# pixeli99/SVD_Xtend

Hardware: NVIDIA H100
Metric: SVD UNet train-step frames/sec @ 14x320x512 bf16 (higher is better)
Workload: dtype bf16

## Files before the change

include/svd_xtend_b200.h:

```cpp
#ifndef SVD_XTEND_B200_H_
#define SVD_XTEND_B200_H_

#include <stdint.h>

#ifdef __cplusplus
extern "C" {
#endif

#define SVDX_OK 0
#define SVDX_E_BADARG (-1)
#define SVDX_E_CUDA (-2)
#define SVDX_E_NODRIVER (-3)

#define SVDX_MAX_TAPS 27

#define SVDX_A_ROWS 0
#define SVDX_A_CONV2D 1

#define SVDX_OUT_BF16 0
#define SVDX_OUT_F32 1
#define SVDX_OUT_F32_ATOMIC 2

typedef struct SvdxTapGemm {
  const void* a;
  int64_t lda;
  int32_t a_mode;
  int32_t a_major_mn;
  int32_t rows_per_group, groups;
  int32_t W, H, nimg;
  int32_t num_taps;
  int32_t tap_d0[SVDX_MAX_TAPS];
  int32_t tap_d1[SVDX_MAX_TAPS];
  int32_t tap_d2[SVDX_MAX_TAPS];
  const void* b;
  int64_t ldb;
  int32_t b_major_mn;
  int32_t b_mode;
  int32_t M, N, K;
  int32_t block_n;
  int32_t split_k;
  void* out;
  int64_t ldo;
  int32_t out_dtype;
  int32_t geglu;
  const float* bias;
  const float* rowbias;
  int32_t rowbias_div;
  int64_t ldrb;
  const void* res1;
  int64_t ldr1;
  const void* res2;
  int64_t ldr2;
  const float* scales;
  void* pre;
  int64_t ldpre;
  float* gn_sum;
  int64_t gn_ld;
  int32_t gn_rows;
  const void* gnb_x;
  int64_t gnb_ldx;
  const void* gnb_x2;
  int64_t gnb_ldx2;
  int32_t gnb_c1;
  const float* gnb_ab;
  float* gnb_sum;
  int32_t gnb_rows;
  int32_t gnb_silu;
  int32_t interleave;
  int32_t phase_h, phase_w;
  int32_t act;
} SvdxTapGemm;

#define SVDX_ACT_NONE 0
#define SVDX_ACT_GELU 1
#define SVDX_ACT_QUICK_GELU 2

int svdx_tapgemm(const SvdxTapGemm* desc, void* stream);

int svdx_splitk_epilogue(float* ws, int64_t ldw, void* out, int64_t ldo, int64_t rows, int32_t cols, const float* bias,
                         const float* rowbias, int32_t rowbias_div, int64_t ldrb, const void* res1, int64_t ldr1,
                         const void* res2, int64_t ldr2, const float* scales, void* stream);

int svdx_num_sms(void);
int svdx_enable_peer_access(int32_t peer_device);
int svdx_ipc_export(const void* ptr, void* handle64_out, int64_t* offset_out);
int svdx_ipc_import(const void* handle64, int64_t offset, void** ptr_out);
int svdx_struct_size(int which);
const char* svdx_last_error(void);

int svdx_groupnorm_sums(const void* x, int64_t ldx, int32_t C1, const void* x2, int64_t ldx2, int32_t C2,
                        int32_t outer, int32_t rows, float* sums, int64_t ld, void* stream);
int svdx_groupnorm_apply_fused(const void* x, int64_t ldx, int32_t C1, const void* x2, int64_t ldx2, int32_t C2,
                               int32_t outer, int32_t rows, int32_t num_groups, float eps,
                               const float* csum1, int64_t ldc1, const float* csum2, int64_t ldc2,
                               float* mean, float* rstd, const float* gamma, const float* beta,
                               int32_t fuse_silu, void* y, int64_t ldy, float* ab_out, void* stream);
int svdx_groupnorm_bwd_sums(const void* x, int64_t ldx, int32_t C1, const void* x2, int64_t ldx2, int32_t C2,
                            const void* dy, int64_t lddy, int32_t outer, int32_t rows, const float* ab, int32_t fuse_silu,
                            float* sums, void* stream);
int svdx_groupnorm_bwd_fused(const void* x, int64_t ldx, int32_t C1, const void* x2, int64_t ldx2, int32_t C2,
                             const void* dy, int64_t lddy, int32_t outer, int32_t rows, int32_t num_groups,
                             const float* mean, const float* rstd, const float* gamma, const float* beta,
                             int32_t fuse_silu, const float* csum, void* dx, int64_t lddx, void* dx2, int64_t lddx2,
                             float* dgamma, float* dbeta, const void* dres, int64_t lddres, void* stream);

int svdx_layernorm_fwd(const void* x, int64_t ldx, int32_t rows, int32_t C, const float* gamma, const float* beta,
                       float eps, void* y, int64_t ldy, float* mean, float* rstd,
                       const float* addvec, int32_t add_div, void* xsum, int64_t ldxs, void* stream);
int svdx_layernorm_bwd(const void* x, int64_t ldx, const void* dy, int64_t lddy, int32_t rows, int32_t C,
                       const float* gamma, const float* mean, const float* rstd,
                       void* dx, int64_t lddx, const void* dres, int64_t lddres,
                       float* dgamma, float* dbeta, void* stream);

typedef struct SvdxAttn {
  const void* q; const void* k; const void* v; void* o;
  int64_t ldq, ldk, ldv, ldo;
  int32_t nseq, heads, S;
  int32_t inner;
  int64_t outer_stride, inner_stride, tok_stride;
  float scale;
  float* lse;
  const void* dout; int64_t lddo;
  void* dq; void* dk; void* dv; int64_t lddq, lddk, lddv;
  float* delta;
} SvdxAttn;
int svdx_attention_fwd(const SvdxAttn* d, void* stream);
int svdx_attention_bwd(const SvdxAttn* d, void* stream);

int svdx_attention_hd80_fwd(const void* q, int64_t ldq, const void* k, int64_t ldk, const void* v, int64_t ldv, void* o,
                            int64_t ldo, int32_t nseq, int32_t heads, int32_t S, float scale, void* stream);

#define SVDX_CLIP_MAX_TAPS 63
int svdx_clip_preprocess(const void* x, int32_t x_dtype, const int64_t* x_strides, int32_t B, int32_t H, int32_t W,
                         const float* gy, int32_t ky, const float* gx, int32_t kx, const float* affine,
                         int32_t out_size, int32_t patch, void* out, int64_t ldo, void* stream);

int svdx_prep_weight(const void* src, int32_t src_bf16, void* dst, int32_t mode,
                     int32_t O, int32_t I, int32_t taps, int32_t i_pad, void* stream);
int svdx_unprep_conv_grad(const float* src, float* dst, int32_t O, int32_t I, int32_t taps, int32_t i_pad, void* stream);
int svdx_dot_diff(const void* dy, const void* a, const void* b, int64_t n, float* out, void* stream);
int svdx_silu_bwd_f32(const float* x, const float* dy, float* dx, int64_t n, void* stream);
int svdx_cast_f32_bf16(const float* src, void* dst, int64_t n, void* stream);
int svdx_cast_bf16_f32(const void* src, float* dst, int64_t n, void* stream);
int svdx_cast_f16_f32(const void* src, float* dst, int64_t n, void* stream);
int svdx_nchw_to_nhwc(const void* src, int32_t src_bf16, void* dst, int32_t N, int32_t C, int32_t H, int32_t W,
                      int32_t c_pad, void* stream);
int svdx_nhwc_to_nchw(const void* src, int64_t lds, void* dst, int32_t dst_bf16, int32_t N, int32_t C, int32_t H,
                      int32_t W, void* stream);
int svdx_time_conv_out(const float* x, int64_t ldx, int32_t N, int32_t T, int32_t C, int32_t H, int32_t W, const float* w,
                       const float* bias, void* y, int32_t y_dtype, void* stream);
int svdx_upsample2x(const void* src, void* dst, int32_t N, int32_t H, int32_t W, int32_t C, void* stream);
int svdx_upsample2x_bwd(const void* dsrc, void* ddst, int32_t N, int32_t H, int32_t W, int32_t C, void* stream);
int svdx_space_to_planes(const void* src, void* dst, int32_t N, int32_t H, int32_t W, int32_t C, void* stream);
int svdx_planes_to_space(const void* src, void* dst, int32_t N, int32_t H, int32_t W, int32_t C, void* stream);
int svdx_concat_channels(const void* a, int32_t Ca, const void* b, int32_t Cb, void* dst, int64_t rows, void* stream);
int svdx_split_channels(const void* src, void* a, int32_t Ca, void* b, int32_t Cb, int64_t rows, int32_t accumulate_a,
                        void* stream);
int svdx_add_bf16(const void* a, const void* b, void* y, int64_t n, void* stream);
int svdx_axpby_bf16(const void* a, const void* b, const float* scales, void* y, int64_t n, void* stream);
int svdx_silu_f32(const float* x, float* y, int64_t n, void* stream);
int svdx_colsum(const void* x, int64_t ldx, int64_t rows, int32_t cols, float* out, int32_t accumulate, void* stream);
int svdx_geglu_bwd(const void* pre, int64_t ldpre, const void* dout, int64_t lddo, void* dpre, int64_t lddpre,
                   int64_t rows, int32_t h, float* bias_grad, void* stream);
int svdx_softmax_rows(const void* x, int64_t ldx, int64_t rows, int32_t cols, float scale, void* y, int64_t ldy, void* stream);
int svdx_gemv(const void* a, int64_t lda, const void* w, int64_t ldw, int32_t M, int32_t N, int32_t K, const float* bias,
              void* out, int64_t ldo, int32_t out_dtype, float scale, int32_t accumulate, void* stream);
int svdx_outer_accum(const void* dy, int64_t lddy, const void* x, int64_t ldx, int32_t T, int32_t O, int32_t K,
                     const float* scale, float* g, int64_t ldg, void* stream);
int svdx_blend_scales(const float* mix_factor, float* out16, void* stream);
int svdx_adamw_graph(float* p, const float* g, float* m, float* v, int64_t n, float* state, float grad_scale,
                     void* shadow_bf16, void* stream);
int svdx_adamw_p2p(float* p, float* m, float* v, const void* const* grads, void* const* shadows, int32_t world,
                   int64_t lo, int64_t n, float* state, float grad_scale, int32_t tick, void* stream);

int svdx_grad_sumsq(const float* g, int64_t n, double* sumsq, void* stream);
int svdx_grad_sumsq_p2p(const void* const* grads, int32_t world, int64_t lo, int64_t n, double* sumsq, void* stream);
int svdx_clip_coef(const double* sumsq, const float* max_norm, float scale, float* out, void* stream);

int svdx_adamw_graph_ema(float* p, const float* g, float* m, float* v, int64_t n, float* state, float grad_scale,
                         void* shadow_bf16, float* ema, double* ema_state, void* stream);
int svdx_adamw_p2p_ema(float* p, float* m, float* v, const void* const* grads, void* const* shadows, int32_t world,
                       int64_t lo, int64_t n, float* state, float grad_scale, int32_t tick, float* ema, double* ema_state,
                       void* stream);
int svdx_ema_multi(const void* jobs, const int32_t* block_prefix, int32_t njobs, int32_t total_blocks, double* ema_state,
                   void* stream);

int svdx_adamw8bit(const void* jobs, const int32_t* block_prefix, int32_t njobs, int32_t total_blocks, const float* qmap1,
                   const float* qmap2, float* state, float grad_scale, void* stream);
int svdx_adamw8bit_ema(const void* jobs, const int32_t* block_prefix, int32_t njobs, int32_t total_blocks, const float* qmap1,
                       const float* qmap2, float* state, float grad_scale, double* ema_state, void* stream);

int svdx_adamw_graph_mul(float* p, const float* g, float* m, float* v, int64_t n, float* state, float grad_scale,
                         void* shadow_bf16, const float* grad_mul, void* stream);
int svdx_adamw_graph_ema_mul(float* p, const float* g, float* m, float* v, int64_t n, float* state, float grad_scale,
                             void* shadow_bf16, float* ema, double* ema_state, const float* grad_mul, void* stream);
int svdx_adamw_p2p_mul(float* p, float* m, float* v, const void* const* grads, void* const* shadows, int32_t world,
                       int64_t lo, int64_t n, float* state, float grad_scale, int32_t tick, const float* grad_mul, void* stream);
int svdx_adamw_p2p_ema_mul(float* p, float* m, float* v, const void* const* grads, void* const* shadows, int32_t world,
                           int64_t lo, int64_t n, float* state, float grad_scale, int32_t tick, float* ema, double* ema_state,
                           const float* grad_mul, void* stream);
int svdx_adamw8bit_mul(const void* jobs, const int32_t* block_prefix, int32_t njobs, int32_t total_blocks, const float* qmap1,
                       const float* qmap2, float* state, float grad_scale, const float* grad_mul, void* stream);
int svdx_adamw8bit_ema_mul(const void* jobs, const int32_t* block_prefix, int32_t njobs, int32_t total_blocks, const float* qmap1,
                           const float* qmap2, float* state, float grad_scale, double* ema_state, const float* grad_mul, void* stream);

int svdx_vae_frames_in(const void* x, int32_t x_dtype, const float* cond_eps, const float* cond_sigma, int32_t B, int32_t F,
                       int32_t H, int32_t W, int32_t c_pad, void* dst, void* stream);
int svdx_vae_frames_in_range(const void* x, int32_t x_dtype, const float* cond_eps, const float* cond_sigma, int32_t B, int32_t F,
                             int32_t H, int32_t W, int32_t first, int32_t count, int32_t c_pad, void* dst, void* stream);
typedef struct svdx_clip_desc {
  int64_t start;
  int32_t H0, W0;
  int32_t ty_off, tx_off;
} svdx_clip_desc;
int svdx_resize_taps_ksize(int32_t in_size, int32_t out_size);
int svdx_resize_taps(int32_t in_size, int32_t out_size, int32_t* taps);
int svdx_resize_taps_box_ksize(int32_t in_size, int32_t out_size, float in0, float in1);
int svdx_resize_taps_box(int32_t in_size, int32_t out_size, float in0, float in1, int32_t* taps);
int svdx_frames_u8_in(const uint8_t* src, int32_t H0, int32_t W0, const int32_t* taps_y, int32_t ksize_y, const int32_t* taps_x,
                      int32_t ksize_x, const float* cond_eps, const float* cond_sigma, int32_t B, int32_t F, int32_t H, int32_t W,
                      int32_t first, int32_t count, int32_t c_pad, void* dst, float* first_frames, void* stream);
int svdx_frames_u8_in_clips(const uint8_t* src, int64_t src_bytes, const svdx_clip_desc* descs, const int32_t* taps_y,
                            int32_t ty_rows, int32_t ksize_y, const int32_t* taps_x, int32_t tx_rows, int32_t ksize_x,
// ... 17 lines not shown
```

svd_xtend_b200/_lib.py:

```python
from __future__ import annotations

import ctypes as C
import os
from pathlib import Path

PKG = Path(__file__).resolve().parent
LIB_PATH = Path(os.environ["SVDX_LIB"]) if os.environ.get("SVDX_LIB") else PKG / "lib" / "libsvdx_b200.so"

SVDX_MAX_TAPS = 27
SVDX_CLIP_MAX_TAPS = 63
A_ROWS, A_CONV2D = 0, 1
OUT_BF16, OUT_F32, OUT_F32_ATOMIC = 0, 1, 2
ACT_NONE, ACT_GELU, ACT_QUICK_GELU = 0, 1, 2

c_void_p, c_int, c_i64, c_float = C.c_void_p, C.c_int32, C.c_int64, C.c_float


class SvdxTapGemm(C.Structure):
    _fields_ = [
        ("a", c_void_p), ("lda", c_i64), ("a_mode", c_int), ("a_major_mn", c_int),
        ("rows_per_group", c_int), ("groups", c_int),
        ("W", c_int), ("H", c_int), ("nimg", c_int),
        ("num_taps", c_int),
        ("tap_d0", c_int * SVDX_MAX_TAPS), ("tap_d1", c_int * SVDX_MAX_TAPS), ("tap_d2", c_int * SVDX_MAX_TAPS),
        ("b", c_void_p), ("ldb", c_i64), ("b_major_mn", c_int), ("b_mode", c_int),
        ("M", c_int), ("N", c_int), ("K", c_int),
        ("block_n", c_int), ("split_k", c_int),
        ("out", c_void_p), ("ldo", c_i64), ("out_dtype", c_int), ("geglu", c_int),
        ("bias", c_void_p), ("rowbias", c_void_p), ("rowbias_div", c_int), ("ldrb", c_i64),
        ("res1", c_void_p), ("ldr1", c_i64), ("res2", c_void_p), ("ldr2", c_i64),
        ("scales", c_void_p), ("pre", c_void_p), ("ldpre", c_i64),
        ("gn_sum", c_void_p), ("gn_ld", c_i64), ("gn_rows", c_int),
        ("gnb_x", c_void_p), ("gnb_ldx", c_i64), ("gnb_x2", c_void_p), ("gnb_ldx2", c_i64), ("gnb_c1", c_int),
        ("gnb_ab", c_void_p), ("gnb_sum", c_void_p), ("gnb_rows", c_int), ("gnb_silu", c_int),
        ("interleave", c_int), ("phase_h", c_int), ("phase_w", c_int),
        ("act", c_int),
    ]


class SvdxAttn(C.Structure):
    _fields_ = [
        ("q", c_void_p), ("k", c_void_p), ("v", c_void_p), ("o", c_void_p),
        ("ldq", c_i64), ("ldk", c_i64), ("ldv", c_i64), ("ldo", c_i64),
        ("nseq", c_int), ("heads", c_int), ("S", c_int), ("inner", c_int),
        ("outer_stride", c_i64), ("inner_stride", c_i64), ("tok_stride", c_i64),
        ("scale", c_float), ("lse", c_void_p),
        ("dout", c_void_p), ("lddo", c_i64),
        ("dq", c_void_p), ("dk", c_void_p), ("dv", c_void_p),
        ("lddq", c_i64), ("lddk", c_i64), ("lddv", c_i64),
        ("delta", c_void_p),
    ]


_PROTOS = {
    "svdx_tapgemm": [C.POINTER(SvdxTapGemm), c_void_p],
    "svdx_splitk_epilogue": [c_void_p, c_i64, c_void_p, c_i64, c_i64, c_int, c_void_p, c_void_p, c_int, c_i64, c_void_p, c_i64,
                             c_void_p, c_i64, c_void_p, c_void_p],
    "svdx_num_sms": [],
    "svdx_enable_peer_access": [c_int],
    "svdx_ipc_export": [c_void_p, c_void_p, c_void_p],
    "svdx_ipc_import": [c_void_p, c_i64, c_void_p],
    "svdx_struct_size": [c_int],
    "svdx_groupnorm_sums": [c_void_p, c_i64, c_int, c_void_p, c_i64, c_int, c_int, c_int, c_void_p, c_i64, c_void_p],
    "svdx_groupnorm_apply_fused": [c_void_p, c_i64, c_int, c_void_p, c_i64, c_int, c_int, c_int, c_int, c_float,
                                   c_void_p, c_i64, c_void_p, c_i64, c_void_p, c_void_p, c_void_p, c_void_p, c_int, c_void_p, c_i64, c_void_p,
                                   c_void_p],
    "svdx_groupnorm_bwd_fused": [c_void_p, c_i64, c_int, c_void_p, c_i64, c_int, c_void_p, c_i64, c_int, c_int, c_int,
                                 c_void_p, c_void_p, c_void_p, c_void_p, c_int, c_void_p, c_void_p, c_i64, c_void_p, c_i64,
                                 c_void_p, c_void_p, c_void_p, c_i64, c_void_p],
    "svdx_groupnorm_bwd_sums": [c_void_p, c_i64, c_int, c_void_p, c_i64, c_int, c_void_p, c_i64, c_int, c_int, c_void_p, c_int,
                                c_void_p, c_void_p],
    "svdx_layernorm_fwd": [c_void_p, c_i64, c_int, c_int, c_void_p, c_void_p, c_float, c_void_p, c_i64,
                           c_void_p, c_void_p, c_void_p, c_int, c_void_p, c_i64, c_void_p],
    "svdx_layernorm_bwd": [c_void_p, c_i64, c_void_p, c_i64, c_int, c_int, c_void_p, c_void_p, c_void_p,
                           c_void_p, c_i64, c_void_p, c_i64, c_void_p, c_void_p, c_void_p],
    "svdx_attention_fwd": [C.POINTER(SvdxAttn), c_void_p],
    "svdx_attention_bwd": [C.POINTER(SvdxAttn), c_void_p],
    "svdx_attention_hd80_fwd": [c_void_p, c_i64, c_void_p, c_i64, c_void_p, c_i64, c_void_p, c_i64, c_int, c_int, c_int, c_float, c_void_p],
    "svdx_clip_preprocess": [c_void_p, c_int, C.POINTER(c_i64), c_int, c_int, c_int, C.POINTER(c_float), c_int, C.POINTER(c_float), c_int,
                             C.POINTER(c_float), c_int, c_int, c_void_p, c_i64, c_void_p],
    "svdx_prep_weight": [c_void_p, c_int, c_void_p, c_int, c_int, c_int, c_int, c_int, c_void_p],
    "svdx_unprep_conv_grad": [c_void_p, c_void_p, c_int, c_int, c_int, c_int, c_void_p],
    "svdx_dot_diff": [c_void_p, c_void_p, c_void_p, c_i64, c_void_p, c_void_p],
    "svdx_silu_bwd_f32": [c_void_p, c_void_p, c_void_p, c_i64, c_void_p],
    "svdx_cast_f32_bf16": [c_void_p, c_void_p, c_i64, c_void_p],
    "svdx_cast_bf16_f32": [c_void_p, c_void_p, c_i64, c_void_p],
    "svdx_cast_f16_f32": [c_void_p, c_void_p, c_i64, c_void_p],
    "svdx_nchw_to_nhwc": [c_void_p, c_int, c_void_p, c_int, c_int, c_int, c_int, c_int, c_void_p],
    "svdx_nhwc_to_nchw": [c_void_p, c_i64, c_void_p, c_int, c_int, c_int, c_int, c_int, c_void_p],
    "svdx_time_conv_out": [c_void_p, c_i64, c_int, c_int, c_int, c_int, c_int, c_void_p, c_void_p, c_void_p, c_int, c_void_p],
    "svdx_upsample2x": [c_void_p, c_void_p, c_int, c_int, c_int, c_int, c_void_p],
    "svdx_upsample2x_bwd": [c_void_p, c_void_p, c_int, c_int, c_int, c_int, c_void_p],
    "svdx_space_to_planes": [c_void_p, c_void_p, c_int, c_int, c_int, c_int, c_void_p],
    "svdx_planes_to_space": [c_void_p, c_void_p, c_int, c_int, c_int, c_int, c_void_p],
    "svdx_concat_channels": [c_void_p, c_int, c_void_p, c_int, c_void_p, c_i64, c_void_p],
    "svdx_split_channels": [c_void_p, c_void_p, c_int, c_void_p, c_int, c_i64, c_int, c_void_p],
    "svdx_add_bf16": [c_void_p, c_void_p, c_void_p, c_i64, c_void_p],
    "svdx_axpby_bf16": [c_void_p, c_void_p, c_void_p, c_void_p, c_i64, c_void_p],
    "svdx_silu_f32": [c_void_p, c_void_p, c_i64, c_void_p],
    "svdx_colsum": [c_void_p, c_i64, c_i64, c_int, c_void_p, c_int, c_void_p],
    "svdx_geglu_bwd": [c_void_p, c_i64, c_void_p, c_i64, c_void_p, c_i64, c_i64, c_int, c_void_p, c_void_p],
    "svdx_softmax_rows": [c_void_p, c_i64, c_i64, c_int, c_float, c_void_p, c_i64, c_void_p],
    "svdx_gemv": [c_void_p, c_i64, c_void_p, c_i64, c_int, c_int, c_int, c_void_p, c_void_p, c_i64, c_int, c_float, c_int, c_void_p],
    "svdx_outer_accum": [c_void_p, c_i64, c_void_p, c_i64, c_int, c_int, c_int, c_void_p, c_void_p, c_i64, c_void_p],
    "svdx_blend_scales": [c_void_p, c_void_p, c_void_p],
    "svdx_adamw_graph": [c_void_p, c_void_p, c_void_p, c_void_p, c_i64, c_void_p, c_float, c_void_p, c_void_p],
    "svdx_adamw_p2p": [c_void_p, c_void_p, c_void_p, c_void_p, c_void_p, c_int, c_i64, c_i64, c_void_p, c_float, c_int, c_void_p],
    "svdx_grad_sumsq": [c_void_p, c_i64, c_void_p, c_void_p],
    "svdx_grad_sumsq_p2p": [c_void_p, c_int, c_i64, c_i64, c_void_p, c_void_p],
    "svdx_clip_coef": [c_void_p, c_void_p, c_float, c_void_p, c_void_p],
    "svdx_adamw_graph_ema": [c_void_p, c_void_p, c_void_p, c_void_p, c_i64, c_void_p, c_float, c_void_p, c_void_p, c_void_p, c_void_p],
    "svdx_adamw_p2p_ema": [c_void_p, c_void_p, c_void_p, c_void_p, c_void_p, c_int, c_i64, c_i64, c_void_p, c_float, c_int, c_void_p,
                           c_void_p, c_void_p],
    "svdx_ema_multi": [c_void_p, c_void_p, c_int, c_int, c_void_p, c_void_p],
    "svdx_adamw8bit": [c_void_p, c_void_p, c_int, c_int, c_void_p, c_void_p, c_void_p, c_float, c_void_p],
    "svdx_adamw8bit_ema": [c_void_p, c_void_p, c_int, c_int, c_void_p, c_void_p, c_void_p, c_float, c_void_p, c_void_p],
    "svdx_adamw_graph_mul": [c_void_p, c_void_p, c_void_p, c_void_p, c_i64, c_void_p, c_float, c_void_p, c_void_p, c_void_p],
    "svdx_adamw_graph_ema_mul": [c_void_p, c_void_p, c_void_p, c_void_p, c_i64, c_void_p, c_float, c_void_p, c_void_p, c_void_p,
                                 c_void_p, c_void_p],
    "svdx_adamw_p2p_mul": [c_void_p, c_void_p, c_void_p, c_void_p, c_void_p, c_int, c_i64, c_i64, c_void_p, c_float, c_int, c_void_p,
                           c_void_p],
    "svdx_adamw_p2p_ema_mul": [c_void_p, c_void_p, c_void_p, c_void_p, c_void_p, c_int, c_i64, c_i64, c_void_p, c_float, c_int,
                               c_void_p, c_void_p, c_void_p, c_void_p],
    "svdx_adamw8bit_mul": [c_void_p, c_void_p, c_int, c_int, c_void_p, c_void_p, c_void_p, c_float, c_void_p, c_void_p],
    "svdx_adamw8bit_ema_mul": [c_void_p, c_void_p, c_int, c_int, c_void_p, c_void_p, c_void_p, c_float, c_void_p, c_void_p, c_void_p],
    "svdx_multi_transpose": [c_void_p, c_void_p, c_void_p, c_int, c_int, c_void_p],
    "svdx_lora_merge": [c_void_p, c_void_p, c_void_p, c_int, c_int, c_void_p],
    "svdx_vae_frames_in": [c_void_p, c_int, c_void_p, c_void_p, c_int, c_int, c_int, c_int, c_int, c_void_p, c_void_p],
    "svdx_vae_frames_in_range": [c_void_p, c_int, c_void_p, c_void_p, c_int, c_int, c_int, c_int, c_int, c_int, c_int, c_void_p,
                                 c_void_p],
    "svdx_resize_taps_ksize": [c_int, c_int],
    "svdx_resize_taps": [c_int, c_int, c_void_p],
    "svdx_resize_taps_box_ksize": [c_int, c_int, c_float, c_float],
    "svdx_resize_taps_box": [c_int, c_int, c_float, c_float, c_void_p],
    "svdx_frames_u8_in": [c_void_p, c_int, c_int, c_void_p, c_int, c_void_p, c_int, c_void_p, c_void_p, c_int, c_int, c_int, c_int,
                          c_int, c_int, c_int, c_void_p, c_void_p, c_void_p],
    "svdx_frames_u8_in_clips": [c_void_p, c_i64, c_void_p, c_void_p, c_int, c_int, c_void_p, c_int, c_int, c_void_p, c_void_p, c_int,
                                c_int, c_int, c_int, c_int, c_int, c_int, c_void_p, c_void_p, c_void_p],
    "svdx_edm_prepare": [c_void_p, c_void_p, c_void_p, c_void_p, c_void_p, c_void_p, c_float, c_int, c_int, c_int, c_int, c_int,
                         c_void_p, c_void_p, c_void_p, c_void_p],
}

EXPORTED_SYMBOLS = tuple(_PROTOS) + ("svdx_last_error",)

_lib = None


def load() -> C.CDLL:
    global _lib
    if _lib is None:
        if not LIB_PATH.exists():
            raise RuntimeError(
                f"svd_xtend_b200: native library {LIB_PATH} is missing — run `python -m svd_xtend_b200.build` "
                "(there is no CPU or PyTorch fallback for the hot path)")
        lib = C.CDLL(str(LIB_PATH))
        missing = [n for n in _PROTOS if not hasattr(lib, n)]
        if missing and os.environ.get("SVDX_ALLOW_PARTIAL"):
            for n in missing:
                _PROTOS.pop(n)
            missing = []
        if missing:
            raise RuntimeError(f"svd_xtend_b200: {LIB_PATH} lacks symbols {missing}; rebuild it")
        for name, args in _PROTOS.items():
            fn = getattr(lib, name)
            fn.argtypes = args
            fn.restype = C.c_int
        if lib.svdx_struct_size(0) != C.sizeof(SvdxTapGemm) or lib.svdx_struct_size(1) != C.sizeof(SvdxAttn):
            raise RuntimeError("svd_xtend_b200: ctypes struct layout does not match the C ABI")
        lib.svdx_last_error.restype = C.c_char_p
        lib.svdx_last_error.argtypes = []
        _lib = lib
    return _lib


class SvdxError(RuntimeError):
    pass


def check(rc: int, what: str = "") -> None:
    if rc != 0:
        msg = load().svdx_last_error().decode(errors="replace")
        raise SvdxError(f"{what} failed with status {rc}: {msg}")
```

svd_xtend_b200/csrc/common.cuh:

```cuda
#pragma once
#include <cuda.h>
#include <cuda_bf16.h>
#include <cuda_runtime.h>
#include <stdint.h>
#include <stdio.h>

#include "wgmma.cuh"

namespace svdx {

typedef __nv_bfloat16 bf16;

#define SVDX_DEVINL __device__ __forceinline__

#ifndef SVDX_WAIT_TIMEOUT_CYCLES
#define SVDX_WAIT_TIMEOUT_CYCLES (4000000000ll)
#endif

SVDX_DEVINL uint32_t smem_u32(const void* p) { return (uint32_t)__cvta_generic_to_shared(p); }

SVDX_DEVINL uint32_t lane_id() { return threadIdx.x & 31; }

SVDX_DEVINL bool elect_one() {
  uint32_t pred = 0;
// ... 8 lines not shown
SVDX_DEVINL void mbar_init(uint32_t bar, uint32_t count) {
  asm volatile("mbarrier.init.shared::cta.b64 [%0], %1;" ::"r"(bar), "r"(count) : "memory");
}
SVDX_DEVINL void fence_barrier_init() {
  asm volatile("fence.mbarrier_init.release.cluster;" ::: "memory");
}
SVDX_DEVINL void fence_proxy_async_smem() {
  asm volatile("fence.proxy.async.shared::cta;" ::: "memory");
}
SVDX_DEVINL void mbar_expect_tx(uint32_t bar, uint32_t bytes) {
  asm volatile("mbarrier.arrive.expect_tx.shared::cta.b64 _, [%0], %1;" ::"r"(bar), "r"(bytes) : "memory");
}
SVDX_DEVINL void mbar_arrive(uint32_t bar) {
  asm volatile("mbarrier.arrive.shared::cta.b64 _, [%0];" ::"r"(bar) : "memory");
}
SVDX_DEVINL bool mbar_try_wait(uint32_t bar, uint32_t parity) {
  uint32_t ok;
  asm volatile(
      "{\n\t.reg .pred P;\n\t"
      "mbarrier.try_wait.parity.shared::cta.b64 P, [%1], %2;\n\t"
      "selp.u32 %0, 1, 0, P;\n\t}\n"
      : "=r"(ok)
      : "r"(bar), "r"(parity)
      : "memory");
  return ok != 0;
}
SVDX_DEVINL void mbar_wait(uint32_t bar, uint32_t parity) {
  if (mbar_try_wait(bar, parity)) return;
  long long t0 = clock64();
  while (!mbar_try_wait(bar, parity)) {
    if (clock64() - t0 > SVDX_WAIT_TIMEOUT_CYCLES) {
      printf("svdx: mbarrier wait timeout block %d thread %d bar %u parity %u\n", blockIdx.x, threadIdx.x, bar, parity);
      __trap();
    }
  }
}

SVDX_DEVINL void mbar_wait_mma(uint32_t bar, uint32_t parity) {
  if (mbar_try_wait(bar, parity)) return;
  long long t0 = clock64();
  while (!mbar_try_wait(bar, parity))
    if (clock64() - t0 > SVDX_WAIT_TIMEOUT_CYCLES) __trap();
}

SVDX_DEVINL void prefetch_tmap(const CUtensorMap* m) {
  asm volatile("prefetch.tensormap [%0];" ::"l"(reinterpret_cast<uint64_t>(m)) : "memory");
}
SVDX_DEVINL void tma_load_2d(const CUtensorMap* m, uint32_t bar, uint32_t dst, int c0, int c1) {
  asm volatile(
      "cp.async.bulk.tensor.2d.shared::cluster.global.mbarrier::complete_tx::bytes [%0], [%1, {%3, %4}], [%2];"
      ::"r"(dst), "l"(reinterpret_cast<uint64_t>(m)), "r"(bar), "r"(c0), "r"(c1)
      : "memory");
}
SVDX_DEVINL void tma_load_3d(const CUtensorMap* m, uint32_t bar, uint32_t dst, int c0, int c1, int c2) {
  asm volatile(
      "cp.async.bulk.tensor.3d.shared::cluster.global.mbarrier::complete_tx::bytes [%0], [%1, {%3, %4, %5}], [%2];"
      ::"r"(dst), "l"(reinterpret_cast<uint64_t>(m)), "r"(bar), "r"(c0), "r"(c1), "r"(c2)
      : "memory");
}
SVDX_DEVINL void tma_load_4d(const CUtensorMap* m, uint32_t bar, uint32_t dst, int c0, int c1, int c2, int c3) {
  asm volatile(
      "cp.async.bulk.tensor.4d.shared::cluster.global.mbarrier::complete_tx::bytes [%0], [%1, {%3, %4, %5, %6}], [%2];"
      ::"r"(dst), "l"(reinterpret_cast<uint64_t>(m)), "r"(bar), "r"(c0), "r"(c1), "r"(c2), "r"(c3)
      : "memory");
}
SVDX_DEVINL void tma_load_4d_im2col(const CUtensorMap* m, uint32_t bar, uint32_t dst, int c0, int c1, int c2, int c3, uint16_t ow,
                                    uint16_t oh) {
  asm volatile(
      "cp.async.bulk.tensor.4d.shared::cluster.global.im2col.mbarrier::complete_tx::bytes [%0], [%1, {%3, %4, %5, %6}], [%2], {%7, %8};"
      ::"r"(dst), "l"(reinterpret_cast<uint64_t>(m)), "r"(bar), "r"(c0), "r"(c1), "r"(c2), "r"(c3), "h"(ow), "h"(oh)
      : "memory");
}

SVDX_DEVINL void tma_store_3d(const CUtensorMap* m, uint32_t src, int c0, int c1, int c2) {
  asm volatile("cp.async.bulk.tensor.3d.global.shared::cta.bulk_group [%0, {%2, %3, %4}], [%1];"
               ::"l"(reinterpret_cast<uint64_t>(m)), "r"(src), "r"(c0), "r"(c1), "r"(c2)
               : "memory");
}
SVDX_DEVINL void tma_store_4d(const CUtensorMap* m, uint32_t src, int c0, int c1, int c2, int c3) {
  asm volatile("cp.async.bulk.tensor.4d.global.shared::cta.bulk_group [%0, {%2, %3, %4, %5}], [%1];"
               ::"l"(reinterpret_cast<uint64_t>(m)), "r"(src), "r"(c0), "r"(c1), "r"(c2), "r"(c3)
               : "memory");
}
SVDX_DEVINL void tma_reduce_add_3d(const CUtensorMap* m, uint32_t src, int c0, int c1, int c2) {
  asm volatile("cp.reduce.async.bulk.tensor.3d.global.shared::cta.add.bulk_group [%0, {%2, %3, %4}], [%1];"
               ::"l"(reinterpret_cast<uint64_t>(m)), "r"(src), "r"(c0), "r"(c1), "r"(c2)
               : "memory");
}
SVDX_DEVINL void bulk_commit() { asm volatile("cp.async.bulk.commit_group;" ::: "memory"); }
template <int N>
SVDX_DEVINL void bulk_wait_read() { asm volatile("cp.async.bulk.wait_group.read %0;" ::"n"(N) : "memory"); }
template <int N>
SVDX_DEVINL void bulk_wait() { asm volatile("cp.async.bulk.wait_group %0;" ::"n"(N) : "memory"); }
SVDX_DEVINL void st_shared_v4(uint32_t addr, uint32_t a, uint32_t b, uint32_t c, uint32_t d) {
  asm volatile("st.shared.v4.b32 [%0], {%1, %2, %3, %4};" ::"r"(addr), "r"(a), "r"(b), "r"(c), "r"(d) : "memory");
}

SVDX_DEVINL void wgmma_fence() { asm volatile("wgmma.fence.sync.aligned;" ::: "memory"); }
SVDX_DEVINL void wgmma_commit() { asm volatile("wgmma.commit_group.sync.aligned;" ::: "memory"); }
template <int N>
SVDX_DEVINL void wgmma_wait() { asm volatile("wgmma.wait_group.sync.aligned %0;" ::"n"(N) : "memory"); }
template <int R>
SVDX_DEVINL void reg_fence(float (&d)[R]) {
#pragma unroll
  for (int i = 0; i < R; ++i) asm volatile("" : "+f"(d[i])::"memory");
}

SVDX_DEVINL void named_bar_sync(int id, int nthreads) { asm volatile("bar.sync %0, %1;" ::"r"(id), "r"(nthreads) : "memory"); }

SVDX_DEVINL uint64_t make_smem_desc_sw128(uint32_t saddr, uint32_t lbo_bytes, uint32_t sbo_bytes) {
  uint64_t d = 0;
  d |= (uint64_t)((saddr & 0x3FFFF) >> 4);
  d |= (uint64_t)((lbo_bytes >> 4) & 0x3FFF) << 16;
  d |= (uint64_t)((sbo_bytes >> 4) & 0x3FFF) << 32;
  d |= (uint64_t)1 << 62;
  return d;
}

SVDX_DEVINL float silu_f(float x) { return __fdividef(x, 1.0f + __expf(-x)); }
SVDX_DEVINL float silu_grad_f(float x) {
  const float s = __fdividef(1.0f, 1.0f + __expf(-x));
  return s * fmaf(x, 1.0f - s, 1.0f);
}
#define SVDX_HDINL __host__ __device__ __forceinline__
SVDX_HDINL float gelu_tail_log2(float ax) {
  float p = -1.92123457e-06f;
  p = fmaf(p, ax, 6.32884985e-05f);
  p = fmaf(p, ax, -0.000943420862f);
  p = fmaf(p, ax, 0.0085562719f);
  p = fmaf(p, ax, -0.0540522821f);
  p = fmaf(p, ax, -0.458381772f);
  p = fmaf(p, ax, -1.15127838f);
  p = fmaf(p, ax, -0.999993861f);
  return p;
}
SVDX_HDINL float exp2_fast(float x) {
#ifdef __CUDA_ARCH__
  float y;
  asm("ex2.approx.ftz.f32 %0, %1;" : "=f"(y) : "f"(x));
  return y;
#else
  return exp2f(x);
#endif
}
SVDX_HDINL float normal_cdf_f(float x) {
  const float q = exp2_fast(gelu_tail_log2(fminf(fabsf(x), 5.5f)));
  return x < 0.f ? q : 1.0f - q;
}
SVDX_HDINL float gelu_erf_f(float x) { return x * normal_cdf_f(x); }
SVDX_HDINL float gelu_erf_grad_f(float x) {
  const float pdf = 0.3989422804014327f * exp2_fast(-0.72134752044448170f * x * x);
  return fmaf(x, pdf, normal_cdf_f(x));
}

SVDX_DEVINL uint32_t pack_bf16x2(float lo, float hi) {
  __nv_bfloat162 v = __floats2bfloat162_rn(lo, hi);
  return *reinterpret_cast<uint32_t*>(&v);
}
SVDX_DEVINL float2 unpack_bf16x2(uint32_t u) {
  __nv_bfloat162 v = *reinterpret_cast<__nv_bfloat162*>(&u);
  return __bfloat1622float2(v);
}

SVDX_DEVINL float warp_sum(float v) {
#pragma unroll
  for (int o = 16; o > 0; o >>= 1) v += __shfl_xor_sync(0xffffffffu, v, o);
  return v;
}
SVDX_DEVINL float warp_max(float v) {
#pragma unroll
  for (int o = 16; o > 0; o >>= 1) v = fmaxf(v, __shfl_xor_sync(0xffffffffu, v, o));
  return v;
}

}
```

svd_xtend_b200/csrc/elementwise.cu:

```cuda
#include "common.cuh"
#include "../../include/svd_xtend_b200.h"
#include "host_util.h"
#include <cuda_fp16.h>
#include <type_traits>

namespace svdx {

SVDX_DEVINL long long gtid() { return (long long)blockIdx.x * blockDim.x + threadIdx.x; }
static inline unsigned nblocks(long long n, int threads = 256) { return (unsigned)((n + threads - 1) / threads); }

template <typename T>
SVDX_DEVINL float ldf(const T* p, long long i);
template <>
SVDX_DEVINL float ldf<float>(const float* p, long long i) { return p[i]; }
template <>
SVDX_DEVINL float ldf<bf16>(const bf16* p, long long i) { return __bfloat162float(p[i]); }
template <>
SVDX_DEVINL float ldf<__half>(const __half* p, long long i) { return __half2float(p[i]); }

template <typename T>
__global__ void prep_gather_kernel(const T* __restrict__ src, bf16* __restrict__ dst, int mode, int O, int I, int taps, int i_pad) {
  const long long idx = gtid();
  if (mode == 0) {
    if (idx >= (long long)O * I) return;
// ... 137 lines not shown
  const int w2 = (int)(pix % (2 * W));
  const int h2 = (int)((pix / (2 * W)) % (2 * H));
  const int n = (int)(pix / ((long long)4 * W * H));
  dst[idx] = src[(((long long)n * H + (h2 >> 1)) * W + (w2 >> 1)) * CV + cv];
}
SVDX_DEVINL uint32_t add_bf16x2_f32(uint32_t a, uint32_t b, uint32_t c, uint32_t d) {
  const float2 x = unpack_bf16x2(a), y = unpack_bf16x2(b), z = unpack_bf16x2(c), w = unpack_bf16x2(d);
  return pack_bf16x2(x.x + y.x + z.x + w.x, x.y + y.y + z.y + w.y);
}
__global__ void upsample2x_bwd_kernel(const uint4* __restrict__ dsrc, uint4* __restrict__ ddst, int N, int H, int W, int CV) {
  const long long idx = gtid();
  const long long total = (long long)N * H * W * CV;
  if (idx >= total) return;
  const int cv = (int)(idx % CV);
  const long long pix = idx / CV;
  const int w = (int)(pix % W);
  const int h = (int)((pix / W) % H);
  const int n = (int)(pix / ((long long)W * H));
  const long long base = (((long long)n * 2 * H + 2 * h) * 2 * W + 2 * w) * CV + cv;
  const uint4 a = dsrc[base], b = dsrc[base + CV], c = dsrc[base + (long long)2 * W * CV], d = dsrc[base + (long long)2 * W * CV + CV];
  uint4 o;
  o.x = add_bf16x2_f32(a.x, b.x, c.x, d.x); o.y = add_bf16x2_f32(a.y, b.y, c.y, d.y);
  o.z = add_bf16x2_f32(a.z, b.z, c.z, d.z); o.w = add_bf16x2_f32(a.w, b.w, c.w, d.w);
  ddst[idx] = o;
}

__global__ void planes_kernel(const uint4* __restrict__ src, uint4* __restrict__ dst, int N, int H, int W, int CV, int to_planes) {
  const long long idx = gtid();
  const long long total = (long long)N * H * W * CV;
  if (idx >= total) return;
  const int cv = (int)(idx % CV);
  const long long pix = idx / CV;
  const int w = (int)(pix % W);
  const int h = (int)((pix / W) % H);
  const int n = (int)(pix / ((long long)W * H));
  const int Ho = H / 2, Wo = W / 2;
  const long long pidx = ((((long long)((h & 1) * 2 + (w & 1)) * N + n) * Ho + (h >> 1)) * Wo + (w >> 1)) * CV + cv;
  if (to_planes) dst[pidx] = src[idx]; else dst[idx] = src[pidx];
}

__global__ void concat_kernel(const uint4* __restrict__ a, int CVa, const uint4* __restrict__ b, int CVb, uint4* __restrict__ dst, long long rows) {
  const long long idx = gtid();
  const int CV = CVa + CVb;
  if (idx >= rows * CV) return;
  const long long r = idx / CV;
  const int c = (int)(idx - r * CV);
  dst[idx] = (c < CVa) ? a[r * CVa + c] : b[r * CVb + (c - CVa)];
}
__global__ void split_kernel(const uint4* __restrict__ src, uint4* __restrict__ a, int CVa, uint4* __restrict__ b, int CVb, long long rows,
                             int accumulate_a) {
  const long long idx = gtid();
  const int CV = CVa + CVb;
  if (idx >= rows * CV) return;
  const long long r = idx / CV;
  const int c = (int)(idx - r * CV);
  const uint4 v = src[idx];
  if (c < CVa) {
    uint4* p = a + r * CVa + c;
    if (accumulate_a) {
      const uint4 o = *p;
      uint4 s;
      float2 x, y;
      x = unpack_bf16x2(o.x); y = unpack_bf16x2(v.x); s.x = pack_bf16x2(x.x + y.x, x.y + y.y);
      x = unpack_bf16x2(o.y); y = unpack_bf16x2(v.y); s.y = pack_bf16x2(x.x + y.x, x.y + y.y);
      x = unpack_bf16x2(o.z); y = unpack_bf16x2(v.z); s.z = pack_bf16x2(x.x + y.x, x.y + y.y);
      x = unpack_bf16x2(o.w); y = unpack_bf16x2(v.w); s.w = pack_bf16x2(x.x + y.x, x.y + y.y);
      *p = s;
    } else {
      *p = v;
    }
  } else if (b) {
    b[r * CVb + (c - CVa)] = v;
  }
}

__global__ void axpby_kernel(const uint4* __restrict__ a, const uint4* __restrict__ b, const float* __restrict__ scales, uint4* __restrict__ y,
                             long long nvec) {
  const long long idx = gtid();
  if (idx >= nvec) return;
  const float s0 = scales ? scales[0] : 1.f, s1 = scales ? scales[1] : 1.f;
  const uint4 u = a[idx], v = b[idx];
  uint4 o;
  float2 x, z;
  x = unpack_bf16x2(u.x); z = unpack_bf16x2(v.x); o.x = pack_bf16x2(s0 * x.x + s1 * z.x, s0 * x.y + s1 * z.y);
  x = unpack_bf16x2(u.y); z = unpack_bf16x2(v.y); o.y = pack_bf16x2(s0 * x.x + s1 * z.x, s0 * x.y + s1 * z.y);
  x = unpack_bf16x2(u.z); z = unpack_bf16x2(v.z); o.z = pack_bf16x2(s0 * x.x + s1 * z.x, s0 * x.y + s1 * z.y);
  x = unpack_bf16x2(u.w); z = unpack_bf16x2(v.w); o.w = pack_bf16x2(s0 * x.x + s1 * z.x, s0 * x.y + s1 * z.y);
  y[idx] = o;
}

__global__ void silu_f32_kernel(const float* __restrict__ x, float* __restrict__ y, long long n) {
  const long long i = gtid();
  if (i < n) y[i] = silu_f(x[i]);
}

__global__ void __launch_bounds__(256) colsum_kernel(const bf16* __restrict__ x, long long ldx, long long rows, int cols, long long rows_per_cta,
                                                     float* __restrict__ out) {
  __shared__ float sh[8][256 + 8];
  const int cvl = threadIdx.x & 31, rl = threadIdx.x >> 5;
  const int c0 = (blockIdx.x * 32 + cvl) * 8;
  const long long r0 = (long long)blockIdx.y * rows_per_cta;
  const long long r1 = min(r0 + rows_per_cta, rows);
  float a[8];
#pragma unroll
  for (int k = 0; k < 8; ++k) a[k] = 0.f;
  if (c0 < cols) {
    long long r = r0 + rl;
    for (; r + 24 < r1; r += 32) {
      uint4 u[4];
#pragma unroll
      for (int q = 0; q < 4; ++q) u[q] = *reinterpret_cast<const uint4*>(x + (r + 8 * q) * ldx + c0);
#pragma unroll
      for (int q = 0; q < 4; ++q) {
        const uint32_t w[4] = {u[q].x, u[q].y, u[q].z, u[q].w};
#pragma unroll
        for (int k = 0; k < 4; ++k) { const float2 v = unpack_bf16x2(w[k]); a[2 * k] += v.x; a[2 * k + 1] += v.y; }
      }
    }
    for (; r < r1; r += 8) {
      const uint4 u = *reinterpret_cast<const uint4*>(x + r * ldx + c0);
      const uint32_t w[4] = {u.x, u.y, u.z, u.w};
#pragma unroll
      for (int k = 0; k < 4; ++k) { const float2 v = unpack_bf16x2(w[k]); a[2 * k] += v.x; a[2 * k + 1] += v.y; }
    }
  }
#pragma unroll
  for (int k = 0; k < 8; ++k) sh[rl][cvl * 8 + k] = a[k];
  __syncthreads();
  {
    const int c = threadIdx.x;
    float sacc = 0.f;
#pragma unroll
    for (int k = 0; k < 8; ++k) sacc += sh[k][c];
    const int cc = blockIdx.x * 256 + c;
    if (cc < cols) atomicAdd(out + cc, sacc);
  }
}

__global__ void geglu_bwd_plain_kernel(const bf16* __restrict__ pre, long long ldpre, const bf16* __restrict__ dout, long long lddo,
                                       bf16* __restrict__ dpre, long long lddpre, long long rows, int h) {
  const long long idx = gtid();
  const int hv = h / 8;
  if (idx >= rows * hv) return;
  const long long r = idx / hv;
  const int c = (int)(idx - r * hv) * 8;
  const uint4 uv = *reinterpret_cast<const uint4*>(pre + r * ldpre + c);
  const uint4 ug = *reinterpret_cast<const uint4*>(pre + r * ldpre + h + c);
  const uint4 ud = *reinterpret_cast<const uint4*>(dout + r * lddo + c);
  const uint32_t v[4] = {uv.x, uv.y, uv.z, uv.w}, g[4] = {ug.x, ug.y, ug.z, ug.w}, d[4] = {ud.x, ud.y, ud.z, ud.w};
  uint32_t ov[4], og[4];
#pragma unroll
  for (int k = 0; k < 4; ++k) {
    const float2 fv = unpack_bf16x2(v[k]), fg = unpack_bf16x2(g[k]), fd = unpack_bf16x2(d[k]);
    ov[k] = pack_bf16x2(fd.x * gelu_erf_f(fg.x), fd.y * gelu_erf_f(fg.y));
    og[k] = pack_bf16x2(fd.x * fv.x * gelu_erf_grad_f(fg.x), fd.y * fv.y * gelu_erf_grad_f(fg.y));
  }
  *reinterpret_cast<uint4*>(dpre + r * lddpre + c) = make_uint4(ov[0], ov[1], ov[2], ov[3]);
  *reinterpret_cast<uint4*>(dpre + r * lddpre + h + c) = make_uint4(og[0], og[1], og[2], og[3]);
}

__global__ void __launch_bounds__(256, 2) geglu_bwd_kernel(const bf16* __restrict__ pre, long long ldpre, const bf16* __restrict__ dout, long long lddo,
                                                        bf16* __restrict__ dpre, long long lddpre, long long rows, int h, long long rows_per_cta,
                                                        float* __restrict__ bias_grad) {
  __shared__ float sh[8][2][256 + 8];
  const int cvl = threadIdx.x & 31, rl = threadIdx.x >> 5;
  const int c = (blockIdx.x * 32 + cvl) * 8;
  const long long r0 = (long long)blockIdx.y * rows_per_cta;
  const long long r1 = min(r0 + rows_per_cta, rows);
  float av[8], ag[8];
#pragma unroll
  for (int k = 0; k < 8; ++k) { av[k] = 0.f; ag[k] = 0.f; }
  if (c < h) {
    for (long long r = r0 + rl; r < r1; r += 32) {
      uint4 uv[4], ug[4], ud[4];
#pragma unroll
      for (int q = 0; q < 4; ++q) {
        if (r + 8 * q < r1) {
          uv[q] = *reinterpret_cast<const uint4*>(pre + (r + 8 * q) * ldpre + c);
          ug[q] = *reinterpret_cast<const uint4*>(pre + (r + 8 * q) * ldpre + h + c);
          ud[q] = *reinterpret_cast<const uint4*>(dout + (r + 8 * q) * lddo + c);
        }
      }
#pragma unroll
      for (int q = 0; q < 4; ++q) {
        if (r + 8 * q >= r1) break;
        const uint32_t v[4] = {uv[q].x, uv[q].y, uv[q].z, uv[q].w}, g[4] = {ug[q].x, ug[q].y, ug[q].z, ug[q].w}, d[4] = {ud[q].x, ud[q].y, ud[q].z, ud[q].w};
        uint32_t ov[4], og[4];
#pragma unroll
        for (int k = 0; k < 4; ++k) {
          const float2 fv = unpack_bf16x2(v[k]), fg = unpack_bf16x2(g[k]), fd = unpack_bf16x2(d[k]);
          ov[k] = pack_bf16x2(fd.x * gelu_erf_f(fg.x), fd.y * gelu_erf_f(fg.y));
          og[k] = pack_bf16x2(fd.x * fv.x * gelu_erf_grad_f(fg.x), fd.y * fv.y * gelu_erf_grad_f(fg.y));
          const float2 rv = unpack_bf16x2(ov[k]), rg = unpack_bf16x2(og[k]);
          av[2 * k] += rv.x; av[2 * k + 1] += rv.y;
          ag[2 * k] += rg.x; ag[2 * k + 1] += rg.y;
        }
        const long long rr = r + 8 * q;
        *reinterpret_cast<uint4*>(dpre + rr * lddpre + c) = make_uint4(ov[0], ov[1], ov[2], ov[3]);
        *reinterpret_cast<uint4*>(dpre + rr * lddpre + h + c) = make_uint4(og[0], og[1], og[2], og[3]);
      }
    }
  }
#pragma unroll
  for (int k = 0; k < 8; ++k) { sh[rl][0][cvl * 8 + k] = av[k]; sh[rl][1][cvl * 8 + k] = ag[k]; }
  __syncthreads();
  {
    const int cc = threadIdx.x;
    float s0 = 0.f, s1 = 0.f;
#pragma unroll
    for (int k = 0; k < 8; ++k) { s0 += sh[k][0][cc]; s1 += sh[k][1][cc]; }
    const int col = blockIdx.x * 256 + cc;
    if (col < h) { atomicAdd(bias_grad + col, s0); atomicAdd(bias_grad + h + col, s1); }
  }
}

__global__ void unprep_conv_grad_kernel(const float* __restrict__ src, float* __restrict__ dst, int O, int I, int taps, int i_pad) {
  const long long idx = gtid();
  if (idx >= (long long)O * I * taps) return;
  const int t = (int)(idx % taps);
  const int i = (int)((idx / taps) % I);
  const int o = (int)(idx / ((long long)taps * I));
  dst[idx] += src[((long long)o * taps + t) * i_pad + i];
}

__global__ void __launch_bounds__(256) dot_diff_kernel(const uint4* __restrict__ dy, const uint4* __restrict__ a, const uint4* __restrict__ b,
                                                       long long nvec, float* out) {
  float acc = 0.f;
  for (long long i = gtid(); i < nvec; i += (long long)gridDim.x * blockDim.x) {
    const uint4 d = dy[i], x = a[i], y = b[i];
    const uint32_t dd[4] = {d.x, d.y, d.z, d.w}, xx[4] = {x.x, x.y, x.z, x.w}, yy[4] = {y.x, y.y, y.z, y.w};
#pragma unroll
    for (int k = 0; k < 4; ++k) {
      const float2 fd = unpack_bf16x2(dd[k]), fx = unpack_bf16x2(xx[k]), fy = unpack_bf16x2(yy[k]);
      acc += fd.x * (fx.x - fy.x) + fd.y * (fx.y - fy.y);
    }
  }
  acc = warp_sum(acc);
  __shared__ float sh[8];
  if ((threadIdx.x & 31) == 0) sh[threadIdx.x >> 5] = acc;
  __syncthreads();
  if (threadIdx.x == 0) {
    float s = 0.f;
    for (int k = 0; k < 8; ++k) s += sh[k];
    atomicAdd(out, s);
  }
}

__global__ void silu_bwd_f32_kernel(const float* __restrict__ x, const float* __restrict__ dy, float* __restrict__ dx, long long n) {
  const long long i = gtid();
  if (i < n) dx[i] = dy[i] * silu_grad_f(x[i]);
}

__global__ void __launch_bounds__(256) splitk_epilogue_kernel(float* __restrict__ ws, long long ldw, bf16* __restrict__ out, long long ldo,
                                                              long long rows, int cols, const float* __restrict__ bias,
                                                              const float* __restrict__ rowbias, int rb_div, long long ldrb,
                                                              const bf16* __restrict__ res1, long long ldr1, const bf16* __restrict__ res2,
                                                              long long ldr2, const float* __restrict__ scales) {
  const int cv = cols / 8;
  const long long idx = gtid();
  if (idx >= rows * cv) return;
  const long long r = idx / cv;
  const int c = (int)(idx - r * cv) * 8;
  float s0 = 1.f, s1 = 1.f, s2 = 1.f;
  if (scales) { s0 = scales[0]; s1 = scales[1]; s2 = scales[2]; }
  const float4 a = *reinterpret_cast<const float4*>(ws + r * ldw + c);
  const float4 b = *reinterpret_cast<const float4*>(ws + r * ldw + c + 4);
  *reinterpret_cast<float4*>(ws + r * ldw + c) = make_float4(0.f, 0.f, 0.f, 0.f);
  *reinterpret_cast<float4*>(ws + r * ldw + c + 4) = make_float4(0.f, 0.f, 0.f, 0.f);
  float f[8] = {a.x, a.y, a.z, a.w, b.x, b.y, b.z, b.w};
  if (bias) {
#pragma unroll
    for (int k = 0; k < 8; ++k) f[k] += bias[c + k];
  }
  if (rowbias) {
    const float* rb = rowbias + (r / rb_div) * ldrb + c;
#pragma unroll
    for (int k = 0; k < 8; ++k) f[k] += rb[k];
  }
#pragma unroll
  for (int k = 0; k < 8; ++k) f[k] *= s0;
  if (res1) {
    const uint4 u = *reinterpret_cast<const uint4*>(res1 + r * ldr1 + c);
    const uint32_t w[4] = {u.x, u.y, u.z, u.w};
#pragma unroll
    for (int k = 0; k < 4; ++k) { const float2 v = unpack_bf16x2(w[k]); f[2 * k] += s1 * v.x; f[2 * k + 1] += s1 * v.y; }
  }
  if (res2) {
    const uint4 u = *reinterpret_cast<const uint4*>(res2 + r * ldr2 + c);
    const uint32_t w[4] = {u.x, u.y, u.z, u.w};
#pragma unroll
    for (int k = 0; k < 4; ++k) { const float2 v = unpack_bf16x2(w[k]); f[2 * k] += s2 * v.x; f[2 * k + 1] += s2 * v.y; }
  }
  *reinterpret_cast<uint4*>(out + r * ldo + c) =
      make_uint4(pack_bf16x2(f[0], f[1]), pack_bf16x2(f[2], f[3]), pack_bf16x2(f[4], f[5]), pack_bf16x2(f[6], f[7]));
}

__global__ void blend_scales_kernel(const float* mix, float* out) {
  const float a = 1.f / (1.f + __expf(-mix[0]));
  out[0] = 1.f - a; out[1] = a; out[2] = 1.f - a; out[3] = 0.f;
  out[4] = 1.f - a; out[5] = 1.f; out[6] = 0.f; out[7] = a * (1.f - a);
  out[8] = 1.f - a; out[9] = 0.f; out[10] = 0.f; out[11] = 0.f;
  out[12] = a; out[13] = 0.f; out[14] = 1.f - a; out[15] = 0.f;
}

SVDX_DEVINL void adamw_advance(float* state) {
  const float step = state[5] + 1.f;
  state[5] = step;
  state[6] = 1.f - powf(state[1], step);
  state[7] = 1.f - powf(state[2], step);
}
__global__ void adamw_tick_kernel(float* state) { adamw_advance(state); }

SVDX_DEVINL void ema_advance(double* s) {
  const double t = s[0] + 1.0;
  s[0] = t;
  const double st = fmax(0.0, t - s[3] - 1.0);
  double d = 0.0;
  if (st > 0.0) {
    d = s[4] != 0.0 ? 1.0 - pow(1.0 + st / s[5], -s[6]) : (1.0 + st) / (10.0 + st);
    d = fmax(fmin(d, s[1]), s[2]);
  }
  s[7] = d;
  s[8] = 1.0 - d;
}
__global__ void ema_tick_kernel(double* ema_state) { ema_advance(ema_state); }
__global__ void adamw_ema_tick_kernel(float* state, double* ema_state) {
  adamw_advance(state);
  ema_advance(ema_state);
}
SVDX_DEVINL float ema_update(float e, float p, float omd) { return __fsub_rn(e, __fmul_rn(omd, __fsub_rn(e, p))); }

SVDX_DEVINL float4 ema_update4(float4 e, const float* p, float omd) {
  return make_float4(ema_update(e.x, p[0], omd), ema_update(e.y, p[1], omd), ema_update(e.z, p[2], omd), ema_update(e.w, p[3], omd));
}

struct AdamCoef {
  float b1, b2, eps, decay, step_size, inv_sqrt_bc2;
};
SVDX_DEVINL AdamCoef adamw_coef(const float* __restrict__ state) {
  const float lr = state[0], b1 = state[1], b2 = state[2], eps = state[3], wd = state[4], bc1 = state[6], bc2 = state[7];
  return {b1, b2, eps, 1.f - lr * wd, lr / bc1, rsqrtf(bc2)};
}
SVDX_DEVINL void adamw_update(const AdamCoef& c, float g, float& p, float& m, float& v) {
  m = c.b1 * m + (1.f - c.b1) * g;
  v = c.b2 * v + (1.f - c.b2) * g * g;
// ... 1145 lines not shown
```

svd_xtend_b200/csrc/tapgemm.cu:

```cuda
#include "tapgemm_common.cuh"

namespace svdx {

struct Ring {
  uint32_t sA, sB, bar_full, bar_empty;
  int stage;
  uint32_t phase;
};
template <int BN, int TA, int TB, int STG>
__device__ __forceinline__ void tile_mainloop(float (&acc)[BN / 2], int kb0, int kb1, Ring& rg, int wg) {
#pragma unroll
  for (int i = 0; i < BN / 2; ++i) acc[i] = 0.f;
  const int lane = threadIdx.x & 31;
  const uint32_t astep = TA ? (2048 >> 4) : (32 >> 4), bstep = TB ? (2048 >> 4) : (32 >> 4);
  int prev_stage = -1;
  for (int kb = kb0; kb < kb1; ++kb) {
    mbar_wait_mma(rg.bar_full + 8 * rg.stage, rg.phase);
    const uint32_t aaddr = rg.sA + rg.stage * A_STAGE_BYTES + wg * 8192;
    const uint32_t baddr = rg.sB + rg.stage * B_STAGE_BYTES;
    const uint64_t ad0 = make_smem_desc_sw128(aaddr, 8192, 1024);
    const uint64_t bd0 = make_smem_desc_sw128(baddr, 8192, 1024);
    wgmma_fence();
#pragma unroll
    for (int j = 0; j < BLOCK_K / 16; ++j) {
      const uint32_t accumulate = (kb > kb0 || j > 0) ? 1u : 0u;
      if constexpr (BN == 32) wgmma_ss_n32<TA, TB>(acc, ad0 + j * astep, bd0 + j * bstep, accumulate);
      else if constexpr (BN == 64) wgmma_ss_n64<TA, TB>(acc, ad0 + j * astep, bd0 + j * bstep, accumulate);
      else if constexpr (BN == 96) wgmma_ss_n96<TA, TB>(acc, ad0 + j * astep, bd0 + j * bstep, accumulate);
      else if constexpr (BN == 128) wgmma_ss_n128<TA, TB>(acc, ad0 + j * astep, bd0 + j * bstep, accumulate);
      else wgmma_ss_n160<TA, TB>(acc, ad0 + j * astep, bd0 + j * bstep, accumulate);
    }
    wgmma_commit();
    wgmma_wait<1>();
    reg_fence(acc);
    if (prev_stage >= 0) {
      __syncwarp();
      if (lane == 0) mbar_arrive(rg.bar_empty + 8 * prev_stage);
    }
    prev_stage = rg.stage;
    if (++rg.stage == STG) { rg.stage = 0; rg.phase ^= 1; }
  }
  wgmma_wait<0>();
  reg_fence(acc);
  __syncwarp();
  if (lane == 0 && prev_stage >= 0) mbar_arrive(rg.bar_empty + 8 * prev_stage);
}

template <int BN, int TA, int TB>
SVDX_DEVINL void tile_parked_bn(int kb0, int kb1, Ring& rg, uint32_t sAcc, int wg) {
  float acc[BN / 2];
  tile_mainloop<BN, TA, TB, STAGES_PARKED>(acc, kb0, kb1, rg, wg);
  const int lane = threadIdx.x & 31;
  const int r0 = wg * 64 + ((threadIdx.x >> 5) & 3) * 16 + (lane >> 2);
  const uint32_t base = sAcc + (uint32_t)(r0 * ACC_LD + 2 * (lane & 3)) * 4u;
#pragma unroll
  for (int j = 0; j < BN / 8; ++j) {
#pragma unroll
    for (int h = 0; h < 2; ++h)
      asm volatile("st.shared.v2.f32 [%0], {%1, %2};" ::"r"(base + (uint32_t)(h * 8 * ACC_LD + 8 * j) * 4u), "f"(acc[4 * j + 2 * h]),
                   "f"(acc[4 * j + 2 * h + 1]) : "memory");
  }
}

template <int TA, int TB>
SVDX_DEVINL void tile_parked(int bn, int kb0, int kb1, Ring& rg, uint32_t sAcc, int wg) {
  switch (bn) {
    case 32: tile_parked_bn<32, TA, TB>(kb0, kb1, rg, sAcc, wg); break;
    case 64: tile_parked_bn<64, TA, TB>(kb0, kb1, rg, sAcc, wg); break;
    case 96: tile_parked_bn<96, TA, TB>(kb0, kb1, rg, sAcc, wg); break;
    case 128: tile_parked_bn<128, TA, TB>(kb0, kb1, rg, sAcc, wg); break;
    default: tile_parked_bn<160, TA, TB>(kb0, kb1, rg, sAcc, wg); break;
  }
}

template <int EPI, int BN, int TB>
SVDX_DEVINL void tile_regs_bn(const TapGemmKParams& p, int kb0, int kb1, Ring& rg, int wg, PairStage& ps, const EpiTile& t, int lane,
                              float s_acc, float s_r1, float s_r2) {
  float acc[BN / 2];
  tile_mainloop<BN, 0, TB, STAGES_REGS>(acc, kb0, kb1, rg, wg);
  epilogue_regs<EPI, BN>(p, acc, ps, t, lane, s_acc, s_r1, s_r2);
}

template <int EPI>
SVDX_DEVINL void tile_regs(const TapGemmKParams& p, int kb0, int kb1, Ring& rg, int wg, PairStage& ps, const EpiTile& t, int lane,
                           float s_acc, float s_r1, float s_r2) {
  if constexpr (EPI == EPI_GEGLU) {
    if (p.block_n == 64) tile_regs_bn<EPI, 64, 0>(p, kb0, kb1, rg, wg, ps, t, lane, s_acc, s_r1, s_r2);
    else tile_regs_bn<EPI, 128, 0>(p, kb0, kb1, rg, wg, ps, t, lane, s_acc, s_r1, s_r2);
  } else {
    if constexpr (EPI == EPI_FAST) {
      if (p.b_mn) {
        if (p.block_n == 64) tile_regs_bn<EPI, 64, 1>(p, kb0, kb1, rg, wg, ps, t, lane, s_acc, s_r1, s_r2);
        else tile_regs_bn<EPI, 128, 1>(p, kb0, kb1, rg, wg, ps, t, lane, s_acc, s_r1, s_r2);
        return;
      }
    }
    switch (p.block_n) {
      case 32: tile_regs_bn<EPI, 32, 0>(p, kb0, kb1, rg, wg, ps, t, lane, s_acc, s_r1, s_r2); break;
      case 64: tile_regs_bn<EPI, 64, 0>(p, kb0, kb1, rg, wg, ps, t, lane, s_acc, s_r1, s_r2); break;
      case 96: tile_regs_bn<EPI, 96, 0>(p, kb0, kb1, rg, wg, ps, t, lane, s_acc, s_r1, s_r2); break;
      case 128: tile_regs_bn<EPI, 128, 0>(p, kb0, kb1, rg, wg, ps, t, lane, s_acc, s_r1, s_r2); break;
      default: tile_regs_bn<EPI, 160, 0>(p, kb0, kb1, rg, wg, ps, t, lane, s_acc, s_r1, s_r2); break;
    }
  }
}

template <int BN, int TA, int TB>
SVDX_DEVINL void tile_f32_bn(const TapGemmKParams& p, int kb0, int kb1, Ring& rg, int wg, EpiStage& st, const EpiTile& t, int sub, int lane,
                             float s_acc) {
  float acc[BN / 2];
  tile_mainloop<BN, TA, TB, STAGES_REGS>(acc, kb0, kb1, rg, wg);
  epilogue_f32<BN>(p, acc, st, t, sub, lane, s_acc);
}

template <int TA>
SVDX_DEVINL void tile_f32(const TapGemmKParams& p, int kb0, int kb1, Ring& rg, int wg, EpiStage& st, const EpiTile& t, int sub, int lane,
                          float s_acc) {
  if (p.b_mn) {
    if (p.block_n == 64) tile_f32_bn<64, TA, 1>(p, kb0, kb1, rg, wg, st, t, sub, lane, s_acc);
    else tile_f32_bn<128, TA, 1>(p, kb0, kb1, rg, wg, st, t, sub, lane, s_acc);
    return;
  }
  switch (p.block_n) {
    case 32: tile_f32_bn<32, TA, 0>(p, kb0, kb1, rg, wg, st, t, sub, lane, s_acc); break;
    case 64: tile_f32_bn<64, TA, 0>(p, kb0, kb1, rg, wg, st, t, sub, lane, s_acc); break;
    case 96: tile_f32_bn<96, TA, 0>(p, kb0, kb1, rg, wg, st, t, sub, lane, s_acc); break;
    case 128: tile_f32_bn<128, TA, 0>(p, kb0, kb1, rg, wg, st, t, sub, lane, s_acc); break;
    default: tile_f32_bn<160, TA, 0>(p, kb0, kb1, rg, wg, st, t, sub, lane, s_acc); break;
  }
}

template <int EPI>
__global__ void __launch_bounds__(NUM_THREADS, 1) tapgemm_kernel(const __grid_constant__ TapGemmKParams p) {
  constexpr bool PARKED = EPI == EPI_GENERIC;
  constexpr int STAGES = PARKED ? STAGES_PARKED : STAGES_REGS;
  extern __shared__ uint8_t smem_raw[];
  const uint32_t smem_base = (smem_u32(smem_raw) + 1023u) & ~1023u;
  const uint32_t sA = smem_base;
  const uint32_t sB = smem_base + STAGES * A_STAGE_BYTES;
  const uint32_t sAcc = sB + STAGES * B_STAGE_BYTES;
  const uint32_t sEpi = sAcc + (PARKED ? ACC_BYTES : 0);
  const uint32_t sBar = sEpi + NUM_EPI_WARPS * EPI_STAGE_BYTES;
  const uint32_t bar_full = sBar;
  const uint32_t bar_empty = sBar + 8 * STAGES;

  const int warp = threadIdx.x >> 5;
  const int lane = threadIdx.x & 31;

  if (warp == PRODUCER_WARP && lane == 0) {
    prefetch_tmap(&p.tma);
    prefetch_tmap(&p.tmb);
    for (int i = 0; i < STAGES; ++i) {
      mbar_init(bar_full + 8 * i, 1);
      mbar_init(bar_empty + 8 * i, NUM_EPI_WARPS);
    }
    fence_barrier_init();
  }
  __syncthreads();

  const int total_tiles = p.m_tiles * p.n_tiles * p.split_k;
  const int b_bytes = p.block_n * BLOCK_K * 2;

  if (warp == PRODUCER_WARP) {
    const bool conv_par = (p.a_mode == SVDX_A_CONV2D) && !p.a_mn && !p.b_mn && !p.geglu && !p.wtiles && !p.im2col && (BLOCK_M / p.W) <= 32;
    if (conv_par) {
      int stage = 0;
      uint32_t phase = 0;
      for (int tile = blockIdx.x; tile < total_tiles; tile += gridDim.x) {
        const int nt = tile % p.n_tiles;
        const int mt = (tile / p.n_tiles) % p.m_tiles;
        const int ks = tile / (p.n_tiles * p.m_tiles);
        const int kb0 = ks * p.kb_per_split;
        const int kb1 = min(kb0 + p.kb_per_split, p.kb_total);
        const int n0 = nt * p.block_n;
        ConvBox bx;
        conv_tile_boxes(p, mt, lane, bx);
        const CUtensorMap* amap = bx.lg == 0 ? &p.tma : &p.tma_bh[bx.lg - 1];
        int tap = kb0 / p.kb_per_tap;
        int kci = kb0 - tap * p.kb_per_tap;
        for (int kb = kb0; kb < kb1; ++kb) {
          const uint32_t full = bar_full + 8 * stage;
          if (lane == 0) {
            mbar_wait_mma(bar_empty + 8 * stage, phase ^ 1);
            mbar_expect_tx(full, A_STAGE_BYTES + b_bytes);
          }
          __syncwarp();
          const int kc = kci * BLOCK_K;
          if (bx.active)
            tma_load_4d(amap, full, sA + stage * A_STAGE_BYTES + bx.dst_off, kc, p.tap_d0[tap], bx.hh + p.tap_d1[tap],
                        bx.nvalid ? bx.n + p.tap_d2[tap] : (1 << 28));
          if (lane == 0) tma_load_2d(&p.tmb, full, sB + stage * B_STAGE_BYTES, tap * p.K + kc, n0);
          if (++kci == p.kb_per_tap) { kci = 0; ++tap; }
          if (++stage == STAGES) { stage = 0; phase ^= 1; }
        }
      }
    } else if (p.a_mn && p.b_mn && p.b_mode != 1) {
      int stage = 0;
      uint32_t phase = 0;
      const int nb = p.block_n / 64;
      for (int tile = blockIdx.x; tile < total_tiles; tile += gridDim.x) {
        const int nt = tile % p.n_tiles;
        const int mt = (tile / p.n_tiles) % p.m_tiles;
        const int ks = tile / (p.n_tiles * p.m_tiles);
        const int kb0 = ks * p.kb_per_split;
        const int kb1 = min(kb0 + p.kb_per_split, p.kb_total);
        const int n0 = nt * p.block_n;
        int g = 0, kbi = kb0;
        if (p.b_mode == 2) { g = kb0 / p.kb_per_group; kbi = kb0 - g * p.kb_per_group; }
        const int shift = p.b_mode == 2 ? p.tap_d0[0] : 0;
        for (int kb = kb0; kb < kb1; ++kb) {
          const uint32_t full = bar_full + 8 * stage;
          if (lane == 0) {
            mbar_wait_mma(bar_empty + 8 * stage, phase ^ 1);
            mbar_expect_tx(full, A_STAGE_BYTES + b_bytes);
          }
          __syncwarp();
          const uint32_t dA = sA + stage * A_STAGE_BYTES;
          const uint32_t dB = sB + stage * B_STAGE_BYTES;
          if (p.b_mode == 2) {
            const int k0 = kbi * BLOCK_K;
            if (lane < 2) tma_load_3d(&p.tma, full, dA + lane * 8192, mt * BLOCK_M + 64 * lane, k0, g);
            else if (lane < 2 + nb) tma_load_3d(&p.tmb, full, dB + (lane - 2) * 8192, n0 + 64 * (lane - 2), k0 + shift, g);
            if (++kbi == p.kb_per_group) { kbi = 0; ++g; }
          } else {
            if (lane < 2) tma_load_2d(&p.tma, full, dA + lane * 8192, mt * BLOCK_M + 64 * lane, kb * BLOCK_K);
            else if (lane < 2 + nb) tma_load_2d(&p.tmb, full, dB + (lane - 2) * 8192, n0 + 64 * (lane - 2), kb * BLOCK_K);
          }
          if (++stage == STAGES) { stage = 0; phase ^= 1; }
        }
      }
    } else if (lane == 0) {
      int stage = 0;
      uint32_t phase = 0;
      for (int tile = blockIdx.x; tile < total_tiles; tile += gridDim.x) {
        const int nt = tile % p.n_tiles;
        const int mt = (tile / p.n_tiles) % p.m_tiles;
        const int ks = tile / (p.n_tiles * p.m_tiles);
        const int kb0 = ks * p.kb_per_split;
        const int kb1 = min(kb0 + p.kb_per_split, p.kb_total);
        const int n0 = nt * (p.geglu ? p.block_n / 2 : p.block_n);
        int iw = 0, ih = 0, in = 0;
        if (p.im2col && p.a_mode == SVDX_A_CONV2D) {
          const int row = mt * BLOCK_M / p.W;
          iw = mt * BLOCK_M - row * p.W;
          in = row / p.H;
          ih = row - in * p.H;
        }
        int tap = kb0 / p.kb_per_tap;
        int kci = kb0 - tap * p.kb_per_tap - 1;
        for (int kb = kb0; kb < kb1; ++kb) {
          if (++kci == p.kb_per_tap) { kci = 0; ++tap; }
          mbar_wait_mma(bar_empty + 8 * stage, phase ^ 1);
          const uint32_t full = bar_full + 8 * stage;
          mbar_expect_tx(full, A_STAGE_BYTES + b_bytes);
          const uint32_t dA = sA + stage * A_STAGE_BYTES;
          const uint32_t dB = sB + stage * B_STAGE_BYTES;
          const int kc = kci * BLOCK_K;
          if (p.a_mn) {
            if (p.b_mode == 2) {
              const int g = kb / p.kb_per_group;
              const int k0 = (kb - g * p.kb_per_group) * BLOCK_K;
              tma_load_3d(&p.tma, full, dA, mt * BLOCK_M, k0, g);
              tma_load_3d(&p.tma, full, dA + 8192, mt * BLOCK_M + 64, k0, g);
            } else {
              tma_load_2d(&p.tma, full, dA, mt * BLOCK_M, kb * BLOCK_K);
              tma_load_2d(&p.tma, full, dA + 8192, mt * BLOCK_M + 64, kb * BLOCK_K);
            }
          } else if (p.a_mode == SVDX_A_ROWS) {
            const int g = mt / p.tiles_per_group;
            const int t = mt - g * p.tiles_per_group;
            tma_load_3d(&p.tma, full, dA, kc, t * BLOCK_M + p.tap_d0[tap], g);
          } else if (p.im2col) {
            tma_load_4d_im2col(&p.tma, full, dA, kc, iw - 1, ih - 1, in + p.tap_d2[tap], (uint16_t)(p.tap_d0[tap] + 1),
                               (uint16_t)(p.tap_d1[tap] + 1));
          } else if (p.wtiles) {
            const int row = mt / p.wtiles;
            const int w0 = (mt - row * p.wtiles) * BLOCK_M;
            const int n = row / p.H;
            const int h = row - n * p.H;
            tma_load_4d(&p.tma, full, dA, kc, w0 + p.tap_d0[tap], h + p.tap_d1[tap], (n < p.nimg) ? n + p.tap_d2[tap] : (1 << 28));
          } else {
            const int R = BLOCK_M / p.W;
            const int dw = p.tap_d0[tap], dh = p.tap_d1[tap], dn = p.tap_d2[tap];
            int rowid = mt * R, left = R;
            uint32_t dst = dA;
            while (left > 0) {
              const int n = rowid / p.H;
              const int h = rowid - n * p.H;
              const int nn = (n < p.nimg) ? n + dn : (1 << 28);
              int run = min(left, p.H - h);
              int hh = h;
              while (run > 0) {
                int lg = min(p.max_bh_log2, 31 - __clz(run));
                const int bh = 1 << lg;
                tma_load_4d(lg == 0 ? &p.tma : &p.tma_bh[lg - 1], full, dst, kc, dw, hh + dh, nn);
                dst += bh * p.W * 128;
                hh += bh; run -= bh; left -= bh; rowid += bh;
              }
            }
          }
          if (p.b_mn && p.b_mode == 1 && p.im2col) {
            const int pix0 = kb * BLOCK_K;
            const int row = pix0 / p.W;
            const int n = row / p.H;
            for (int j = 0; j < p.block_n / 64; ++j)
              tma_load_4d_im2col(&p.tmb, full, dB + j * 8192, n0 + 64 * j, pix0 - row * p.W - 1, row - n * p.H - 1, n + p.tap_d2[0],
                                 (uint16_t)(p.tap_d0[0] + 1), (uint16_t)(p.tap_d1[0] + 1));
          } else if (p.b_mn && p.b_mode == 1) {
            const int dw = p.tap_d0[0], dh = p.tap_d1[0], dn = p.tap_d2[0];
            const int pix0 = kb * BLOCK_K;
            for (int j = 0; j < p.block_n / 64; ++j) {
              if (p.W >= 64) {
                const int row = pix0 / p.W;
                const int n = row / p.H;
                const int nn = (n < p.nimg) ? n + dn : (1 << 28);
                tma_load_4d(&p.tmb, full, dB + j * 8192, n0 + 64 * j, pix0 - row * p.W + dw, row - n * p.H + dh, nn);
              } else {
                const int R = 64 / p.W;
                for (int i = 0; i < R; ++i) {
                  const int row = pix0 / p.W + i;
                  const int n = row / p.H;
                  const int nn = (n < p.nimg) ? n + dn : (1 << 28);
                  tma_load_4d(&p.tmb, full, dB + j * 8192 + i * p.W * 128, n0 + 64 * j, dw, row - n * p.H + dh, nn);
                }
              }
            }
          } else if (p.b_mn && p.b_mode == 2) {
            const int g = kb / p.kb_per_group;
            const int k0 = (kb - g * p.kb_per_group) * BLOCK_K;
            for (int j = 0; j < p.block_n / 64; ++j)
              tma_load_3d(&p.tmb, full, dB + j * 8192, n0 + 64 * j, k0 + p.tap_d0[0], g);
          } else if (p.b_mn) {
            for (int j = 0; j < p.block_n / 64; ++j)
              tma_load_2d(&p.tmb, full, dB + j * 8192, n0 + 64 * j, kb * BLOCK_K);
          } else if (p.geglu) {
            const int h = p.block_n / 2;
            tma_load_2d(&p.tmb, full, dB, tap * p.K + kc, n0);
            tma_load_2d(&p.tmb, full, dB + h * 128, tap * p.K + kc, p.N / 2 + n0);
          } else {
            tma_load_2d(&p.tmb, full, dB, tap * p.K + kc, n0);
          }
          if (++stage == STAGES) { stage = 0; phase ^= 1; }
        }
      }
    }
  } else {
    const int wg = warp >> 2;
    const int q = PARKED ? (warp & 3) : (warp >> 1);
    const int half = PARKED ? (warp >> 2) : (warp & 1);
    Ring rg{sA, sB, bar_full, bar_empty, 0, 0u};
    float s_acc = 1.f, s_r1 = 1.f, s_r2 = 1.f;
    if (p.scales) { s_acc = p.scales[0]; s_r1 = p.scales[1]; s_r2 = p.scales[2]; }
    const int n_out_total = p.geglu ? p.N / 2 : p.N;
    const int bn_out = p.geglu ? p.block_n / 2 : p.block_n;
    EpiStage st;
    st.base = sEpi + warp * EPI_STAGE_BYTES;
    st.off = 0;
    PairStage ps{sEpi + q * 2 * EPI_STAGE_BYTES, 2 + q, half, 0u};
    const uint32_t t_base = sAcc + (uint32_t)((q * 32 + lane) * ACC_LD) * 4u;
    for (int tile = blockIdx.x; tile < total_tiles; tile += gridDim.x) {
      const int nt = tile % p.n_tiles;
      const int mt = (tile / p.n_tiles) % p.m_tiles;
      const int ks = tile / (p.n_tiles * p.m_tiles);
      const int kb0 = ks * p.kb_per_split;
      const int kb1 = min(kb0 + p.kb_per_split, p.kb_total);
      const int n0 = nt * bn_out;
      long long m;
      bool row_ok;
      tile_row(p, mt, q * 32 + lane, m, row_ok);
      if (p.a_mode == SVDX_A_ROWS && !p.a_mn) {
        st.grp = mt / p.tiles_per_group;
        st.row0 = (mt - st.grp * p.tiles_per_group) * BLOCK_M + q * 32;
      } else {
        st.grp = 0;
        st.row0 = mt * BLOCK_M + q * 32;
      }
      long long m0;
      int valid_rows;
      if (p.a_mode == SVDX_A_ROWS && !p.a_mn) {
        m0 = (long long)st.grp * p.rows_per_group + st.row0;
        valid_rows = max(0, min(32, p.rows_per_group - st.row0));
      } else {
        m0 = st.row0;
        valid_rows = max(0, min(32, p.M - st.row0));
      }
      if constexpr (EPI == EPI_RES || EPI == EPI_RES_GN || EPI == EPI_FAST_GNB)
        prefetch_epilogue_operands(p, EPI, m0, valid_rows, n0, bn_out, n_out_total, lane, half);
      if constexpr (PARKED) {
        named_bar_sync(1, 32 * NUM_EPI_WARPS);
        if (p.a_mn && p.b_mn) tile_parked<1, 1>(p.block_n, kb0, kb1, rg, sAcc, wg);
        else if (p.a_mn) tile_parked<1, 0>(p.block_n, kb0, kb1, rg, sAcc, wg);
        else if (p.b_mn) tile_parked<0, 1>(p.block_n, kb0, kb1, rg, sAcc, wg);
        else tile_parked<0, 0>(p.block_n, kb0, kb1, rg, sAcc, wg);
        named_bar_sync(1, 32 * NUM_EPI_WARPS);
        epilogue_tile(p, t_base, m, row_ok, n0, half, bn_out, n_out_total, s_acc, s_r1, s_r2, st, lane);
      } else {
        EpiTile et;
        et.n0 = n0; et.n_out_total = n_out_total; et.row0 = st.row0; et.grp = st.grp; et.valid_rows = valid_rows; et.m0 = m0;
#pragma unroll
        for (int h = 0; h < 2; ++h) tile_row(p, mt, q * 32 + half * 16 + (lane >> 2) + 8 * h, et.m[h], et.ok[h]);
        if constexpr (EPI == EPI_F32) {
          if (p.a_mn) tile_f32<1>(p, kb0, kb1, rg, wg, st, et, half, lane, s_acc);
          else tile_f32<0>(p, kb0, kb1, rg, wg, st, et, half, lane, s_acc);
        } else {
          tile_regs<EPI>(p, kb0, kb1, rg, wg, ps, et, lane, s_acc, s_r1, s_r2);
        }
      }
    }
    if (lane == 0) bulk_wait<0>();
  }
}

}

using namespace svdx;

static int kernel_block_n(int block_n, bool step64) {
  const int step = step64 ? 64 : 32, cap = step64 ? 128 : MAX_BN;
  if (block_n <= cap) return block_n;
  for (int w = cap; w > step; w -= step)
    if (block_n % w == 0) return w;
  return step;
}

int svdx_tapgemm_fill(const SvdxTapGemm* d, TapGemmKParams& p) {
  if (!d || !d->a || !d->b || !d->out) return svdx_fail(SVDX_E_BADARG, "tapgemm: null pointer");
  const bool wide320 = d->block_n == 320;
  if (wide320 && (d->geglu || d->N % 320 || d->M < 512 || d->out_dtype != SVDX_OUT_BF16))
    return svdx_fail(SVDX_E_BADARG, "tapgemm: block_n 320 needs N %% 320 == 0, M >= 512 and a bf16 output without GEGLU");
  if (!wide320 && (d->block_n < 32 || d->block_n > 256 || d->block_n % 32))
    return svdx_fail(SVDX_E_BADARG, "tapgemm: block_n must be a multiple of 32 in [32,256] (or 320)");
  if (d->b_major_mn && d->block_n % 64) return svdx_fail(SVDX_E_BADARG, "tapgemm: block_n %% 64 for MN-major B");
  if (d->num_taps < 1 || d->num_taps > SVDX_MAX_TAPS) return svdx_fail(SVDX_E_BADARG, "tapgemm: num_taps");
  if (d->M <= 0 || d->N <= 0 || d->K <= 0) return svdx_fail(SVDX_E_BADARG, "tapgemm: empty problem");
  if (d->split_k < 1 || (d->split_k > 1 && d->out_dtype != SVDX_OUT_F32_ATOMIC)) return svdx_fail(SVDX_E_BADARG, "tapgemm: split_k needs atomic output");
  if (d->geglu && (d->N % 2 || d->block_n % 64 || d->b_major_mn || (d->N / 2) % (d->block_n / 2))) return svdx_fail(SVDX_E_BADARG, "tapgemm: geglu shape");
  if ((d->lda % 8) || (d->ldb % 8)) return svdx_fail(SVDX_E_BADARG, "tapgemm: lda/ldb must be multiples of 8 elements (16 B)");
  if ((reinterpret_cast<uintptr_t>(d->a) & 15) || (reinterpret_cast<uintptr_t>(d->b) & 15)) return svdx_fail(SVDX_E_BADARG, "tapgemm: operands must be 16 B aligned");
  if ((d->a_major_mn || d->b_major_mn) && (d->a_mode != SVDX_A_ROWS || d->num_taps != 1)) return svdx_fail(SVDX_E_BADARG, "tapgemm: MN-major operands only in single-tap ROWS mode");
  if (d->b_mode != 0 && !(d->a_major_mn && d->b_major_mn)) return svdx_fail(SVDX_E_BADARG, "tapgemm: b_mode needs MN-major A and B (weight-gradient form)");

  memset(&p, 0, sizeof(p));
  p.a_mode = d->a_mode; p.a_mn = d->a_major_mn; p.b_mn = d->b_major_mn;
  p.num_taps = d->num_taps;
  for (int i = 0; i < d->num_taps; ++i) { p.tap_d0[i] = d->tap_d0[i]; p.tap_d1[i] = d->tap_d1[i]; p.tap_d2[i] = d->tap_d2[i]; }
  const int block_n = kernel_block_n(d->block_n, d->b_major_mn || d->geglu);
  p.M = d->M; p.N = d->N; p.K = d->K; p.block_n = block_n; p.split_k = d->split_k;
  p.geglu = d->geglu;
  const int bn_out = d->geglu ? block_n / 2 : block_n;
  const int n_out = d->geglu ? d->N / 2 : d->N;
  p.n_tiles = (n_out + bn_out - 1) / bn_out;

  int rc;
  p.b_mode = d->b_mode;
  if (d->a_major_mn) {
    if (d->groups > 1 && d->b_mode != 2) return svdx_fail(SVDX_E_BADARG, "tapgemm: MN-major A requires groups==1");
    if (d->b_mode == 2) {
      uint64_t dims[3] = {(uint64_t)d->M, (uint64_t)d->rows_per_group, (uint64_t)d->groups};
      uint64_t strides[2] = {(uint64_t)d->lda * 2, (uint64_t)d->lda * 2 * (uint64_t)d->rows_per_group};
      uint32_t box[3] = {64, 64, 1};
      rc = svdx_make_tmap(&p.tma, d->a, 3, dims, strides, box);
    } else {
      uint64_t dims[2] = {(uint64_t)d->M, (uint64_t)d->K};
      uint64_t strides[1] = {(uint64_t)d->lda * 2};
      uint32_t box[2] = {64, 64};
      rc = svdx_make_tmap(&p.tma, d->a, 2, dims, strides, box);
    }
    p.rows_per_group = d->M; p.groups = 1; p.tiles_per_group = (d->M + BLOCK_M - 1) / BLOCK_M;
    p.m_tiles = p.tiles_per_group;
  } else if (d->a_mode == SVDX_A_ROWS) {
    if (d->rows_per_group <= 0 || d->groups <= 0 || (long long)d->rows_per_group * d->groups != d->M) return svdx_fail(SVDX_E_BADARG, "tapgemm: rows_per_group*groups != M");
    uint64_t dims[3] = {(uint64_t)d->K, (uint64_t)d->rows_per_group, (uint64_t)d->groups};
    uint64_t strides[2] = {(uint64_t)d->lda * 2, (uint64_t)d->lda * 2 * (uint64_t)d->rows_per_group};
    uint32_t box[3] = {64, 128, 1};
    rc = svdx_make_tmap(&p.tma, d->a, 3, dims, strides, box);
    p.rows_per_group = d->rows_per_group; p.groups = d->groups;
    p.tiles_per_group = (d->rows_per_group + BLOCK_M - 1) / BLOCK_M;
    p.m_tiles = p.tiles_per_group * d->groups;
  } else if (d->a_mode == SVDX_A_CONV2D) {
    const bool wide = d->W > 128;
    if (d->W <= 0 || d->H <= 0 || d->nimg <= 0) return svdx_fail(SVDX_E_BADARG, "tapgemm: conv2d needs W, H, images > 0");
    const bool boxes = wide ? (d->W % 128 == 0) : (128 % d->W == 0);
    uint64_t dims[4] = {(uint64_t)d->K, (uint64_t)d->W, (uint64_t)d->H, (uint64_t)d->nimg};
    uint64_t strides[3] = {(uint64_t)d->lda * 2, (uint64_t)d->lda * 2 * d->W, (uint64_t)d->lda * 2 * d->W * d->H};
    uint32_t box[4] = {64, (uint32_t)(wide ? 128 : d->W), 1, 1};
    p.max_bh_log2 = 0;
    if (!boxes) {
      for (int i = 0; i < d->num_taps; ++i)
        if (d->tap_d0[i] < -1 || d->tap_d0[i] > 1 || d->tap_d1[i] < -1 || d->tap_d1[i] > 1)
          return svdx_fail(SVDX_E_BADARG, "tapgemm: conv2d at a width with neither W | 128 nor 128 | W needs taps with |dw|, |dh| <= 1");
      rc = svdx_make_tmap_im2col(&p.tma, d->a, dims, strides, BLOCK_M);
      p.im2col = 1;
    } else {
      rc = svdx_make_tmap(&p.tma, d->a, 4, dims, strides, box);
    }
    p.wtiles = (wide && boxes) ? d->W / 128 : 0;
    for (int lg = 1; lg <= 4 && !rc && !wide && boxes; ++lg) {
      const int bh = 1 << lg;
      if (bh * d->W > BLOCK_M || bh > d->H) break;
      uint32_t boxh[4] = {64, (uint32_t)d->W, (uint32_t)bh, 1};
      rc = svdx_make_tmap(&p.tma_bh[lg - 1], d->a, 4, dims, strides, boxh);
      p.max_bh_log2 = lg;
    }
    p.W = d->W; p.H = d->H; p.nimg = d->M / (d->H * d->W);
    if ((long long)p.nimg * d->H * d->W != d->M) return svdx_fail(SVDX_E_BADARG, "tapgemm: conv2d M must be images*H*W");
    p.m_tiles = (d->M + BLOCK_M - 1) / BLOCK_M;
    p.rows_per_group = d->M; p.groups = 1; p.tiles_per_group = p.m_tiles;
  } else {
    return svdx_fail(SVDX_E_BADARG, "tapgemm: a_mode");
  }
  if (rc) return rc;

  if (d->b_major_mn && d->b_mode == 1) {
    if (d->W <= 0 || d->H <= 0 || d->nimg <= 0) return svdx_fail(SVDX_E_BADARG, "tapgemm: b_mode 1 needs W, H, images > 0");
    uint64_t dims[4] = {(uint64_t)d->N, (uint64_t)d->W, (uint64_t)d->H, (uint64_t)d->nimg};
    uint64_t strides[3] = {(uint64_t)d->ldb * 2, (uint64_t)d->ldb * 2 * d->W, (uint64_t)d->ldb * 2 * d->W * d->H};
    uint32_t box[4] = {64, (uint32_t)(d->W >= 64 ? 64 : d->W), 1, 1};
    if ((d->W < 64 && 64 % d->W) || (d->W >= 64 && d->W % 64)) {
      if (d->tap_d0[0] < -1 || d->tap_d0[0] > 1 || d->tap_d1[0] < -1 || d->tap_d1[0] > 1)
        return svdx_fail(SVDX_E_BADARG, "tapgemm: b_mode 1 at a width with neither W | 64 nor 64 | W needs a tap with |dw|, |dh| <= 1");
      rc = svdx_make_tmap_im2col(&p.tmb, d->b, dims, strides, 64);
      p.im2col = 1;
    } else {
      rc = svdx_make_tmap(&p.tmb, d->b, 4, dims, strides, box);
    }
    p.W = d->W; p.H = d->H; p.nimg = d->K / (d->W * d->H);
    if ((long long)p.nimg * d->W * d->H != d->K) return svdx_fail(SVDX_E_BADARG, "tapgemm: b_mode 1 K must be images*H*W");
  } else if (d->b_major_mn && d->b_mode == 2) {
    if (d->rows_per_group <= 0 || d->groups <= 0 || (long long)d->rows_per_group * d->groups != d->K) return svdx_fail(SVDX_E_BADARG, "tapgemm: b_mode 2 rows_per_group*groups != K");
    uint64_t dims[3] = {(uint64_t)d->N, (uint64_t)d->rows_per_group, (uint64_t)d->groups};
    uint64_t strides[2] = {(uint64_t)d->ldb * 2, (uint64_t)d->ldb * 2 * (uint64_t)d->rows_per_group};
    uint32_t box[3] = {64, 64, 1};
    rc = svdx_make_tmap(&p.tmb, d->b, 3, dims, strides, box);
    p.rows_per_group = d->rows_per_group; p.groups = d->groups;
  } else if (d->b_major_mn) {
    uint64_t dims[2] = {(uint64_t)d->N, (uint64_t)d->K};
    uint64_t strides[1] = {(uint64_t)d->ldb * 2};
    uint32_t box[2] = {64, 64};
    rc = svdx_make_tmap(&p.tmb, d->b, 2, dims, strides, box);
  } else {
    uint64_t dims[2] = {(uint64_t)d->K * d->num_taps, (uint64_t)d->N};
    uint64_t strides[1] = {(uint64_t)d->ldb * 2};
    uint32_t box[2] = {64, (uint32_t)(d->geglu ? block_n / 2 : block_n)};
    rc = svdx_make_tmap(&p.tmb, d->b, 2, dims, strides, box);
  }
  if (rc) return rc;

  p.kb_per_tap = (d->K + BLOCK_K - 1) / BLOCK_K;
  p.kb_total = p.kb_per_tap * d->num_taps;
  p.kb_per_group = p.kb_per_tap;
  if (d->b_mode == 2) {
    p.kb_per_group = (d->rows_per_group + BLOCK_K - 1) / BLOCK_K;
    p.kb_per_tap = p.kb_per_group * d->groups;
    p.kb_total = p.kb_per_tap;
  }
  p.kb_per_split = (p.kb_total + d->split_k - 1) / d->split_k;
  p.split_k = (p.kb_total + p.kb_per_split - 1) / p.kb_per_split;

  p.out = d->out; p.ldo = d->ldo; p.out_dtype = d->out_dtype;
  p.bias = d->bias; p.rowbias = d->rowbias; p.rowbias_div = d->rowbias_div > 0 ? d->rowbias_div : 1; p.ldrb = d->ldrb;
  p.res1 = reinterpret_cast<const bf16*>(d->res1); p.ldr1 = d->ldr1;
  p.res2 = reinterpret_cast<const bf16*>(d->res2); p.ldr2 = d->ldr2;
  p.scales = d->scales; p.pre = reinterpret_cast<bf16*>(d->pre); p.ldpre = d->ldpre;
  p.gn_sum = d->gn_sum; p.gn_ld = d->gn_ld; p.gn_rows = d->gn_rows;
  p.gnb_x = reinterpret_cast<const bf16*>(d->gnb_x); p.gnb_ldx = d->gnb_ldx; p.gnb_c1 = d->gnb_x2 ? d->gnb_c1 : d->N;
  p.gnb_x2 = reinterpret_cast<const bf16*>(d->gnb_x2); p.gnb_ldx2 = d->gnb_ldx2;
  p.gnb_ab = d->gnb_ab; p.gnb_sum = d->gnb_sum; p.gnb_rows = d->gnb_rows; p.gnb_silu = d->gnb_silu;
  {
    static int probe = -1;
    if (probe < 0) { const char* e = getenv("SVDX_EPI_PROBE"); probe = e ? atoi(e) : 0; }
    p.probe = probe;
  }
  {
    static int use = -1;
    if (use < 0) { const char* e = getenv("SVDX_TMA_STORE"); use = e ? atoi(e) : 1; }
    const bool grouped = (d->a_mode == SVDX_A_ROWS && !d->a_major_mn);
    const uint64_t R = grouped ? (uint64_t)d->rows_per_group : (uint64_t)d->M;
    const uint64_t G = grouped ? (uint64_t)d->groups : 1;
    const bool f32 = d->out_dtype != SVDX_OUT_BF16;
    const int esz = f32 ? 4 : 2;
    bool ok = use != 0 && (d->ldo * esz) % 16 == 0 && (reinterpret_cast<uintptr_t>(d->out) & 15) == 0;
    if (d->geglu && d->pre && ((d->N / 2) % 32 || (d->ldpre % 8) || (reinterpret_cast<uintptr_t>(d->pre) & 15))) ok = false;
    if (ok) {
      uint64_t dims[3] = {(uint64_t)n_out, R, G};
      uint64_t strides[2] = {(uint64_t)d->ldo * esz, (uint64_t)d->ldo * esz * R};
      uint32_t box[3] = {32, 32, 1};
      rc = svdx_make_tmap_ex(&p.tmo, d->out, f32, f32 ? 128 : 64, 3, dims, strides, box);
      if (rc) return rc;
      if (d->geglu && d->pre) {
        uint64_t pdims[3] = {(uint64_t)d->N, R, G};
        uint64_t pstrides[2] = {(uint64_t)d->ldpre * 2, (uint64_t)d->ldpre * 2 * R};
        rc = svdx_make_tmap_ex(&p.tmpre, d->pre, 0, 64, 3, pdims, pstrides, box);
        if (rc) return rc;
      }
      p.tma_store = 1;
    }
    p.epi_mode = EPI_GENERIC;
    const bool vec_ok = (reinterpret_cast<uintptr_t>(d->bias) & 15) == 0
                        && (!d->rowbias || ((reinterpret_cast<uintptr_t>(d->rowbias) & 15) == 0 && d->ldrb % 4 == 0));
    const bool has_res = d->res1 || d->res2 || d->scales;
    if (p.tma_store && !f32 && n_out % 32 == 0 && vec_ok && !d->a_major_mn && !(d->b_major_mn && has_res) && !p.probe && use != 2)
      p.epi_mode = d->geglu ? EPI_GEGLU : has_res ? EPI_RES : EPI_FAST;
    const bool f32_plain = !d->bias && !d->rowbias && !d->res1 && !d->res2 && !d->geglu && !d->gn_sum && !d->gnb_sum && !d->interleave &&
                           d->act == SVDX_ACT_NONE;
    if (p.tma_store && f32 && f32_plain && !p.probe && use != 2) {
      uint32_t box16[3] = {32, 16, 1};
      uint64_t dims[3] = {(uint64_t)n_out, R, G};
      uint64_t strides[2] = {(uint64_t)d->ldo * 4, (uint64_t)d->ldo * 4 * R};
      rc = svdx_make_tmap_ex(&p.tmo16, d->out, 1, 128, 3, dims, strides, box16);
      if (rc) return rc;
      p.epi_mode = EPI_F32;
    }
  }
  if (p.split_k > 1 && (p.bias || p.rowbias || p.res1 || p.res2 || p.geglu)) return svdx_fail(SVDX_E_BADARG, "tapgemm: split_k with epilogue operands");
  if (p.gnb_sum) {
    if (p.epi_mode != EPI_FAST || p.gn_sum)
      return svdx_fail(SVDX_E_BADARG, "tapgemm: gnb_sum needs the plain bf16 TMA-store epilogue (no residual / scales / GEGLU / split-K / gn_sum)");
    if (!p.gnb_x || p.gnb_rows <= 0 || (p.gnb_silu && !p.gnb_ab) || (d->N & 1) || (p.gnb_ldx % 8) || (reinterpret_cast<uintptr_t>(p.gnb_x) & 15) ||
        (reinterpret_cast<uintptr_t>(p.gnb_sum) & 7) || (p.gnb_ab && (reinterpret_cast<uintptr_t>(p.gnb_ab) & 7)) ||
        (p.gnb_x2 && (p.gnb_c1 <= 0 || p.gnb_c1 >= d->N || p.gnb_c1 % 32 || (p.gnb_ldx2 % 8) || (reinterpret_cast<uintptr_t>(p.gnb_x2) & 15))))
      return svdx_fail(SVDX_E_BADARG, "tapgemm: gnb operands (x rows 16-byte aligned, gnb_rows > 0, scale/shift table for SiLU, concat split % 32)");
    p.epi_mode = EPI_FAST_GNB;
  }
  if (d->interleave) {
    if (d->a_mode != SVDX_A_CONV2D || d->a_major_mn || d->b_major_mn || (d->phase_h & ~1) || (d->phase_w & ~1))
      return svdx_fail(SVDX_E_BADARG, "tapgemm: interleave needs CONV2D mode and phases in {0, 1}");
    if (p.epi_mode != EPI_FAST || p.rowbias || p.split_k > 1 || p.gnb_sum)
      return svdx_fail(SVDX_E_BADARG, "tapgemm: interleave needs the plain bf16 TMA-store epilogue (bias only: no rowbias / residual / "
                                      "scales / GEGLU / split-K / gnb sums; N %% 32 == 0, aligned rows)");
    if (p.W < 32 && 32 % p.W)
      return svdx_fail(SVDX_E_BADARG, "tapgemm: interleave with W < 32 needs W | 32 (a store chunk is whole image rows)");
    if (p.W < 32 && (p.H * p.W) % 32)
      return svdx_fail(SVDX_E_BADARG, "tapgemm: interleave with W < 32 needs H*W %% 32 == 0 (a store chunk must not straddle images)");
    const uint64_t rb = (uint64_t)d->ldo * 2;
    uint64_t dims[4] = {(uint64_t)n_out, (uint64_t)p.W, (uint64_t)p.H, (uint64_t)p.nimg};
    uint64_t strides[3] = {2 * rb, 4 * (uint64_t)p.W * rb, 4 * (uint64_t)p.W * p.H * rb};
    uint32_t box[4] = {32, (uint32_t)(p.W < 32 ? p.W : 32), (uint32_t)(p.W < 32 ? 32 / p.W : 1), 1};
    const bf16* base = reinterpret_cast<const bf16*>(d->out) + (2LL * p.W * d->phase_h + d->phase_w) * d->ldo;
    rc = svdx_make_tmap_ex(&p.tmo, base, 0, 64, 4, dims, strides, box);
    if (rc) return rc;
    p.il_out = const_cast<bf16*>(base);
    p.interleave = 1;
    p.epi_mode = EPI_FAST_IL;
  }
  if (d->act != SVDX_ACT_NONE) {
    if (d->act != SVDX_ACT_GELU && d->act != SVDX_ACT_QUICK_GELU) return svdx_fail(SVDX_E_BADARG, "tapgemm: act must be SVDX_ACT_GELU or SVDX_ACT_QUICK_GELU");
    if (p.epi_mode != EPI_FAST || p.rowbias || p.split_k > 1 || p.gn_sum)
      return svdx_fail(SVDX_E_BADARG, "tapgemm: act needs the plain bf16 TMA-store epilogue (bias only: no rowbias / residual / scales / "
                                      "GEGLU / split-K / gn_sum / gnb sums / interleave; N %% 32 == 0, aligned rows)");
    p.act = d->act;
    p.epi_mode = EPI_FAST_ACT;
  }
  if (d->b_major_mn && p.epi_mode != EPI_GENERIC && p.epi_mode != EPI_F32 && (p.epi_mode != EPI_FAST || p.gn_sum))
    return svdx_fail(SVDX_E_BADARG, "tapgemm: MN-major B takes the plain epilogue only (no gn_sum / gnb sums / act)");
  if (wide320 && p.epi_mode != EPI_FAST && p.epi_mode != EPI_RES && p.epi_mode != EPI_FAST_GNB && p.epi_mode != EPI_FAST_IL && p.epi_mode != EPI_FAST_ACT)
    return svdx_fail(SVDX_E_BADARG, "tapgemm: block_n 320 needs a bf16 output through the TMA-store epilogues (N % 320 == 0, aligned rows)");
  if (p.gn_sum) {
    if (p.epi_mode != EPI_FAST && p.epi_mode != EPI_RES && p.epi_mode != EPI_FAST_IL)
      return svdx_fail(SVDX_E_BADARG, "tapgemm: gn_sum needs a bf16 output through the TMA-store epilogues (N % 32 == 0, aligned rows), no split-K / GEGLU");
    if (p.gn_rows <= 0 || p.gn_ld < n_out || (p.gn_ld & 1) || (reinterpret_cast<uintptr_t>(p.gn_sum) & 7))
      return svdx_fail(SVDX_E_BADARG, "tapgemm: gn_sum needs gn_rows > 0, even gn_ld >= N, 8-byte aligned buffer");
  }
  if (d->out_dtype == SVDX_OUT_BF16 && ((d->ldo % 8) || (reinterpret_cast<uintptr_t>(d->out) & 15))) return svdx_fail(SVDX_E_BADARG, "tapgemm: out alignment");
  if (d->out_dtype != SVDX_OUT_BF16 && ((d->ldo % 4) || (reinterpret_cast<uintptr_t>(d->out) & 15))) return svdx_fail(SVDX_E_BADARG, "tapgemm: out alignment");
  if (d->res1 && ((d->ldr1 % 8) || (reinterpret_cast<uintptr_t>(d->res1) & 15))) return svdx_fail(SVDX_E_BADARG, "tapgemm: res1 alignment");
  if (d->res2 && ((d->ldr2 % 8) || (reinterpret_cast<uintptr_t>(d->res2) & 15))) return svdx_fail(SVDX_E_BADARG, "tapgemm: res2 alignment");
  if (d->pre && ((d->ldpre % 8) || (reinterpret_cast<uintptr_t>(d->pre) & 15))) return svdx_fail(SVDX_E_BADARG, "tapgemm: pre alignment");

  return SVDX_OK;
}

static constexpr int kernel_smem(int epi) { return epi == EPI_GENERIC ? smem_bytes(STAGES_PARKED, true) : smem_bytes(STAGES_REGS, false); }

template <int EPI>
static cudaError_t set_smem() {
  return cudaFuncSetAttribute(tapgemm_kernel<EPI>, cudaFuncAttributeMaxDynamicSharedMemorySize, kernel_smem(EPI));
}
template <int EPI>
static void launch(int grid, cudaStream_t stream, const TapGemmKParams& p) {
  tapgemm_kernel<EPI><<<grid, NUM_THREADS, kernel_smem(EPI), stream>>>(p);
}

extern "C" int svdx_tapgemm(const SvdxTapGemm* d, void* stream_v) {
  cudaStream_t stream = reinterpret_cast<cudaStream_t>(stream_v);
  TapGemmKParams p;
  int rc = svdx_tapgemm_fill(d, p);
  if (rc) return rc;
  static bool attr_done[SVDX_MAX_DEVICES] = {false};
  const int slot = svdx_device_slot();
  if (!attr_done[slot]) {
    cudaError_t e = set_smem<EPI_GENERIC>();
    if (e == cudaSuccess) e = set_smem<EPI_FAST>();
    if (e == cudaSuccess) e = set_smem<EPI_GEGLU>();
    if (e == cudaSuccess) e = set_smem<EPI_RES>();
    if (e == cudaSuccess) e = set_smem<EPI_FAST_GN>();
    if (e == cudaSuccess) e = set_smem<EPI_RES_GN>();
    if (e == cudaSuccess) e = set_smem<EPI_FAST_GNB>();
    if (e == cudaSuccess) e = set_smem<EPI_FAST_IL>();
    if (e == cudaSuccess) e = set_smem<EPI_FAST_IL_GN>();
    if (e == cudaSuccess) e = set_smem<EPI_FAST_ACT>();
    if (e == cudaSuccess) e = set_smem<EPI_F32>();
    if (e != cudaSuccess) return svdx_fail_cuda(e, "tapgemm: set smem attribute");
    attr_done[slot] = true;
  }
  const int total_tiles = p.m_tiles * p.n_tiles * p.split_k;
  int grid = svdx_num_sms();
  if (grid > total_tiles) grid = total_tiles;
  if (p.epi_mode == EPI_F32) launch<EPI_F32>(grid, stream, p);
  else if (p.epi_mode == EPI_FAST_ACT) launch<EPI_FAST_ACT>(grid, stream, p);
  else if (p.epi_mode == EPI_FAST_IL && p.gn_sum) launch<EPI_FAST_IL_GN>(grid, stream, p);
  else if (p.epi_mode == EPI_FAST_IL) launch<EPI_FAST_IL>(grid, stream, p);
  else if (p.epi_mode == EPI_FAST_GNB) launch<EPI_FAST_GNB>(grid, stream, p);
  else if (p.epi_mode == EPI_FAST && p.gn_sum) launch<EPI_FAST_GN>(grid, stream, p);
  else if (p.epi_mode == EPI_RES && p.gn_sum) launch<EPI_RES_GN>(grid, stream, p);
  else if (p.epi_mode == EPI_FAST) launch<EPI_FAST>(grid, stream, p);
  else if (p.epi_mode == EPI_GEGLU) launch<EPI_GEGLU>(grid, stream, p);
  else if (p.epi_mode == EPI_RES) launch<EPI_RES>(grid, stream, p);
  else launch<EPI_GENERIC>(grid, stream, p);
  cudaError_t e = cudaGetLastError();
  if (e != cudaSuccess) return svdx_fail_cuda(e, "tapgemm: launch");
  return SVDX_OK;
}
```

svd_xtend_b200/csrc/tapgemm_common.cuh:

```cuda
#pragma once
#include "common.cuh"
#include "../../include/svd_xtend_b200.h"
#include "host_util.h"

namespace svdx {

constexpr int BLOCK_M = 128;
constexpr int BLOCK_K = 64;
constexpr int MAX_BN = 160;
constexpr int A_STAGE_BYTES = BLOCK_M * BLOCK_K * 2;
constexpr int B_STAGE_BYTES = MAX_BN * BLOCK_K * 2;
constexpr int NUM_EPI_WARPS = 8;
constexpr int PRODUCER_WARP = NUM_EPI_WARPS;
constexpr int NUM_THREADS = 32 * NUM_EPI_WARPS + 32;
constexpr int ACC_LD = MAX_BN + 4;
constexpr int ACC_BYTES = BLOCK_M * ACC_LD * 4;
constexpr int EPI_STAGE_BYTES = 4096;
constexpr int STAGES_PARKED = 3;
constexpr int STAGES_REGS = 5;
constexpr int smem_bytes(int stages, bool parked) {
  return 1024 + stages * (A_STAGE_BYTES + B_STAGE_BYTES) + (parked ? ACC_BYTES : 0) + NUM_EPI_WARPS * EPI_STAGE_BYTES + 256;
}
static_assert(smem_bytes(STAGES_PARKED, true) <= 227 * 1024, "tapgemm shared memory exceeds the 227 KB a block may use");
static_assert(smem_bytes(STAGES_REGS, false) <= 227 * 1024, "tapgemm shared memory exceeds the 227 KB a block may use");
static_assert(16 * STAGES_REGS <= 256, "ring barriers must fit their 256-byte region");
static_assert((ACC_BYTES % 1024) == 0 && (B_STAGE_BYTES % 1024) == 0, "staging buffers must stay 1024-byte aligned");

struct __align__(64) TapGemmKParams {
  CUtensorMap tma;
  CUtensorMap tmb;
  CUtensorMap tma_bh[4];
  int max_bh_log2;
  int a_mode, a_mn, b_mn, b_mode, kb_per_group;
  int rows_per_group, groups, tiles_per_group;
  int W, H, nimg;
  int wtiles;
  int im2col;
  int num_taps;
  int tap_d0[SVDX_MAX_TAPS], tap_d1[SVDX_MAX_TAPS], tap_d2[SVDX_MAX_TAPS];
  int M, N, K;
  int block_n, m_tiles, n_tiles, split_k, kb_total, kb_per_split, kb_per_tap;
  void* out;
  long long ldo;
  int out_dtype, geglu;
  const float* bias;
  const float* rowbias;
  int rowbias_div;
  long long ldrb;
  const bf16* res1;
  long long ldr1;
  const bf16* res2;
  long long ldr2;
  const float* scales;
  bf16* pre;
  long long ldpre;
  CUtensorMap tmo;
  CUtensorMap tmo16;
  CUtensorMap tmpre;
  float* gn_sum;
  long long gn_ld;
  int gn_rows;
  const bf16* gnb_x;
  long long gnb_ldx;
  const bf16* gnb_x2;
  long long gnb_ldx2;
  int gnb_c1;
  const float* gnb_ab;
  float* gnb_sum;
  int gnb_rows, gnb_silu;
  int tma_store;
  int epi_mode;
  int probe;
  int interleave;
  int act;
  bf16* il_out;
};


SVDX_DEVINL void acc_ld32(uint32_t row, int col, uint32_t (&r)[32]) {
  const uint32_t a = row + col * 4;
#pragma unroll
  for (int k = 0; k < 8; ++k)
    asm volatile("ld.shared.v4.b32 {%0, %1, %2, %3}, [%4];" : "=r"(r[4 * k]), "=r"(r[4 * k + 1]), "=r"(r[4 * k + 2]), "=r"(r[4 * k + 3])
                 : "r"(a + 16 * k));
}

SVDX_DEVINL void tile_row(const TapGemmKParams& p, int mt, int r, long long& m, bool& row_ok) {
  if (p.a_mode == SVDX_A_ROWS && !p.a_mn) {
    const int g = mt / p.tiles_per_group;
    const int t = mt - g * p.tiles_per_group;
    const int rin = t * BLOCK_M + r;
    row_ok = rin < p.rows_per_group;
    m = (long long)g * p.rows_per_group + rin;
  } else {
    m = (long long)mt * BLOCK_M + r;
    row_ok = m < p.M;
  }
}

struct ConvBox {
  int lg, hh, n;
  uint32_t dst_off;
  bool nvalid, active;
};
SVDX_DEVINL void conv_tile_boxes(const TapGemmKParams& p, int t, int lane, ConvBox& mine) {
  const int R = BLOCK_M / p.W;
  int rowid = t * R, left = R, idx = 0;
  uint32_t off = 0;
  mine.active = false; mine.lg = 0; mine.hh = 0; mine.n = 0; mine.dst_off = 0; mine.nvalid = false;
  while (left > 0) {
    const int n = rowid / p.H;
    const int h = rowid - n * p.H;
    int run = min(left, p.H - h);
    int hh = h;
    while (run > 0) {
      const int lg = min(p.max_bh_log2, 31 - __clz(run));
      const int bh = 1 << lg;
      if (idx == lane) { mine.lg = lg; mine.hh = hh; mine.n = n; mine.nvalid = n < p.nimg; mine.dst_off = off; mine.active = true; }
      off += bh * p.W * 128;
      hh += bh; run -= bh; left -= bh; rowid += bh; ++idx;
    }
  }
}

struct EpiStage {
  uint32_t base;
  uint32_t off;
  int row0, grp;
};

SVDX_DEVINL void stage_store_bf16(const CUtensorMap* tm, EpiStage& st, int lane, const float (&f)[32], int col) {
  if (lane == 0) bulk_wait_read<1>();
  __syncwarp();
  const uint32_t buf = st.base + st.off;
  const uint32_t row = buf + lane * 64;
  const int sw = (lane >> 1) & 3;
#pragma unroll
  for (int j = 0; j < 4; ++j)
    st_shared_v4(row + ((j ^ sw) << 4), pack_bf16x2(f[8 * j], f[8 * j + 1]), pack_bf16x2(f[8 * j + 2], f[8 * j + 3]),
                 pack_bf16x2(f[8 * j + 4], f[8 * j + 5]), pack_bf16x2(f[8 * j + 6], f[8 * j + 7]));
  fence_proxy_async_smem();
  __syncwarp();
  if (lane == 0) { tma_store_3d(tm, buf, col, st.row0, st.grp); bulk_commit(); }
  st.off ^= 2048;
}

SVDX_DEVINL void stage_store_f32(const CUtensorMap* tm, EpiStage& st, int lane, const float (&f)[32], int col, bool reduce) {
  if (lane == 0) bulk_wait_read<0>();
  __syncwarp();
  const uint32_t row = st.base + lane * 128;
  const int sw = lane & 7;
#pragma unroll
  for (int j = 0; j < 8; ++j)
    st_shared_v4(row + ((j ^ sw) << 4), __float_as_uint(f[4 * j]), __float_as_uint(f[4 * j + 1]), __float_as_uint(f[4 * j + 2]),
                 __float_as_uint(f[4 * j + 3]));
  fence_proxy_async_smem();
  __syncwarp();
  if (lane == 0) {
    if (reduce) tma_reduce_add_3d(tm, st.base, col, st.row0, st.grp);
    else tma_store_3d(tm, st.base, col, st.row0, st.grp);
    bulk_commit();
  }
}

SVDX_DEVINL void gn_chunk_sums(const TapGemmKParams& p, uint32_t buf, int lane, int col0, int n_out_total, long long m0, int valid_rows) {
  const int pr = lane & 15, h = lane >> 4;
  const uint32_t in_chunk = (uint32_t)(pr & 3) * 4u;
  const int jch = pr >> 2;
  long long slab = m0 / p.gn_rows;
  int left = p.gn_rows - (int)(m0 - slab * p.gn_rows);
  int r = 0;
  while (r < valid_rows) {
    const int seg_end = min(valid_rows, r + left);
    float s0 = 0.f, s1 = 0.f, q0 = 0.f, q1 = 0.f;
    for (int rr = r + ((h ^ r) & 1); rr < seg_end; rr += 2) {
      uint32_t w;
      asm volatile("ld.shared.u32 %0, [%1];" : "=r"(w) : "r"(buf + rr * 64 + ((uint32_t)(jch ^ ((rr >> 1) & 3)) << 4) + in_chunk));
      const float2 v = unpack_bf16x2(w);
      s0 += v.x; s1 += v.y;
      q0 = fmaf(v.x, v.x, q0); q1 = fmaf(v.y, v.y, q1);
    }
    s0 += __shfl_xor_sync(0xffffffffu, s0, 16); s1 += __shfl_xor_sync(0xffffffffu, s1, 16);
    q0 += __shfl_xor_sync(0xffffffffu, q0, 16); q1 += __shfl_xor_sync(0xffffffffu, q1, 16);
    const int col = col0 + 2 * pr;
    if (h == 0 && col < n_out_total) {
      float* d = p.gn_sum + (2 * slab) * p.gn_ld + col;
      asm volatile("red.global.add.v2.f32 [%0], {%1, %2};" ::"l"(d), "f"(s0), "f"(s1) : "memory");
      asm volatile("red.global.add.v2.f32 [%0], {%1, %2};" ::"l"(d + p.gn_ld), "f"(q0), "f"(q1) : "memory");
    }
    r = seg_end; ++slab; left = p.gn_rows;
  }
}

constexpr int EPI_GENERIC = 0, EPI_FAST = 1, EPI_GEGLU = 2, EPI_RES = 3;
constexpr int EPI_FAST_GN = 4, EPI_RES_GN = 5;
constexpr int EPI_FAST_GNB = 6;
constexpr int EPI_FAST_IL = 7, EPI_FAST_IL_GN = 8;
constexpr int EPI_FAST_ACT = 9;
constexpr int EPI_F32 = 10;

template <int N>
SVDX_DEVINL void act_n(float (&f)[N], int act) {
  if (act == SVDX_ACT_GELU) {
#pragma unroll
    for (int i = 0; i < N; ++i) f[i] = gelu_erf_f(f[i]);
  } else {
#pragma unroll
    for (int i = 0; i < N; ++i) f[i] = __fdividef(f[i], 1.0f + __expf(-1.702f * f[i]));
  }
}

template <bool IL>
SVDX_DEVINL void store_chunk(const TapGemmKParams& p, uint32_t src, int col, int row0, int grp) {
  if constexpr (IL) {
    const int w0 = row0 % p.W, r = row0 / p.W;
    tma_store_4d(&p.tmo, src, col, w0, r % p.H, r / p.H);
  } else {
    tma_store_3d(&p.tmo, src, col, row0, grp);
  }
}

SVDX_DEVINL void il_store_next_row(const TapGemmKParams& p, uint32_t src, int col, int row0, int lane) {
  const int k = p.W - row0 % p.W;
  if (p.W < 32 || k >= 32 || lane < k || row0 + lane >= p.M) return;
  const long long orow = 4LL * p.W * (row0 / p.W + 1) + 2 * (lane - k);
  uint4* dst = reinterpret_cast<uint4*>(p.il_out + orow * p.ldo + col);
  const uint32_t row = src + lane * 64;
  const int sw = (lane >> 1) & 3;
#pragma unroll
  for (int j = 0; j < 4; ++j) {
    uint4 v;
    asm volatile("ld.shared.v4.b32 {%0, %1, %2, %3}, [%4];" : "=r"(v.x), "=r"(v.y), "=r"(v.z), "=r"(v.w) : "r"(row + ((j ^ sw) << 4)));
    dst[j] = v;
  }
}

SVDX_DEVINL void prefetch_rows_l2(const bf16* base, long long ld, long long m0, int valid_rows, int col0, int ncols, int lane, int half) {
  if (!base || lane >= valid_rows) return;
  const char* row = reinterpret_cast<const char*>(base + (m0 + lane) * ld + col0);
  const int bytes = ncols * 2;
  for (int b = half * 128; b < bytes; b += 256) asm volatile("prefetch.global.L2 [%0];" ::"l"(row + b));
}
SVDX_DEVINL void prefetch_epilogue_operands(const TapGemmKParams& p, int epi, long long m0, int valid_rows, int n0, int bn_out, int n_out_total,
                                            int lane, int half) {
  const int ncols = min(bn_out, n_out_total - n0);
  if (ncols <= 0) return;
  if (epi == EPI_RES || epi == EPI_RES_GN) {
    prefetch_rows_l2(p.res1, p.ldr1, m0, valid_rows, n0, ncols, lane, half);
    prefetch_rows_l2(p.res2, p.ldr2, m0, valid_rows, n0, ncols, lane, half);
  } else if (epi == EPI_FAST_GNB) {
    if (n0 < p.gnb_c1) prefetch_rows_l2(p.gnb_x, p.gnb_ldx, m0, valid_rows, n0, min(ncols, p.gnb_c1 - n0), lane, half);
    if (n0 + ncols > p.gnb_c1) {
      const int c0 = max(n0, p.gnb_c1);
      prefetch_rows_l2(p.gnb_x2, p.gnb_ldx2, m0, valid_rows, c0 - p.gnb_c1, n0 + ncols - c0, lane, half);
    }
  }
}

template <int ROWS = 32>
SVDX_DEVINL void gnb_chunk_sums(const TapGemmKParams& p, uint32_t buf_dy, uint32_t buf_x, int lane, int col0, int n_out_total, long long m0,
                                int valid_rows) {
  const int pr = lane & 15, h = lane >> 4;
  const uint32_t in_chunk = (uint32_t)(pr & 3) * 4u;
  const int jch = pr >> 2;
  long long slab = m0 / p.gnb_rows;
  int left = p.gnb_rows - (int)(m0 - slab * p.gnb_rows);
  const int col = col0 + 2 * pr;
  const bool col_ok = col < n_out_total;
  int r = 0;
  while (r < valid_rows) {
    const int seg_end = min(valid_rows, r + left);
    float2 A = make_float2(0.f, 0.f), B = make_float2(0.f, 0.f);
    if (col_ok && p.gnb_silu) {
      A = *reinterpret_cast<const float2*>(p.gnb_ab + (2 * slab) * p.N + col);
      B = *reinterpret_cast<const float2*>(p.gnb_ab + (2 * slab + 1) * p.N + col);
    }
    float s0 = 0.f, s1 = 0.f, x0 = 0.f, x1 = 0.f;
    if (r == 0 && seg_end == ROWS) {
#pragma unroll
      for (int b = 0; b < ROWS / 16; ++b) {
        uint32_t wd[8], wx[8];
#pragma unroll
        for (int i = 0; i < 8; ++i) {
          const int rr = h + 2 * (8 * b + i);
          const uint32_t off = rr * 64 + ((uint32_t)(jch ^ ((rr >> 1) & 3)) << 4) + in_chunk;
          asm volatile("ld.shared.u32 %0, [%1];" : "=r"(wd[i]) : "r"(buf_dy + off));
          asm volatile("ld.shared.u32 %0, [%1];" : "=r"(wx[i]) : "r"(buf_x + off));
        }
        float e0[8], e1[8];
#pragma unroll
        for (int i = 0; i < 8; ++i) {
          const float2 d = unpack_bf16x2(wd[i]), xv = unpack_bf16x2(wx[i]);
          e0[i] = d.x; e1[i] = d.y;
          if (p.gnb_silu) {
            e0[i] *= silu_grad_f(fmaf(xv.x, A.x, B.x));
            e1[i] *= silu_grad_f(fmaf(xv.y, A.y, B.y));
          }
        }
#pragma unroll
        for (int i = 0; i < 8; ++i) {
          const float2 xv = unpack_bf16x2(wx[i]);
          s0 += e0[i]; s1 += e1[i];
          x0 = fmaf(e0[i], xv.x, x0); x1 = fmaf(e1[i], xv.y, x1);
        }
      }
    } else {
      for (int rr = r + ((h ^ r) & 1); rr < seg_end; rr += 2) {
        const uint32_t off = rr * 64 + ((uint32_t)(jch ^ ((rr >> 1) & 3)) << 4) + in_chunk;
        uint32_t wd, wx;
        asm volatile("ld.shared.u32 %0, [%1];" : "=r"(wd) : "r"(buf_dy + off));
        asm volatile("ld.shared.u32 %0, [%1];" : "=r"(wx) : "r"(buf_x + off));
        const float2 d = unpack_bf16x2(wd), xv = unpack_bf16x2(wx);
        float e0 = d.x, e1 = d.y;
        if (p.gnb_silu) {
          e0 *= silu_grad_f(fmaf(xv.x, A.x, B.x));
          e1 *= silu_grad_f(fmaf(xv.y, A.y, B.y));
        }
        s0 += e0; s1 += e1;
        x0 = fmaf(e0, xv.x, x0); x1 = fmaf(e1, xv.y, x1);
      }
    }
    s0 += __shfl_xor_sync(0xffffffffu, s0, 16); s1 += __shfl_xor_sync(0xffffffffu, s1, 16);
    x0 += __shfl_xor_sync(0xffffffffu, x0, 16); x1 += __shfl_xor_sync(0xffffffffu, x1, 16);
    if (h == 0 && col_ok) {
      float* d = p.gnb_sum + (2 * slab) * p.N + col;
      asm volatile("red.global.add.v2.f32 [%0], {%1, %2};" ::"l"(d), "f"(s0), "f"(s1) : "memory");
      asm volatile("red.global.add.v2.f32 [%0], {%1, %2};" ::"l"(d + p.N), "f"(x0), "f"(x1) : "memory");
    }
    r = seg_end; ++slab; left = p.gnb_rows;
  }
}

struct PairStage {
  uint32_t slots;
  int bar;
  int sub;
  uint32_t round;
};
struct EpiTile {
  int n0, n_out_total, row0, grp, valid_rows;
  long long m0;
  long long m[2];
  bool ok[2];
};

SVDX_DEVINL uint32_t sw64(int r, int j) { return (uint32_t)(r * 64 + ((j ^ ((r >> 1) & 3)) << 4)); }
SVDX_DEVINL uint32_t frag_row_addr(uint32_t base16, int lane, int x) {
  const int mi = lane >> 3;
  return base16 + sw64(8 * (mi & 1) + (lane & 7), 2 * x + (mi >> 1));
}
SVDX_DEVINL void stmatrix_x4(uint32_t addr, uint32_t a, uint32_t b, uint32_t c, uint32_t d) {
  asm volatile("stmatrix.sync.aligned.m8n8.x4.shared.b16 [%0], {%1, %2, %3, %4};" ::"r"(addr), "r"(a), "r"(b), "r"(c), "r"(d) : "memory");
}
SVDX_DEVINL void ldmatrix_x4(uint32_t addr, uint32_t& a, uint32_t& b, uint32_t& c, uint32_t& d) {
  asm volatile("ldmatrix.sync.aligned.m8n8.x4.shared.b16 {%0, %1, %2, %3}, [%4];" : "=r"(a), "=r"(b), "=r"(c), "=r"(d) : "r"(addr) : "memory");
}
SVDX_DEVINL void stage_frag16(uint32_t base16, int lane, const float (&f)[16]) {
#pragma unroll
  for (int x = 0; x < 2; ++x)
    stmatrix_x4(frag_row_addr(base16, lane, x), pack_bf16x2(f[8 * x], f[8 * x + 1]), pack_bf16x2(f[8 * x + 2], f[8 * x + 3]),
                pack_bf16x2(f[8 * x + 4], f[8 * x + 5]), pack_bf16x2(f[8 * x + 6], f[8 * x + 7]));
}
SVDX_DEVINL void load_rows16(const bf16* base, long long ld, int nrows, int lane, uint4 (&v)[2]) {
#pragma unroll
  for (int j = 0; j < 2; ++j) {
    const int rr = (lane >> 2) + 8 * j;
    v[j] = rr < nrows ? *reinterpret_cast<const uint4*>(base + (long long)rr * ld + (lane & 3) * 8) : make_uint4(0u, 0u, 0u, 0u);
  }
}
SVDX_DEVINL void stage_rows16(uint32_t base16, int lane, const uint4 (&v)[2]) {
#pragma unroll
  for (int j = 0; j < 2; ++j) st_shared_v4(base16 + sw64((lane >> 2) + 8 * j, lane & 3), v[j].x, v[j].y, v[j].z, v[j].w);
}

template <int EPI, int BN>
SVDX_DEVINL void epilogue_regs(const TapGemmKParams& p, const float (&acc)[BN / 2], PairStage& ps, const EpiTile& t, int lane, float s_acc,
                               float s_r1, float s_r2) {
  constexpr bool GEGLU = EPI == EPI_GEGLU;
  constexpr bool RES = EPI == EPI_RES || EPI == EPI_RES_GN;
  constexpr bool GN = EPI == EPI_FAST_GN || EPI == EPI_RES_GN || EPI == EPI_FAST_IL_GN;
  constexpr bool IL = EPI == EPI_FAST_IL || EPI == EPI_FAST_IL_GN;
  constexpr bool GNB = EPI == EPI_FAST_GNB;
  constexpr int BN_OUT = GEGLU ? BN / 2 : BN;
  const int cq = 2 * (lane & 3);
  const bool issuer = ps.sub == 0 && lane == 0;
  const bool save_pre = GEGLU && p.pre != nullptr;
  const int vr = t.valid_rows - 16 * ps.sub;
  const long long mw = t.m0 + 16 * ps.sub;
  const float* bias = p.bias;
  const float* rb[2] = {nullptr, nullptr};
  const bf16* r2[2] = {nullptr, nullptr};
#pragma unroll
  for (int h = 0; h < 2; ++h) {
    if (!GEGLU && p.rowbias) rb[h] = p.rowbias + (t.ok[h] ? t.m[h] / p.rowbias_div : 0) * p.ldrb;
    if (RES && p.res2) r2[h] = p.res2 + (t.ok[h] ? t.m[h] : 0) * p.ldr2;
  }
#pragma unroll
  for (int ch = 0; ch < BN_OUT / 32; ++ch) {
    const int col0 = t.n0 + 32 * ch;
    if (col0 >= t.n_out_total) break;
    const uint32_t slot = ps.slots + 2048u * (GNB ? 2 * (ps.round & 1) : save_pre ? 2 : (ps.round & 3));
    const uint32_t mine = slot + 1024u * ps.sub;
    uint4 xa[2];
    if constexpr (RES) {
      if (p.res1) load_rows16(p.res1 + mw * p.ldr1 + col0, p.ldr1, vr, lane, xa);
    }
    if constexpr (GNB) {
      const bool src1 = col0 < p.gnb_c1;
      const long long xld = src1 ? p.gnb_ldx : p.gnb_ldx2;
      load_rows16((src1 ? p.gnb_x + col0 : p.gnb_x2 + (col0 - p.gnb_c1)) + mw * xld, xld, vr, lane, xa);
    }
    uint32_t a2[8];
    if constexpr (RES) {
      if (p.res2) {
#pragma unroll
        for (int k = 0; k < 8; ++k) a2[k] = *reinterpret_cast<const uint32_t*>(r2[k & 1] + col0 + 8 * (k >> 1) + cq);
      }
    }
    float f[16], g[16];
#pragma unroll
    for (int i = 0; i < 16; ++i) {
      f[i] = acc[16 * ch + i];
      if constexpr (GEGLU) g[i] = acc[BN_OUT / 2 + 16 * ch + i];
    }
    if (bias) {
#pragma unroll
      for (int j = 0; j < 4; ++j) {
        const float2 b = __ldg(reinterpret_cast<const float2*>(bias + col0 + 8 * j + cq));
        f[4 * j] += b.x; f[4 * j + 1] += b.y; f[4 * j + 2] += b.x; f[4 * j + 3] += b.y;
        if constexpr (GEGLU) {
          const float2 bg = __ldg(reinterpret_cast<const float2*>(bias + p.N / 2 + col0 + 8 * j + cq));
          g[4 * j] += bg.x; g[4 * j + 1] += bg.y; g[4 * j + 2] += bg.x; g[4 * j + 3] += bg.y;
        }
      }
    }
    if (!GEGLU && p.rowbias) {
#pragma unroll
      for (int k = 0; k < 8; ++k) {
        const float2 b = __ldg(reinterpret_cast<const float2*>(rb[k & 1] + col0 + 8 * (k >> 1) + cq));
        f[2 * k] += b.x; f[2 * k + 1] += b.y;
      }
    }
    if constexpr (EPI == EPI_FAST_ACT) act_n(f, p.act);
    if constexpr (RES) {
      if (p.scales) {
#pragma unroll
        for (int i = 0; i < 16; ++i) f[i] = __fmul_rn(f[i], s_acc);
      }
      if (p.res1) {
        uint32_t a1[8];
        stage_rows16(mine, lane, xa);
        __syncwarp();
        ldmatrix_x4(frag_row_addr(mine, lane, 0), a1[0], a1[1], a1[2], a1[3]);
        ldmatrix_x4(frag_row_addr(mine, lane, 1), a1[4], a1[5], a1[6], a1[7]);
        __syncwarp();
#pragma unroll
        for (int k = 0; k < 8; ++k) {
          const float2 a = unpack_bf16x2(a1[k]);
          f[2 * k] = __fmaf_rn(s_r1, a.x, f[2 * k]); f[2 * k + 1] = __fmaf_rn(s_r1, a.y, f[2 * k + 1]);
        }
      }
      if (p.res2) {
#pragma unroll
        for (int k = 0; k < 8; ++k) {
          const float2 a = unpack_bf16x2(a2[k]);
          f[2 * k] = __fmaf_rn(s_r2, a.x, f[2 * k]); f[2 * k + 1] = __fmaf_rn(s_r2, a.y, f[2 * k + 1]);
        }
      }
    }
    if constexpr (GEGLU) {
      if (save_pre) {
        stage_frag16(ps.slots + 1024u * ps.sub, lane, f);
        stage_frag16(ps.slots + 2048u + 1024u * ps.sub, lane, g);
        fence_proxy_async_smem();
        if (issuer) bulk_wait_read<0>();
        named_bar_sync(ps.bar, 64);
        if (issuer) {
          tma_store_3d(&p.tmpre, ps.slots, col0, t.row0, t.grp);
          tma_store_3d(&p.tmpre, ps.slots + 2048u, p.N / 2 + col0, t.row0, t.grp);
          bulk_commit();
        }
      }
#pragma unroll
      for (int i = 0; i < 16; ++i) {
        const float fv = __bfloat162float(__float2bfloat16(f[i]));
        const float gv = __bfloat162float(__float2bfloat16(g[i]));
        f[i] = fv * gelu_erf_f(gv);
      }
    }
    stage_frag16(mine, lane, f);
    if constexpr (GNB) stage_rows16(mine + 2048u, lane, xa);
    fence_proxy_async_smem();
    if (issuer) {
      if (GNB || save_pre) bulk_wait_read<0>();
      else bulk_wait_read<2>();
    }
    named_bar_sync(ps.bar, 64);
    if (issuer) { store_chunk<IL>(p, slot, col0, t.row0, t.grp); bulk_commit(); }
    if constexpr (IL) {
      if ((ps.round & 1) == (uint32_t)ps.sub) il_store_next_row(p, slot, col0, t.row0, lane);
    }
    if constexpr (GN) gn_chunk_sums(p, mine, lane, col0, t.n_out_total, mw, max(0, min(16, vr)));
    if constexpr (GNB) gnb_chunk_sums<16>(p, mine, mine + 2048u, lane, col0, t.n_out_total, mw, max(0, min(16, vr)));
    ++ps.round;
  }
}

template <int BN>
SVDX_DEVINL void epilogue_f32(const TapGemmKParams& p, const float (&acc)[BN / 2], EpiStage& st, const EpiTile& t, int sub, int lane,
                              float s_acc) {
  const bool reduce = p.out_dtype == SVDX_OUT_F32_ATOMIC;
  const uint32_t row_off = (uint32_t)(lane >> 2) * 128u + 8u * (lane & 1);
  const int sw = lane >> 2, pc = (lane & 3) >> 1;
#pragma unroll
  for (int ch = 0; ch < BN / 32; ++ch) {
    const int col0 = t.n0 + 32 * ch;
    if (col0 >= t.n_out_total) break;
    if (lane == 0) bulk_wait_read<1>();
    __syncwarp();
    const uint32_t buf = st.base + st.off + row_off;
#pragma unroll
    for (int j = 0; j < 4; ++j) {
      const uint32_t a = buf + ((uint32_t)((2 * j + pc) ^ sw) << 4);
#pragma unroll
      for (int h = 0; h < 2; ++h) {
        float x = acc[16 * ch + 4 * j + 2 * h], y = acc[16 * ch + 4 * j + 2 * h + 1];
        if (p.scales) { x *= s_acc; y *= s_acc; }
        asm volatile("st.shared.v2.f32 [%0], {%1, %2};" ::"r"(a + h * 1024u), "f"(x), "f"(y) : "memory");
      }
    }
    fence_proxy_async_smem();
    __syncwarp();
    if (lane == 0) {
      const uint32_t src = st.base + st.off;
      if (reduce) tma_reduce_add_3d(&p.tmo16, src, col0, t.row0 + 16 * sub, t.grp);
      else tma_store_3d(&p.tmo16, src, col0, t.row0 + 16 * sub, t.grp);
      bulk_commit();
    }
    st.off ^= 2048;
  }
}

SVDX_DEVINL void epilogue_tile(const TapGemmKParams& p, uint32_t t_base, long long m, bool row_ok, int n0, int half, int bn_out,
                               int n_out_total, float s_acc, float s_r1, float s_r2, EpiStage& st, int lane) {
      if (p.probe == 2) return;
      const float* rb = (p.rowbias && row_ok) ? p.rowbias + (m / p.rowbias_div) * p.ldrb : nullptr;
      for (int c = half * 32; c < bn_out; c += 64) {
        uint32_t v[32];
        uint32_t gte[32];
        const int col0 = n0 + c;
        if (col0 >= n_out_total) break;
        const bool full_chunk = (col0 + 32 <= n_out_total);
        uint4 rr1[4], rr2[4];
        if (row_ok && full_chunk) {
          if (p.res1) {
            const uint4* r1p = reinterpret_cast<const uint4*>(p.res1 + m * p.ldr1 + col0);
#pragma unroll
            for (int k = 0; k < 4; ++k) rr1[k] = r1p[k];
          }
          if (p.res2) {
            const uint4* r2p = reinterpret_cast<const uint4*>(p.res2 + m * p.ldr2 + col0);
#pragma unroll
            for (int k = 0; k < 4; ++k) rr2[k] = r2p[k];
          }
        }
        __syncwarp();
        acc_ld32(t_base, c, v);
        if (p.geglu) acc_ld32(t_base, bn_out + c, gte);
        float f[32];
#pragma unroll
        for (int i = 0; i < 32; ++i) f[i] = __uint_as_float(v[i]);
        if (p.geglu) {
          float g[32];
#pragma unroll
          for (int i = 0; i < 32; ++i) g[i] = __uint_as_float(gte[i]);
          if (p.bias) {
            if (full_chunk && ((p.N / 2) & 3) == 0) {
              const float4* bv = reinterpret_cast<const float4*>(p.bias + col0);
              const float4* bg = reinterpret_cast<const float4*>(p.bias + p.N / 2 + col0);
#pragma unroll
              for (int k = 0; k < 8; ++k) {
                const float4 x4 = __ldg(bv + k), y4 = __ldg(bg + k);
                f[4 * k] += x4.x; f[4 * k + 1] += x4.y; f[4 * k + 2] += x4.z; f[4 * k + 3] += x4.w;
                g[4 * k] += y4.x; g[4 * k + 1] += y4.y; g[4 * k + 2] += y4.z; g[4 * k + 3] += y4.w;
              }
            } else {
#pragma unroll
              for (int i = 0; i < 32; ++i) {
                if (full_chunk || col0 + i < n_out_total) {
                  f[i] += __ldg(p.bias + col0 + i);
                  g[i] += __ldg(p.bias + p.N / 2 + col0 + i);
                }
              }
            }
          }
          if (p.pre) {
            if (p.tma_store) {
              stage_store_bf16(&p.tmpre, st, lane, f, col0);
              stage_store_bf16(&p.tmpre, st, lane, g, p.N / 2 + col0);
            } else if (row_ok) {
              bf16* pv = p.pre + m * p.ldpre + col0;
              bf16* pg = pv + p.N / 2;
              if (full_chunk) {
#pragma unroll
                for (int i = 0; i < 32; i += 8) {
                  uint4 a, b;
                  a.x = pack_bf16x2(f[i], f[i + 1]); a.y = pack_bf16x2(f[i + 2], f[i + 3]);
                  a.z = pack_bf16x2(f[i + 4], f[i + 5]); a.w = pack_bf16x2(f[i + 6], f[i + 7]);
                  b.x = pack_bf16x2(g[i], g[i + 1]); b.y = pack_bf16x2(g[i + 2], g[i + 3]);
                  b.z = pack_bf16x2(g[i + 4], g[i + 5]); b.w = pack_bf16x2(g[i + 6], g[i + 7]);
                  *reinterpret_cast<uint4*>(pv + i) = a;
                  *reinterpret_cast<uint4*>(pg + i) = b;
                }
              } else {
                for (int i = 0; i < 32; ++i)
                  if (col0 + i < n_out_total) { pv[i] = __float2bfloat16(f[i]); pg[i] = __float2bfloat16(g[i]); }
              }
            }
          }
#pragma unroll
          for (int i = 0; i < 32; ++i) {
            const float fv = __bfloat162float(__float2bfloat16(f[i]));
            const float gv = __bfloat162float(__float2bfloat16(g[i]));
            f[i] = fv * gelu_erf_f(gv);
          }
        } else {
          if (p.bias) {
            if (full_chunk) {
              const float4* bp = reinterpret_cast<const float4*>(p.bias + col0);
#pragma unroll
              for (int k = 0; k < 8; ++k) {
                const float4 b4 = __ldg(bp + k);
                f[4 * k] += b4.x; f[4 * k + 1] += b4.y; f[4 * k + 2] += b4.z; f[4 * k + 3] += b4.w;
              }
            } else {
              for (int i = 0; i < 32; ++i)
                if (col0 + i < n_out_total) f[i] += __ldg(p.bias + col0 + i);
            }
          }
        }
        if (rb) {
          if (full_chunk && (reinterpret_cast<uintptr_t>(rb + col0) & 15) == 0) {
            const float4* bp = reinterpret_cast<const float4*>(rb + col0);
#pragma unroll
            for (int k = 0; k < 8; ++k) {
              const float4 b4 = __ldg(bp + k);
              f[4 * k] += b4.x; f[4 * k + 1] += b4.y; f[4 * k + 2] += b4.z; f[4 * k + 3] += b4.w;
            }
          } else {
#pragma unroll
            for (int i = 0; i < 32; ++i)
// ... 89 lines not shown
```

svd_xtend_b200/engine.py:

```python
from __future__ import annotations

from typing import Callable, Dict, List, Optional, Sequence, Tuple

import torch

from . import raw
from .raw import A_CONV2D, A_ROWS, OUT_F32_ATOMIC, bf16

F32 = torch.float32


class Var:

    __slots__ = ("data", "grad", "needs_grad", "owned", "csum", "gnb", "gnb_sums")

    def __init__(self, data: torch.Tensor, needs_grad: bool = False):
        self.data = data
        self.grad: Optional[torch.Tensor] = None
        self.needs_grad = needs_grad
        self.owned = False
        self.csum = None
        self.gnb = None
        self.gnb_sums = None

    def take_grad(self) -> Optional[torch.Tensor]:
        g, self.grad, self.owned = self.grad, None, False
        return g

    @property
    def rows(self) -> int:
        return self.data.shape[0]

    @property
    def cols(self) -> int:
        return self.data.shape[1]


class Geom:

    __slots__ = ("B", "T", "H", "W")

    def __init__(self, B, T, H, W):
        self.B, self.T, self.H, self.W = B, T, H, W

    @property
    def HW(self):
        return self.H * self.W

    @property
    def M(self):
        return self.B * self.T * self.H * self.W

    def down(self):
        return Geom(self.B, self.T, self.H // 2, self.W // 2)

    def up(self):
        return Geom(self.B, self.T, self.H * 2, self.W * 2)


CONV3x3_TAPS = tuple((kw - 1, kh - 1, 0) for kh in range(3) for kw in range(3))


def _neg_taps(taps):
    return tuple((-a, -b, -c) for a, b, c in taps)


def _copy_taps(dst: torch.Tensor, src: torch.Tensor, sel: Sequence[int]) -> None:
    for j, t in enumerate(sel):
        dst[:, j, :].copy_(src[:, t, :])


class WeightCache:

    def __init__(self):
        self._store: Dict[Tuple, Tuple[torch.Tensor, Tuple, Callable[[], None], bool]] = {}

    @staticmethod
    def _ver(params):
        return tuple((p._version, p.data_ptr()) for p in params)

    def get(self, key, params: Sequence[torch.Tensor], shape, build: Callable[[torch.Tensor], None], dtype=bf16):
        ent = self._store.get(key)
        ver = self._ver(params)
        if ent is None or ent[0].shape != torch.Size(shape) or ent[0].device != params[0].device:
            buf = torch.empty(shape, device=params[0].device, dtype=dtype)
            fn = lambda buf=buf: build(buf)
            fn()
            self._store[key] = (buf, ver, fn, any(p.requires_grad for p in params))
            return buf
        if ent[1] != ver:
            ent[2]()
            self._store[key] = (ent[0], ver, ent[2], ent[3])
        return ent[0]

    def refresh_trainable(self):
        for key, (buf, ver, fn, trainable) in list(self._store.items()):
            if trainable:
                fn()

    def clear(self):
        self._store.clear()


class Engine:

    def __init__(self):
        self.wc = WeightCache()
        self.tape: List[Callable[[], None]] = []
        self.recording = False
        self.pgrads: Dict[torch.nn.Parameter, torch.Tensor] = {}
        self.launches = 0
        self.grad_views: Dict[torch.nn.Parameter, torch.Tensor] = {}
        self.arena = None
        self.keep: List[torch.Tensor] = []
        self._consts: Dict[Tuple, torch.Tensor] = {}
        self.grad_ready_hook: Optional[Callable[[List[torch.nn.Parameter]], None]] = None
        self._stat_arena: Optional[torch.Tensor] = None
        self._stat_ptr = 0

    def begin(self, recording: bool):
        self.tape = []
        self.recording = recording
        if self._stat_arena is not None:
            self._stat_arena.zero_()
        self._stat_ptr = 0

    STAT_ARENA_FLOATS = 8 << 20

    def stat_zeros(self, n: int, device) -> torch.Tensor:
        n_al = (n + 63) // 64 * 64
        if self._stat_arena is None or self._stat_arena.device != torch.device(device):
            self._stat_arena = torch.zeros(self.STAT_ARENA_FLOATS, device=device, dtype=F32)
            self._stat_ptr = 0
        if self._stat_ptr + n_al > self._stat_arena.numel():
            return torch.zeros(n, device=device, dtype=F32)
        t = self._stat_arena[self._stat_ptr:self._stat_ptr + n]
        self._stat_ptr += n_al
        return t

    def _gn_sink(self, gn_rows: Optional[int], M: int, N: int, K: int, ntaps: int, device, n_out: Optional[int] = None):
        if gn_rows is None or N % 32 or M % gn_rows:
            return None
        if raw.split_plan(True, M, N, K, ntaps) is not None:
            return None
        return self.stat_zeros((M // gn_rows) * 2 * N, device).view(M // gn_rows, 2, N)

    def _gnb_for(self, x: Var, M: int, N: int, K: int, ntaps: int, scales, device):
        ctx = x.gnb
        if ctx is None or scales is not None or x.grad is not None or N % 32 or M % ctx["rows"] or N != ctx["C"] or M <= 8:
            return None
        if raw.split_plan(True, M, N, K, ntaps) is not None:
            return None
        sums = self.stat_zeros((M // ctx["rows"]) * 2 * N, device).view(M // ctx["rows"], 2, N)
        return dict(x=ctx["x"], x2=ctx["x2"], ab=ctx["ab"], rows=ctx["rows"], silu=ctx["silu"], sum=sums)

    def detach_tape(self) -> List[Callable[[], None]]:
        tape, self.tape = self.tape, []
        self.recording = False
        return tape

    def record(self, fn: Callable[[], None]):
        if self.recording:
            self.tape.append(fn)

    def run_backward(self, tape: Optional[List[Callable[[], None]]] = None):
        if tape is None:
            tape, self.tape = self.tape, []
        self.pgrads = {}
        was, self.recording = self.recording, True
        try:
            while tape:
                tape.pop()()
        finally:
            self.recording = was
        self.keep.clear()

    def checkpoint(self, fn: Callable[..., Var], *inputs: Var) -> Var:
        if not self.recording:
            return fn(*inputs)
        self.recording = False
        try:
            out = fn(*inputs)
        finally:
            self.recording = True
        if not out.needs_grad:
            return out

        def bwd():
            dy = out.take_grad()
            if dy is None:
                return
            outer, self.tape = self.tape, []
            ins2 = [Var(v.data, v.needs_grad) for v in inputs]
            out2 = fn(*ins2)
            self.add_grad(out2, dy, owned=False)
            sub, self.tape = self.tape, outer
            while sub:
                sub.pop()()
            for v, v2 in zip(inputs, ins2):
                g = v2.take_grad()
                if g is not None:
                    self.add_grad(v, g)
        self.record(bwd)
        return out

    def add_grad(self, v: Var, g: torch.Tensor, owned: bool = True):
        if not v.needs_grad:
            return
        v.gnb_sums = None
        if v.grad is None:
            v.grad, v.owned = g, owned
        elif v.grad.dtype != bf16:
            v.grad = v.grad + g
            v.owned = True
        elif v.owned:
            raw.axpby(v.grad, g, v.grad)
        else:
            out = torch.empty_like(v.grad)
            raw.axpby(v.grad, g, out)
            v.grad, v.owned = out, True

    def pgrad(self, p: torch.nn.Parameter) -> torch.Tensor:
        g = self.pgrads.get(p)
        if g is None:
            g = self.grad_views.get(p)
            if g is None:
                g = torch.zeros(p.shape, device=p.device, dtype=F32)
            self.pgrads[p] = g
        return g

    def w_lin(self, p: torch.Tensor, transposed: bool) -> torch.Tensor:
        if self.arena is not None and p.dim() == 2:
            m = self.arena.transposed_matrix([p]) if transposed else self.arena.shadow_matrix([p])
            if m is not None:
                return m
        O, I = p.shape[0], p[0].numel()
        src = lambda: p.detach().reshape(O, I)
        if transposed:
            return self.wc.get(("linT", id(p)), [p], (I, O), lambda buf: raw.prep_weight(src(), buf, 1, O, I))
        return self.wc.get(("lin", id(p)), [p], (O, I), lambda buf: raw.prep_weight(src(), buf, 0, O, I))

    def w_lin_cat(self, ps: Sequence[torch.Tensor], transposed: bool) -> torch.Tensor:
        if self.arena is not None:
            m = self.arena.transposed_matrix(list(ps)) if transposed else self.arena.shadow_matrix(list(ps))
            if m is not None:
                return m
        I = ps[0].shape[1]
        Os = [p.shape[0] for p in ps]
        key = ("catT" if transposed else "cat",) + tuple(id(p) for p in ps)
        if transposed:
            def build(buf):
                tmp = torch.empty(sum(Os), I, device=buf.device, dtype=bf16)
                o0 = 0
                for p, O in zip(ps, Os):
                    raw.prep_weight(p.detach(), tmp[o0:o0 + O], 0, O, I)
                    o0 += O
                raw.prep_weight(tmp, buf, 1, sum(Os), I)
            return self.wc.get(key, list(ps), (I, sum(Os)), build)

        def build(buf):
            o0 = 0
            for p, O in zip(ps, Os):
                raw.prep_weight(p.detach(), buf[o0:o0 + O], 0, O, I)
                o0 += O
        return self.wc.get(key, list(ps), (sum(Os), I), build)

    def w_conv(self, p: torch.Tensor, transposed: bool, i_pad: Optional[int] = None) -> torch.Tensor:
        O, I = p.shape[0], p.shape[1]
        taps = p[0, 0].numel()
        if transposed:
            Op = (O + 7) // 8 * 8
            if Op != O:
                def build(buf):
                    w = p.detach()
                    wp = torch.zeros(Op, I, taps, device=w.device, dtype=w.dtype)
                    wp[:O] = w.reshape(O, I, taps)
                    raw.prep_weight(wp, buf, 3, Op, I, taps)
                return self.wc.get(("convT", id(p)), [p], (I, taps * Op), build)
            return self.wc.get(("convT", id(p)), [p], (I, taps * O), lambda buf: raw.prep_weight(p.detach(), buf, 3, O, I, taps))
        ip = i_pad if i_pad is not None else I
        return self.wc.get(("conv", id(p), ip), [p], (O, taps * ip), lambda buf: raw.prep_weight(p.detach(), buf, 2, O, I, taps, ip))

    def vec_f32(self, p: Optional[torch.Tensor]) -> Optional[torch.Tensor]:
        if p is None:
            return None
        if p.dtype == F32:
            return p.detach()
        return self.wc.get(("f32", id(p)), [p], tuple(p.shape), lambda buf: raw.cast_to_f32(p.detach().contiguous(), buf), dtype=F32)

    @staticmethod
    def empty(rows, cols, like: torch.Tensor, dtype=bf16):
        return torch.empty(rows, cols, device=like.device, dtype=dtype)

    def _bias_grad(self, bias_p, dy: torch.Tensor, scale: Optional[torch.Tensor] = None):
        if bias_p is None or not bias_p.requires_grad:
            return
        g = self.pgrad(bias_p)
        n = g.numel()
        if scale is None and dy.shape[1] == n:
            raw.colsum(dy, g, accumulate=True)
        else:
            tmp = torch.empty(dy.shape[1], device=dy.device, dtype=F32)
            raw.colsum(dy, tmp)
            g.add_(tmp[:n] if scale is None else tmp[:n] * scale)

    def _res_grad(self, r: Optional[Var], dy: torch.Tensor, scale: Optional[torch.Tensor]):
        if r is None or not r.needs_grad:
            return
        if scale is None:
            self.add_grad(r, dy, owned=False)
        else:
            self.add_grad(r, self._scaled(dy, scale))

    def _rowbias_grad(self, rb: Optional[Var], dy: torch.Tensor, div: int, scale: Optional[torch.Tensor]):
        if rb is None or not rb.needs_grad:
            return
        nb = rb.rows
        g = torch.empty(nb, dy.shape[1], device=dy.device, dtype=F32)
        for b in range(nb):
            raw.colsum(dy[b * div:(b + 1) * div], g[b])
        if scale is not None:
            g = g * scale
        self.add_grad(rb, g)

    def linear(self, x: Var, weight, bias=None, *, res1: Optional[Var] = None, res2: Optional[Var] = None,
               scales: Optional[torch.Tensor] = None, res1_unit: bool = False, geglu: bool = False,
               rowbias: Optional[Var] = None, rowbias_div: int = 1, out_f32: bool = False,
               fused: Optional[Sequence] = None, blend=None, lora: Optional[Sequence] = None, gn_rows: Optional[int] = None) -> Var:
        ws = list(fused) if fused is not None else [weight]
        wf = self.w_lin_cat(ws, False) if fused is not None else self.w_lin(weight, False)
        N, K = wf.shape
        M = x.rows
        n_out = N // 2 if geglu else N
        out = self.empty(M, n_out, x.data, F32 if out_f32 else bf16)
        pre = self.empty(M, N, x.data) if (geglu and self.recording) else None
        b32 = self.vec_f32(bias)
        lora = [l for l in (lora or []) if l is not None]
        sink = None if (geglu or out_f32 or lora) else self._gn_sink(gn_rows, M, N, K, 1, out.device)
        raw.tapgemm_auto(x.data, wf, out, M=M, N=N, K=K, bias=b32, res1=None if res1 is None else res1.data,
                         res2=None if res2 is None else res2.data, scales=scales, geglu=geglu, pre=pre,
                         rowbias=None if rowbias is None else rowbias.data, rowbias_div=rowbias_div, gn_sum=sink, gn_rows=gn_rows or 0)
        lora_t = []
        for (off, n, A, Bm, sc) in lora:
            rp = (A.shape[0] + 7) // 8 * 8
            t = self.empty(M, rp, x.data)
            ov = out[:, off:off + n]
            if M <= 8:
                raw.gemv(x.data, self.w_lora(A, "A", False), t, M=M, N=rp, K=K)
                raw.gemv(t, self.w_lora(Bm, "B", False), ov, M=M, N=n, K=rp, scale=sc, accumulate=True)
            else:
                raw.tapgemm(x.data, self.w_lora(A, "A", False), t, M=M, N=rp, K=K)
                raw.tapgemm(t, self.w_lora(Bm, "B", False), ov, M=M, N=n, K=rp, res1=ov, scales=self._lora_scales(sc, out.device))
            lora_t.append(t)
        w_train = any(p.requires_grad for p in ws) or (bias is not None and bias.requires_grad) \
            or (blend is not None and blend[0].requires_grad) or any(l[2].requires_grad or l[3].requires_grad for l in lora)
        need = x.needs_grad or w_train or any(v is not None and v.needs_grad for v in (res1, res2, rowbias))
        y = Var(out, need)
        if sink is not None:
            y.csum = (gn_rows, [(sink, N)])
        if need and self.recording:
            def bwd():
                dy = y.take_grad()
                if dy is None:
                    return
                if dy.dtype != bf16:
                    dy = raw.cast_f32_bf16(dy.contiguous(), torch.empty(dy.shape, device=dy.device, dtype=bf16))
                s_acc = None if scales is None else scales[0:1]
                self._mix_grad(blend, dy, res1, out)
                self._res_grad(res1, dy, None if (scales is None or res1_unit) else scales[1:2])
                self._res_grad(res2, dy, None if scales is None else scales[2:3])
                bias_done = False
                if geglu:
                    fuse_b = bias is not None and bias.requires_grad and scales is None and self.pgrad(bias).numel() == pre.shape[1]
                    dyl = raw.geglu_bwd(pre, dy, torch.empty_like(pre), bias_grad=self.pgrad(bias) if fuse_b else None)
                    bias_done = fuse_b
                else:
                    dyl = dy
                self._rowbias_grad(rowbias, dyl, rowbias_div, s_acc)
                sc3 = self._acc_only(s_acc)
                if x.needs_grad:
                    wt = self.w_lin_cat(ws, True) if fused is not None else self.w_lin(weight, True)
                    dx = self.empty(M, K, x.data)
                    gnb = None if lora else self._gnb_for(x, M, K, N, 1, sc3, dyl.device)
                    raw.tapgemm_auto(dyl, wt, dx, M=M, N=K, K=N, scales=sc3, **({} if gnb is None else {"gnb": gnb}))
                    self.add_grad(x, dx)
                    if gnb is not None:
                        x.gnb_sums = (gnb["sum"], dx)
                if any(p.requires_grad for p in ws):
                    self._wgrad(dyl, x.data, ws, N, K, M, sc3)
                if bias is not None and bias.requires_grad and not bias_done:
                    self._bias_grad(bias, dyl, s_acc)
                for (off, n, A, Bm, sc), t in zip(lora, lora_t):
                    r = A.shape[0]
                    rp = (r + 7) // 8 * 8
                    dys = dyl[:, off:off + n]
                    s3 = self._lora_scales(sc, dyl.device, acc_only=True)
                    dt = self.empty(M, rp, x.data)
                    if M <= 8:
                        raw.gemv(dys, self.w_lora(Bm, "B", True), dt, M=M, N=rp, K=n, scale=sc)
                    else:
                        raw.tapgemm(dys, self.w_lora(Bm, "B", True), dt, M=M, N=rp, K=n, scales=s3)
                    if Bm.requires_grad:
                        self._wgrad(dys, t, [Bm], n, rp, M, s3, pad_to=(n, rp))
                    if A.requires_grad:
                        self._wgrad(dt, x.data, [A], rp, K, M, None, pad_to=(rp, K))
                    if x.needs_grad:
                        dxl = self.empty(M, K, x.data)
                        if M <= 8:
                            raw.gemv(dt, self.w_lora(A, "A", True), dxl, M=M, N=K, K=rp)
                        else:
                            raw.tapgemm(dt, self.w_lora(A, "A", True), dxl, M=M, N=K, K=rp)
                        self.add_grad(x, dxl)
            self.record(bwd)
        return y

    def _lora_scales(self, scale: float, device, acc_only: bool = False) -> torch.Tensor:
        key = ("lora_scale", float(scale), acc_only, str(device))
        t = self._consts.get(key)
        if t is None:
            t = torch.tensor([float(scale), 0.0 if acc_only else 1.0, 0.0], device=device, dtype=F32)
            self._consts[key] = t
        return t

    @staticmethod
    def _blend_base(view: torch.Tensor):
        base = view._base
        if base is not None and base.numel() == 16 and base.dtype == F32:
            return base, (view.data_ptr() - base.data_ptr()) // 4
        return None, 0

    def _acc_only(self, s3):
        if s3 is None:
            return None
        base, _ = self._blend_base(s3)
        if base is not None:
            return base[8:11]
        t = torch.zeros(3, device=s3.device, dtype=F32)
        t[0:1].copy_(s3[0:1])
        self.keep.append(t)
        return t

    def _scaled(self, t: torch.Tensor, s: torch.Tensor) -> torch.Tensor:
        out = torch.empty_like(t)
        base, off = self._blend_base(s)
        if base is not None and off in (1, 2):
            sc = base[12:14] if off == 1 else base[14:16]
        else:
            sc = torch.zeros(2, device=t.device, dtype=F32)
            sc[0:1].copy_(s)
            self.keep.append(sc)
        raw.axpby(t.reshape(-1), t.reshape(-1), out.reshape(-1), sc)
        return out

    def w_lora(self, p: torch.Tensor, which: str, transposed: bool) -> torch.Tensor:
        r = p.shape[0] if which == "A" else p.shape[1]
        rp = (r + 7) // 8 * 8
        if rp == r:
            return self.w_lin(p, transposed)
        O, I = p.shape
        Op, Ip = (rp, I) if which == "A" else (O, rp)
        shape = (Ip, Op) if transposed else (Op, Ip)

        def build(buf):
            buf.zero_()
            src = p.detach().t() if transposed else p.detach()
            buf[:src.shape[0], :src.shape[1]].copy_(src)
        return self.wc.get(("lora", id(p), transposed), [p], shape, build)

    def _wgrad(self, dy: torch.Tensor, x: torch.Tensor, ws, N, K, M, scales3, pad_to=None):
        if pad_to is not None and tuple(pad_to) != tuple(ws[0].shape):
            p = ws[0]
            if not p.requires_grad:
                return
            tmp = torch.zeros(pad_to, device=dy.device, dtype=F32)
            bn = raw.choose_block_n(pad_to[0], pad_to[1], mn_major=True)
            raw.tapgemm(dy, x, tmp, M=pad_to[0], N=pad_to[1], K=M, a_mn=True, b_mn=True, split_k=1, out_dtype=OUT_F32_ATOMIC,
                        block_n=bn, lda=dy.stride(0), ldb=x.stride(0), scales=scales3)
            self.pgrad(p).add_(tmp[:p.shape[0], :p.shape[1]])
            return
        if M <= 8 and (pad_to is None or tuple(pad_to) == tuple(ws[0].shape)) and K % 4 == 0 and dy.shape[1] >= sum(p.shape[0] for p in ws):
            o0 = 0
            for p in ws:
                O = p.shape[0]
                if p.requires_grad:
                    raw.outer_accum(dy[:, o0:o0 + O], x, self.pgrad(p).view(O, -1), None if scales3 is None else scales3[0:1])
                o0 += O
            return
        fused_g = None
        if len(ws) > 1 and self.arena is not None and all(p.requires_grad for p in ws):
            fused_g = self.arena.grad_matrix(list(ws))
        if fused_g is not None:
            for p in ws:
                self.pgrads.setdefault(p, self.grad_views[p])
            targets = [(None, 0, N)]
        elif len(ws) == 1:
            targets = [(ws[0], 0, N)]
        else:
            targets, o0 = [], 0
            for p in ws:
                targets.append((p, o0, p.shape[0]))
                o0 += p.shape[0]
        for p, o0, O in targets:
            if p is not None and not p.requires_grad:
                continue
            g = fused_g if p is None else self.pgrad(p).view(O, -1)
            dyp = dy[:, o0:o0 + O]
            bn, split = raw.wgrad_plan(O, K, M)
            raw.tapgemm(dyp, x, g, M=O, N=K, K=M, a_mn=True, b_mn=True, split_k=split, out_dtype=OUT_F32_ATOMIC,
                        block_n=bn, lda=dy.stride(0), ldb=x.stride(0), scales=scales3)

    def _conv_wgrad(self, dy: torch.Tensor, x: torch.Tensor, w: torch.nn.Parameter, taps, *, b_mode: int, Opad: int, ip: int,
                    K: int, conv_whn=None, rows_per_group=None, groups=1, scales3=None):
        O, I = w.shape[0], w.shape[1]
        nt = len(taps)
        ws = torch.zeros(Opad, nt * ip, device=dy.device, dtype=F32)
        bn = raw.choose_block_n(Opad, ip, mn_major=True)
        tiles = ((Opad + 127) // 128) * ((ip + bn - 1) // bn)
        kb = (K + 63) // 64
        split = max(1, min(kb // 32, raw.num_sms() // max(tiles, 1)))
        for t, tap in enumerate(taps):
            raw.tapgemm(dy, x, ws[:, t * ip:(t + 1) * ip], M=Opad, N=ip, K=K, a_mn=True, b_mn=True, b_mode=b_mode, taps=(tap,),
                        conv_whn=conv_whn, rows_per_group=rows_per_group if rows_per_group is not None else K, groups=groups,
                        split_k=split, out_dtype=OUT_F32_ATOMIC, block_n=bn, lda=dy.stride(0), ldb=x.stride(0), ldo=nt * ip,
                        scales=scales3)
        raw.unprep_conv_grad(ws, self.pgrad(w).view(O, I, nt), O, I, nt, ip)

    def _mix_grad(self, blend, dy: torch.Tensor, res1: Var, out: torch.Tensor):
        if blend is None or not blend[0].requires_grad:
            return
        mix, alpha = blend
        acc = torch.zeros(1, device=dy.device, dtype=F32)
        raw.dot_diff(dy.reshape(-1), res1.data.reshape(-1), out.reshape(-1), acc)
        self.pgrad(mix).add_((acc * alpha).to(F32).view(mix.shape))

    def conv2d_3x3(self, x: Var, g: Geom, conv, *, rowbias: Optional[Var] = None, rowbias_div=1, res1: Optional[Var] = None,
                   scales=None, res1_unit: bool = False, i_pad=None, n_pad=None, planes: bool = False, gn_rows: Optional[int] = None,
                   planes_pad0: bool = False) -> Var:
        w = conv.weight
        O, I = w.shape[0], w.shape[1]
        ip = i_pad if i_pad is not None else I
# ... 309 lines not shown
```

svd_xtend_b200/raw.py:

```python
from __future__ import annotations

import ctypes as C
import functools
import math
import os
from typing import Optional, Sequence

import numpy as np
import torch

from . import _lib
from ._lib import ACT_GELU, ACT_NONE, ACT_QUICK_GELU, A_CONV2D, A_ROWS, OUT_BF16, OUT_F32, OUT_F32_ATOMIC, SvdxAttn, SvdxTapGemm, load

bf16 = torch.bfloat16

_DTYPE_CODE = {torch.float32: 0, torch.bfloat16: 1, torch.float16: 2}


def dtype_code(t: torch.Tensor, what: str) -> int:
    try:
        return _DTYPE_CODE[t.dtype]
    except KeyError:
        raise TypeError(f"svd_xtend_b200: {what} has dtype {t.dtype}; supported: float32, bfloat16, float16") from None

LAUNCHES = [0]
_KERNELS_PER_CALL = {"svdx_groupnorm_apply_fused": 1, "svdx_attention_bwd": 3, "svdx_adamw_graph": 2, "svdx_adamw_p2p": 2,
                     "svdx_adamw_graph_ema": 2, "svdx_adamw_p2p_ema": 2, "svdx_ema_multi": 2, "svdx_adamw8bit": 2,
                     "svdx_adamw8bit_ema": 2, "svdx_adamw_graph_mul": 2, "svdx_adamw_graph_ema_mul": 2, "svdx_adamw8bit_mul": 2,
                     "svdx_adamw8bit_ema_mul": 2, "svdx_adamw_p2p_mul": 2, "svdx_adamw_p2p_ema_mul": 2, "svdx_grad_sumsq": 2,
                     "svdx_grad_sumsq_p2p": 2}


def check(rc: int, what: str = "") -> None:
    LAUNCHES[0] += _KERNELS_PER_CALL.get(what, 1)
    _lib.check(rc, what)


ABLATE: set = set()
ACCOUNT = None
SHAPE_LOG = None


def _fam(family: str, flops: float = 0.0, nbytes: float = 0.0) -> bool:
    if ACCOUNT is not None:
        ACCOUNT(family, flops, nbytes)
    return family in ABLATE


def _stream() -> int:
    return torch.cuda.current_stream().cuda_stream


def _ptr(t: Optional[torch.Tensor]) -> Optional[int]:
    return None if t is None else t.data_ptr()


def _layout(t: torch.Tensor) -> dict:
    return dict(shape=list(t.shape), stride=list(t.stride()), dtype=str(t.dtype).replace("torch.", ""))


def _rowmajor(t: torch.Tensor, name: str) -> int:
    if t.stride(-1) != 1:
        raise ValueError(f"{name}: last dimension must be contiguous")
    return t.stride(-2)


def pick_block_n(n_out: int, mn_major: bool = False) -> int:
    if mn_major:
        for bn in (256, 192, 128, 64):
            if n_out % bn == 0:
                return bn
        return 256 if n_out > 256 else ((n_out + 63) // 64) * 64
    for bn in (256, 160, 128, 96, 64, 32):
        if n_out % bn == 0:
            return bn
    return 256 if n_out > 256 else ((n_out + 31) // 32) * 32


_NUM_SMS = [0]


def num_sms() -> int:
    if _NUM_SMS[0] == 0:
        _NUM_SMS[0] = int(load().svdx_num_sms())
    return _NUM_SMS[0]


_L2_BYTES_PER_CLK = 4500.0


def _tile_cost(M: int, n_out: int, bn_out: int, geglu: bool, sms: int) -> float:
    bn = 2 * bn_out if geglu else bn_out
    ctas = ((M + 127) // 128) * ((n_out + bn_out - 1) // bn_out)
    active = min(ctas, sms)
    mma = 4 * max(bn / 2.0, 32.0 + bn / 4.0)
    l2 = (16384 + 128 * bn) * active / _L2_BYTES_PER_CLK
    waves = (ctas + sms - 1) // sms
    return waves * max(mma, l2)


def choose_block_n(M: int, n_out: int, geglu: bool = False, mn_major: bool = False) -> int:
    sms = num_sms()
    if mn_major:
        best, best_cost = None, None
        m_tiles = (M + 127) // 128
        for bn in (128, 64):
            cost = m_tiles * ((n_out + bn - 1) // bn) * max(bn / 2.0, 32.0 + bn / 4.0)
            if best_cost is None or cost < best_cost - 1e-9:
                best, best_cost = bn, cost
        return best
    cands = [64, 32] if geglu else [160, 128, 96, 64, 32]
    best, best_cost = None, None
    for bn in cands:
        if n_out % bn and n_out > bn:
            continue
        cost = _tile_cost(M, n_out, bn, geglu, sms)
        if best_cost is None or cost < best_cost * 0.98:
            best, best_cost = bn, cost
    if best is None:
        best = pick_block_n(n_out, False)
    return 2 * best if geglu else best


WIDE_TILE = os.environ.get("SVDX_WIDE", "1") != "0"
WIDE_MIN_K = int(os.environ.get("SVDX_WIDE_MIN_K", "960"))


def _wide_tile_ok(M, N, k_total, out, ldo, geglu, a_mn, b_mn, b_mode, split_k, out_dtype, bias, rowbias) -> bool:
    if not WIDE_TILE or geglu or a_mn or b_mn or b_mode != 0 or split_k != 1 or N % 320 or N % 256 == 0 or M < 512 or k_total < WIDE_MIN_K:
        return False
    if out.dtype != bf16 or (out_dtype is not None and out_dtype != OUT_BF16):
        return False
    ld = ldo if ldo is not None else out.stride(0)
    if ld % 8 or out.data_ptr() % 16:
        return False
    if bias is not None and bias.data_ptr() % 16:
        return False
    if rowbias is not None and (rowbias.data_ptr() % 16 or rowbias.stride(0) % 4):
        return False
    return True


_WGRAD_SM_BYTES_PER_CLK = 34.0
_WGRAD_L2_BYTES_PER_CLK = 4500.0
_WGRAD_TILE_CLK = 4000.0
_WGRAD_SPLITS = (1, 2, 3, 4, 5, 6, 8, 10, 12, 14, 16, 20, 24, 32)


def wgrad_plan(O: int, K: int, M: int):
    return _wgrad_plan(O, K, M, num_sms())


@functools.lru_cache(maxsize=None)
def _wgrad_plan(O: int, K: int, M: int, sms: int):
    kb = (M + 63) // 64
    m_tiles = (O + 127) // 128
    best = None
    for bn in ((128, 64) if K > 64 else (64,)):
        n_tiles = (K + bn - 1) // bn
        tiles = m_tiles * n_tiles
        for split in _WGRAD_SPLITS:
            if split > 1 and (tiles * split > 4 * sms or kb // split < 4 or -(-kb // -(-kb // split)) != split):
                continue
            ctas = tiles * split
            active = min(ctas, sms)
            bytes_kb = 16384 + 128.0 * K / n_tiles
            per = max(4.0 * max(bn / 2.0, 32.0 + bn / 4.0), bytes_kb / _WGRAD_SM_BYTES_PER_CLK,
                      bytes_kb * active / _WGRAD_L2_BYTES_PER_CLK)
            waves = -(-ctas // sms)
            cost = waves * ((kb / split) * per + _WGRAD_TILE_CLK)
            if best is None or cost < best[0] * 0.97:
                best = (cost, bn, split)
    return best[1], best[2]


def tapgemm(
    a: torch.Tensor,
    b: torch.Tensor,
    out: torch.Tensor,
    *,
    M: int,
    N: int,
    K: int,
    mode: int = A_ROWS,
    taps: Sequence[Sequence[int]] = ((0, 0, 0),),
    rows_per_group: Optional[int] = None,
    groups: int = 1,
    conv_whn: Optional[Sequence[int]] = None,
    lda: Optional[int] = None,
    ldb: Optional[int] = None,
    ldo: Optional[int] = None,
    a_mn: bool = False,
    b_mn: bool = False,
    b_mode: int = 0,
    block_n: Optional[int] = None,
    split_k: int = 1,
    out_dtype: Optional[int] = None,
    geglu: bool = False,
    bias: Optional[torch.Tensor] = None,
    rowbias: Optional[torch.Tensor] = None,
    rowbias_div: int = 1,
    res1: Optional[torch.Tensor] = None,
    res2: Optional[torch.Tensor] = None,
    scales: Optional[torch.Tensor] = None,
    pre: Optional[torch.Tensor] = None,
    gn_sum: Optional[torch.Tensor] = None,
    gn_rows: int = 0,
    gnb: Optional[dict] = None,
    phase: Optional[Sequence[int]] = None,
    act: int = ACT_NONE,
) -> torch.Tensor:
    family = "conv" if (mode == A_CONV2D or len(taps) > 1 or b_mode != 0) else "linear"
    if _fam(family, 2.0 * M * N * K * len(taps)):
        return out
    if SHAPE_LOG is not None:
        SHAPE_LOG.append(dict(M=M, N=N, K=K, taps=len(taps), conv2d=int(mode == A_CONV2D), geglu=int(geglu), a_mn=int(a_mn), b_mode=b_mode,
                              split_k=split_k, block_n=block_n, f32out=int(out.dtype != bf16), bias=int(bias is not None),
                              rowbias=int(rowbias is not None), res=int(res1 is not None) + int(res2 is not None),
                              scales=int(scales is not None), pre=int(pre is not None),
                              launch=dict(M=M, N=N, K=K, mode=mode, taps=[[int(v) for v in t] for t in taps], rows_per_group=rows_per_group,
                                          groups=groups, conv_whn=None if conv_whn is None else [int(v) for v in conv_whn], lda=lda, ldb=ldb,
                                          ldo=ldo, a_mn=bool(a_mn), b_mn=bool(b_mn), b_mode=b_mode, block_n=block_n, split_k=split_k,
                                          out_dtype=out_dtype, geglu=bool(geglu), rowbias_div=rowbias_div, gn_rows=gn_rows,
                                          phase=None if phase is None else [int(v) for v in phase], act=int(act),
                                          gnb=None if gnb is None else dict(rows=int(gnb["rows"]), silu=bool(gnb["silu"])),
                                          tensors={k: _layout(t) for k, t in (
                                              ("a", a), ("b", b), ("out", out), ("bias", bias), ("rowbias", rowbias), ("res1", res1),
                                              ("res2", res2), ("scales", scales), ("pre", pre), ("gn_sum", gn_sum),
                                              ("gnb_x", None if gnb is None else gnb["x"]), ("gnb_x2", None if gnb is None else gnb.get("x2")),
                                              ("gnb_ab", None if gnb is None else gnb.get("ab")), ("gnb_sum", None if gnb is None else gnb["sum"]))
                                              if t is not None})))
    d = SvdxTapGemm()
    assert a.dtype == bf16 and b.dtype == bf16
    d.a = a.data_ptr()
    d.lda = lda if lda is not None else _rowmajor(a, "a")
    d.a_mode = mode
    d.a_major_mn = int(a_mn)
    d.rows_per_group = rows_per_group if rows_per_group is not None else M
    d.groups = groups
    if conv_whn is not None:
        d.W, d.H, d.nimg = conv_whn
    d.num_taps = len(taps)
    for i, t in enumerate(taps):
        d.tap_d0[i], d.tap_d1[i], d.tap_d2[i] = int(t[0]), int(t[1]), int(t[2])
    d.b = b.data_ptr()
    d.ldb = ldb if ldb is not None else _rowmajor(b, "b")
    d.b_major_mn = int(b_mn)
    d.b_mode = b_mode
    d.M, d.N, d.K = M, N, K
    n_out = N // 2 if geglu else N
    if block_n is None:
        block_n = choose_block_n(M, n_out, geglu, b_mn)
        if _wide_tile_ok(M, N, K * len(taps), out, ldo, geglu, a_mn, b_mn, b_mode, split_k, out_dtype, bias, rowbias):
            block_n = 320
    d.block_n = block_n
    d.split_k = split_k
    d.out = out.data_ptr()
    d.ldo = ldo if ldo is not None else _rowmajor(out, "out")
    if out_dtype is None:
        out_dtype = OUT_BF16 if out.dtype == bf16 else OUT_F32
    d.out_dtype = out_dtype
    d.geglu = int(geglu)
    if bias is not None:
        assert bias.dtype == torch.float32
        d.bias = bias.data_ptr()
    if rowbias is not None:
        assert rowbias.dtype == torch.float32
        d.rowbias = rowbias.data_ptr()
        d.rowbias_div = rowbias_div
        d.ldrb = _rowmajor(rowbias, "rowbias")
    if res1 is not None:
        assert res1.dtype == bf16
        d.res1 = res1.data_ptr()
        d.ldr1 = _rowmajor(res1, "res1")
    if res2 is not None:
        assert res2.dtype == bf16
        d.res2 = res2.data_ptr()
        d.ldr2 = _rowmajor(res2, "res2")
    if scales is not None:
        assert scales.dtype == torch.float32 and scales.numel() >= 3
        d.scales = scales.data_ptr()
    if pre is not None:
        assert pre.dtype == bf16
        d.pre = pre.data_ptr()
        d.ldpre = _rowmajor(pre, "pre")
    if gn_sum is not None:
        assert gn_sum.dtype == torch.float32 and gn_sum.dim() == 3 and gn_sum.shape[1] == 2 and gn_sum.is_contiguous() and gn_rows > 0
        d.gn_sum = gn_sum.data_ptr()
        d.gn_ld = gn_sum.shape[2]
        d.gn_rows = gn_rows
    if gnb is not None:
        gx, gx2 = gnb["x"], gnb.get("x2")
        assert gx.dtype == bf16 and gnb["sum"].dtype == torch.float32 and gnb["sum"].is_contiguous() and gnb["sum"].shape[-1] == N
        d.gnb_x = gx.data_ptr()
        d.gnb_ldx = _rowmajor(gx, "gnb x")
        if gx2 is not None:
            d.gnb_x2 = gx2.data_ptr()
            d.gnb_ldx2 = _rowmajor(gx2, "gnb x2")
            d.gnb_c1 = gx.shape[-1]
        d.gnb_ab = _ptr(gnb.get("ab"))
        d.gnb_sum = gnb["sum"].data_ptr()
        d.gnb_rows = gnb["rows"]
        d.gnb_silu = int(gnb["silu"])
    if phase is not None:
        d.interleave = 1
        d.phase_h, d.phase_w = int(phase[0]), int(phase[1])
    d.act = int(act)
    check(load().svdx_tapgemm(C.byref(d), _stream()), "svdx_tapgemm")
    return out


_SPLITK_WS: dict = {}


def _splitk_workspace(M: int, N: int, device) -> torch.Tensor:
    key = (M, N, str(device), _stream() if torch.device(device).type == "cuda" else 0)
    ws = _SPLITK_WS.get(key)
    if ws is None:
        ws = torch.zeros(M, N, device=device, dtype=torch.float32)
        _SPLITK_WS[key] = ws
    return ws


def split_plan(out_is_bf16: bool, M: int, N: int, K: int, ntaps: int = 1, geglu=False, a_mn=False, b_mn=False, block_n=None):
    if not (out_is_bf16 and not geglu and not a_mn and not b_mn and block_n is None and N % 8 == 0 and N >= 256):
        return None
    bn = 256 if N % 256 == 0 else (160 if N % 160 == 0 else 0)
    if not bn:
        return None
    kb = ((K + 63) // 64) * ntaps
    tiles = ((M + 127) // 128) * (N // bn)
    split = min(num_sms() // max(tiles, 1), kb // 8)
    if tiles <= num_sms() // 3 and split >= 2:
        return bn, split
    return None


def tapgemm_auto(a, b, out, *, M, N, K, taps=((0, 0, 0),), bias=None, rowbias=None, rowbias_div=1, res1=None, res2=None,
                 scales=None, gn_sum=None, gn_rows=0, **kw):
    kw = dict(kw)
    if kw.get("block_n") is None:
        kw.pop("block_n", None)
    if (M <= 8 and not kw.get("act") and len(taps) == 1 and kw.get("mode", A_ROWS) == A_ROWS and not kw.get("geglu") and not kw.get("a_mn") and not kw.get("b_mn")
            and rowbias is None and res1 is None and res2 is None and scales is None and gn_sum is None and kw.get("groups", 1) == 1
            and K % 8 == 0 and a.stride(-1) == 1 and b.stride(-1) == 1 and out.dtype in (bf16, torch.float32)):
        return gemv(a, b, out, M=M, N=N, K=K, bias=bias, lda=kw.get("lda"), ldw=kw.get("ldb"))
    plan = None if kw.get("act") else split_plan(out.dtype == bf16, M, N, K, len(taps), kw.get("geglu"), kw.get("a_mn"), kw.get("b_mn"),
                                                 kw.get("block_n"))
    if plan is not None:
        assert gn_sum is None, "fused GroupNorm statistics are not available on the split-K path"
        bn, split = plan
        ws = _splitk_workspace(M, N, out.device)
        tapgemm(a, b, ws, M=M, N=N, K=K, taps=taps, block_n=bn, split_k=split, out_dtype=OUT_F32_ATOMIC, **kw)
        if _fam("conv" if (kw.get("mode", A_ROWS) == A_CONV2D or len(taps) > 1) else "linear"):
            return out
        check(load().svdx_splitk_epilogue(ws.data_ptr(), N, out.data_ptr(), _rowmajor(out, "out"), M, N, _ptr(bias), _ptr(rowbias),
                                          rowbias_div, _rowmajor(rowbias, "rowbias") if rowbias is not None else 0,
                                          _ptr(res1), _rowmajor(res1, "res1") if res1 is not None else 0,
                                          _ptr(res2), _rowmajor(res2, "res2") if res2 is not None else 0,
                                          _ptr(scales), _stream()), "svdx_splitk_epilogue")
        return out
    return tapgemm(a, b, out, M=M, N=N, K=K, taps=taps, bias=bias, rowbias=rowbias, rowbias_div=rowbias_div, res1=res1, res2=res2,
                   scales=scales, gn_sum=gn_sum, gn_rows=gn_rows, **kw)


CONV3x3_TAPS = tuple((kw - 1, kh - 1, 0) for kh in range(3) for kw in range(3))


def _attn_desc(q, k, v, o, heads, S, nseq, inner, outer_stride, inner_stride, tok_stride, scale, lse):
    d = SvdxAttn()
    d.q, d.k, d.v, d.o = q.data_ptr(), k.data_ptr(), v.data_ptr(), o.data_ptr()
    d.ldq, d.ldk, d.ldv, d.ldo = _rowmajor(q, "q"), _rowmajor(k, "k"), _rowmajor(v, "v"), _rowmajor(o, "o")
    d.nseq, d.heads, d.S, d.inner = nseq, heads, S, inner
    d.outer_stride, d.inner_stride, d.tok_stride = outer_stride, inner_stride, tok_stride
    d.scale = scale
    d.lse = _ptr(lse)
    return d


def attention_fwd(q, k, v, o, *, heads, S, nseq, inner=1, outer_stride=None, inner_stride=0, tok_stride=1,
                  scale=0.125, lse=None):
    if outer_stride is None:
        outer_stride = S
    if _fam("attention", 4.0 * nseq * heads * S * S * 64):
        return o
    d = _attn_desc(q, k, v, o, heads, S, nseq, inner, outer_stride, inner_stride, tok_stride, scale, lse)
    check(load().svdx_attention_fwd(C.byref(d), _stream()), "svdx_attention_fwd")
    return o


def attention_bwd(q, k, v, o, dout, dq, dk, dv, lse, delta, *, heads, S, nseq, inner=1, outer_stride=None,
                  inner_stride=0, tok_stride=1, scale=0.125):
    if outer_stride is None:
        outer_stride = S
    if _fam("attention", 10.0 * nseq * heads * S * S * 64):
        return
    d = _attn_desc(q, k, v, o, heads, S, nseq, inner, outer_stride, inner_stride, tok_stride, scale, lse)
    d.dout, d.lddo = dout.data_ptr(), _rowmajor(dout, "dout")
    d.dq, d.dk, d.dv = dq.data_ptr(), dk.data_ptr(), dv.data_ptr()
    d.lddq, d.lddk, d.lddv = _rowmajor(dq, "dq"), _rowmajor(dk, "dk"), _rowmajor(dv, "dv")
    d.delta = delta.data_ptr()
    check(load().svdx_attention_bwd(C.byref(d), _stream()), "svdx_attention_bwd")


def attention_hd80_fwd(q, k, v, o, *, heads, S, nseq, scale):
    for t, n in ((q, "q"), (k, "k"), (v, "v"), (o, "o")):
        if t.dtype != bf16 or not t.is_cuda or t.shape[0] < nseq * S:
            raise ValueError(f"attention_hd80_fwd: {n} must be a CUDA bf16 [nseq*S, ld] matrix")
    if _fam("attention", 4.0 * nseq * heads * S * S * 80):
        return o
    check(load().svdx_attention_hd80_fwd(q.data_ptr(), _rowmajor(q, "q"), k.data_ptr(), _rowmajor(k, "k"), v.data_ptr(), _rowmajor(v, "v"),
                                         o.data_ptr(), _rowmajor(o, "o"), nseq, heads, S, float(scale), _stream()), "svdx_attention_hd80_fwd")
    return o


def groupnorm_sums(x, x2, outer, rows, sums=None):
    C1 = x.shape[-1]
    C2 = x2.shape[-1] if x2 is not None else 0
    if sums is None:
        sums = torch.zeros(outer, 2, C1 + C2, device=x.device, dtype=torch.float32)
    if _fam("groupnorm", 0.0, 2.0 * x.shape[0] * (C1 + C2)):
        return sums
    assert sums.dtype == torch.float32 and sums.dim() == 3 and sums.shape[:2] == (outer, 2) and sums.is_contiguous()
    check(load().svdx_groupnorm_sums(x.data_ptr(), _rowmajor(x, "x"), C1, _ptr(x2), _rowmajor(x2, "x2") if x2 is not None else 0, C2,
                                     outer, rows, sums.data_ptr(), sums.shape[2], _stream()), "svdx_groupnorm_sums")
    return sums


def groupnorm_apply_fused(x, x2, outer, rows, eps, csum1, csum2, gamma, beta, silu, y, groups=32, ab=None):
    C1 = x.shape[-1]
    C2 = x2.shape[-1] if x2 is not None else 0
    stats = torch.empty(2, outer * groups, device=x.device, dtype=torch.float32)
    mean, rstd = stats[0], stats[1]
    if _fam("groupnorm", 0.0, 4.0 * x.shape[0] * (C1 + C2)):
        return mean, rstd
    check(load().svdx_groupnorm_apply_fused(x.data_ptr(), _rowmajor(x, "x"), C1, _ptr(x2), _rowmajor(x2, "x2") if x2 is not None else 0, C2,
                                            outer, rows, groups, eps, csum1.data_ptr(), csum1.stride(1),
                                            _ptr(csum2), csum2.stride(1) if csum2 is not None else 0, mean.data_ptr(), rstd.data_ptr(),
                                            gamma.data_ptr(), beta.data_ptr(), int(silu), y.data_ptr(), _rowmajor(y, "y"), _ptr(ab), _stream()),
          "svdx_groupnorm_apply_fused")
    return mean, rstd


def groupnorm_bwd_sums(x, x2, dy, outer, rows, ab, silu, sums=None):
    C1 = x.shape[-1]
    C2 = x2.shape[-1] if x2 is not None else 0
    if sums is None:
        sums = torch.zeros(outer, 2, C1 + C2, device=x.device, dtype=torch.float32)
    if _fam("groupnorm", 0.0, 4.0 * x.shape[0] * (C1 + C2)):
        return sums
    assert sums.dtype == torch.float32 and sums.shape == (outer, 2, C1 + C2) and sums.is_contiguous()
    check(load().svdx_groupnorm_bwd_sums(x.data_ptr(), _rowmajor(x, "x"), C1, _ptr(x2), _rowmajor(x2, "x2") if x2 is not None else 0, C2,
                                         dy.data_ptr(), _rowmajor(dy, "dy"), outer, rows, _ptr(ab), int(silu), sums.data_ptr(), _stream()),
          "svdx_groupnorm_bwd_sums")
    return sums


def groupnorm_bwd_fused(x, x2, dy, outer, rows, mean, rstd, gamma, beta, silu, csum, dx, dx2, dgamma=None, dbeta=None, groups=32, dres=None):
    C1 = x.shape[-1]
    C2 = x2.shape[-1] if x2 is not None else 0
# ... 507 lines not shown
```

Baseline: 159.4.

## Fuse GEGLU backward into the down-projection dgrad GEMM epilogue

Adds a GEMM epilogue mode that, while computing the gradient flowing into a GEGLU output, loads the saved pre-activation, applies the GEGLU backward and writes both value and gate gradients directly. It also accumulates the GEGLU bias gradient via column sums. The engine defers the GEGLU backward to this fused path when the next layer's dgrad can produce it, which removes the intermediate dx tensor round trip and a separate elementwise kernel. In exchange the epilogue does more work per tile, writes twice as many output columns, and limits tile width to 128, which may cost some GEMM efficiency.

```diff
diff --git a/include/svd_xtend_b200.h b/include/svd_xtend_b200.h
--- a/include/svd_xtend_b200.h
+++ b/include/svd_xtend_b200.h
@@ -69,6 +69,9 @@
   int32_t interleave;
   int32_t phase_h, phase_w;
   int32_t act;
+  const void* geglu_pre;
+  int64_t geglu_ldpre;
+  float* geglu_bias_grad;
 } SvdxTapGemm;
 
 #define SVDX_ACT_NONE 0
diff --git a/svd_xtend_b200/_lib.py b/svd_xtend_b200/_lib.py
--- a/svd_xtend_b200/_lib.py
+++ b/svd_xtend_b200/_lib.py
@@ -35,6 +35,7 @@
         ("gnb_ab", c_void_p), ("gnb_sum", c_void_p), ("gnb_rows", c_int), ("gnb_silu", c_int),
         ("interleave", c_int), ("phase_h", c_int), ("phase_w", c_int),
         ("act", c_int),
+        ("geglu_pre", c_void_p), ("geglu_ldpre", c_i64), ("geglu_bias_grad", c_void_p),
     ]
 
 
diff --git a/svd_xtend_b200/csrc/common.cuh b/svd_xtend_b200/csrc/common.cuh
--- a/svd_xtend_b200/csrc/common.cuh
+++ b/svd_xtend_b200/csrc/common.cuh
@@ -184,6 +184,9 @@
   const float pdf = 0.3989422804014327f * exp2_fast(-0.72134752044448170f * x * x);
   return fmaf(x, pdf, normal_cdf_f(x));
 }
+SVDX_DEVINL float2 geglu_bwd_elem(float value, float gate, float d) {
+  return make_float2(__fmul_rn(d, gelu_erf_f(gate)), __fmul_rn(__fmul_rn(d, value), gelu_erf_grad_f(gate)));
+}
 
 SVDX_DEVINL uint32_t pack_bf16x2(float lo, float hi) {
   __nv_bfloat162 v = __floats2bfloat162_rn(lo, hi);
diff --git a/svd_xtend_b200/csrc/elementwise.cu b/svd_xtend_b200/csrc/elementwise.cu
--- a/svd_xtend_b200/csrc/elementwise.cu
+++ b/svd_xtend_b200/csrc/elementwise.cu
@@ -313,8 +313,9 @@
 #pragma unroll
   for (int k = 0; k < 4; ++k) {
     const float2 fv = unpack_bf16x2(v[k]), fg = unpack_bf16x2(g[k]), fd = unpack_bf16x2(d[k]);
-    ov[k] = pack_bf16x2(fd.x * gelu_erf_f(fg.x), fd.y * gelu_erf_f(fg.y));
-    og[k] = pack_bf16x2(fd.x * fv.x * gelu_erf_grad_f(fg.x), fd.y * fv.y * gelu_erf_grad_f(fg.y));
+    const float2 e0 = geglu_bwd_elem(fv.x, fg.x, fd.x), e1 = geglu_bwd_elem(fv.y, fg.y, fd.y);
+    ov[k] = pack_bf16x2(e0.x, e1.x);
+    og[k] = pack_bf16x2(e0.y, e1.y);
   }
   *reinterpret_cast<uint4*>(dpre + r * lddpre + c) = make_uint4(ov[0], ov[1], ov[2], ov[3]);
   *reinterpret_cast<uint4*>(dpre + r * lddpre + h + c) = make_uint4(og[0], og[1], og[2], og[3]);
@@ -350,8 +351,9 @@
 #pragma unroll
         for (int k = 0; k < 4; ++k) {
           const float2 fv = unpack_bf16x2(v[k]), fg = unpack_bf16x2(g[k]), fd = unpack_bf16x2(d[k]);
-          ov[k] = pack_bf16x2(fd.x * gelu_erf_f(fg.x), fd.y * gelu_erf_f(fg.y));
-          og[k] = pack_bf16x2(fd.x * fv.x * gelu_erf_grad_f(fg.x), fd.y * fv.y * gelu_erf_grad_f(fg.y));
+          const float2 e0 = geglu_bwd_elem(fv.x, fg.x, fd.x), e1 = geglu_bwd_elem(fv.y, fg.y, fd.y);
+          ov[k] = pack_bf16x2(e0.x, e1.x);
+          og[k] = pack_bf16x2(e0.y, e1.y);
           const float2 rv = unpack_bf16x2(ov[k]), rg = unpack_bf16x2(og[k]);
           av[2 * k] += rv.x; av[2 * k + 1] += rv.y;
           ag[2 * k] += rg.x; ag[2 * k + 1] += rg.y;
diff --git a/svd_xtend_b200/csrc/tapgemm.cu b/svd_xtend_b200/csrc/tapgemm.cu
--- a/svd_xtend_b200/csrc/tapgemm.cu
+++ b/svd_xtend_b200/csrc/tapgemm.cu
@@ -77,8 +77,10 @@
 SVDX_DEVINL void tile_regs_bn(const TapGemmKParams& p, int kb0, int kb1, Ring& rg, int wg, PairStage& ps, const EpiTile& t, int lane,
                               float s_acc, float s_r1, float s_r2) {
   float acc[BN / 2];
+  uint4 pa[2], pb[2];
+  if constexpr (EPI == EPI_GEGLU_BWD) gbw_load_chunk0(p, t, ps.sub, lane, pa, pb);
   tile_mainloop<BN, 0, TB, STAGES_REGS>(acc, kb0, kb1, rg, wg);
-  epilogue_regs<EPI, BN>(p, acc, ps, t, lane, s_acc, s_r1, s_r2);
+  epilogue_regs<EPI, BN>(p, acc, ps, t, lane, s_acc, s_r1, s_r2, pa, pb);
 }
 
 template <int EPI>
@@ -87,6 +89,13 @@
   if constexpr (EPI == EPI_GEGLU) {
     if (p.block_n == 64) tile_regs_bn<EPI, 64, 0>(p, kb0, kb1, rg, wg, ps, t, lane, s_acc, s_r1, s_r2);
     else tile_regs_bn<EPI, 128, 0>(p, kb0, kb1, rg, wg, ps, t, lane, s_acc, s_r1, s_r2);
+  } else if constexpr (EPI == EPI_GEGLU_BWD) {
+    switch (p.block_n) {
+      case 32: tile_regs_bn<EPI, 32, 0>(p, kb0, kb1, rg, wg, ps, t, lane, s_acc, s_r1, s_r2); break;
+      case 64: tile_regs_bn<EPI, 64, 0>(p, kb0, kb1, rg, wg, ps, t, lane, s_acc, s_r1, s_r2); break;
+      case 96: tile_regs_bn<EPI, 96, 0>(p, kb0, kb1, rg, wg, ps, t, lane, s_acc, s_r1, s_r2); break;
+      default: tile_regs_bn<EPI, 128, 0>(p, kb0, kb1, rg, wg, ps, t, lane, s_acc, s_r1, s_r2); break;
+    }
   } else {
     if constexpr (EPI == EPI_FAST) {
       if (p.b_mn) {
@@ -384,7 +393,7 @@
         m0 = st.row0;
         valid_rows = max(0, min(32, p.M - st.row0));
       }
-      if constexpr (EPI == EPI_RES || EPI == EPI_RES_GN || EPI == EPI_FAST_GNB)
+      if constexpr (EPI == EPI_RES || EPI == EPI_RES_GN || EPI == EPI_FAST_GNB || EPI == EPI_GEGLU_BWD)
         prefetch_epilogue_operands(p, EPI, m0, valid_rows, n0, bn_out, n_out_total, lane, half);
       if constexpr (PARKED) {
         named_bar_sync(1, 32 * NUM_EPI_WARPS);
@@ -611,7 +620,25 @@
       if (rc) return rc;
       p.epi_mode = EPI_F32;
     }
-  }
+    if (d->geglu_pre) {
+      if ((p.epi_mode != EPI_FAST && p.epi_mode != EPI_RES) || d->res1 || d->res2 || d->bias || d->rowbias || d->geglu || d->gn_sum ||
+          d->gnb_sum || d->interleave || d->act != SVDX_ACT_NONE || d->split_k != 1 || d->b_major_mn || block_n > 128 || wide320)
+        return svdx_fail(SVDX_E_BADARG, "tapgemm: geglu_pre needs the bf16 TMA-store epilogue (scales only: no bias / row-bias / residuals / "
+                                        "GEGLU / gn_sum / gnb sums / interleave / act / split-K / MN-major B; tiles at most 128 wide; N %% 32 == 0, aligned rows)");
+      if ((d->M > 1 && (d->ldo < 2LL * d->N || d->geglu_ldpre < 2LL * d->N)) || (d->geglu_ldpre % 8) ||
+          (reinterpret_cast<uintptr_t>(d->geglu_pre) & 15) || (reinterpret_cast<uintptr_t>(d->geglu_bias_grad) & 7))
+        return svdx_fail(SVDX_E_BADARG, "tapgemm: geglu_pre needs ldo, geglu_ldpre >= 2N, geglu_ldpre %% 8 == 0, 16-byte aligned pre, 8-byte aligned bias gradient");
+      uint64_t dims[3] = {2 * (uint64_t)n_out, R, G};
+      uint64_t strides[2] = {(uint64_t)d->ldo * 2, (uint64_t)d->ldo * 2 * R};
+      uint32_t box[3] = {32, 32, 1};
+      rc = svdx_make_tmap_ex(&p.tmo, d->out, 0, 64, 3, dims, strides, box);
+      if (rc) return rc;
+      p.gpre = reinterpret_cast<const bf16*>(d->geglu_pre); p.ldgpre = d->geglu_ldpre; p.gbias = d->geglu_bias_grad;
+      p.epi_mode = EPI_GEGLU_BWD;
+    }
+  }
+  if (d->geglu_pre && p.epi_mode != EPI_GEGLU_BWD)
+    return svdx_fail(SVDX_E_BADARG, "tapgemm: geglu_pre needs a bf16 output through the TMA-store epilogue (N % 32 == 0, aligned rows)");
   if (p.split_k > 1 && (p.bias || p.rowbias || p.res1 || p.res2 || p.geglu)) return svdx_fail(SVDX_E_BADARG, "tapgemm: split_k with epilogue operands");
   if (p.gnb_sum) {
     if (p.epi_mode != EPI_FAST || p.gn_sum)
@@ -700,6 +727,7 @@
     if (e == cudaSuccess) e = set_smem<EPI_FAST_IL_GN>();
     if (e == cudaSuccess) e = set_smem<EPI_FAST_ACT>();
     if (e == cudaSuccess) e = set_smem<EPI_F32>();
+    if (e == cudaSuccess) e = set_smem<EPI_GEGLU_BWD>();
     if (e != cudaSuccess) return svdx_fail_cuda(e, "tapgemm: set smem attribute");
     attr_done[slot] = true;
   }
@@ -707,6 +735,7 @@
   int grid = svdx_num_sms();
   if (grid > total_tiles) grid = total_tiles;
   if (p.epi_mode == EPI_F32) launch<EPI_F32>(grid, stream, p);
+  else if (p.epi_mode == EPI_GEGLU_BWD) launch<EPI_GEGLU_BWD>(grid, stream, p);
   else if (p.epi_mode == EPI_FAST_ACT) launch<EPI_FAST_ACT>(grid, stream, p);
   else if (p.epi_mode == EPI_FAST_IL && p.gn_sum) launch<EPI_FAST_IL_GN>(grid, stream, p);
   else if (p.epi_mode == EPI_FAST_IL) launch<EPI_FAST_IL>(grid, stream, p);
diff --git a/svd_xtend_b200/csrc/tapgemm_common.cuh b/svd_xtend_b200/csrc/tapgemm_common.cuh
--- a/svd_xtend_b200/csrc/tapgemm_common.cuh
+++ b/svd_xtend_b200/csrc/tapgemm_common.cuh
@@ -74,6 +74,9 @@
   int interleave;
   int act;
   bf16* il_out;
+  const bf16* gpre;
+  long long ldgpre;
+  float* gbias;
 };
 
 
@@ -198,6 +201,7 @@
 constexpr int EPI_FAST_IL = 7, EPI_FAST_IL_GN = 8;
 constexpr int EPI_FAST_ACT = 9;
 constexpr int EPI_F32 = 10;
+constexpr int EPI_GEGLU_BWD = 11;
 
 template <int N>
 SVDX_DEVINL void act_n(float (&f)[N], int act) {
@@ -248,6 +252,9 @@
   if (epi == EPI_RES || epi == EPI_RES_GN) {
     prefetch_rows_l2(p.res1, p.ldr1, m0, valid_rows, n0, ncols, lane, half);
     prefetch_rows_l2(p.res2, p.ldr2, m0, valid_rows, n0, ncols, lane, half);
+  } else if (epi == EPI_GEGLU_BWD) {
+    prefetch_rows_l2(p.gpre, p.ldgpre, m0, valid_rows, n0, ncols, lane, half);
+    prefetch_rows_l2(p.gpre + p.N, p.ldgpre, m0, valid_rows, n0, ncols, lane, half);
   } else if (epi == EPI_FAST_GNB) {
     if (n0 < p.gnb_c1) prefetch_rows_l2(p.gnb_x, p.gnb_ldx, m0, valid_rows, n0, min(ncols, p.gnb_c1 - n0), lane, half);
     if (n0 + ncols > p.gnb_c1) {
@@ -331,6 +338,21 @@
   }
 }
 
+SVDX_DEVINL void chunk_colsum(uint32_t buf, int lane, int rows, float* dst) {
+  const int pr = lane & 15, h = lane >> 4;
+  const uint32_t in_chunk = (uint32_t)(pr & 3) * 4u;
+  const int jch = pr >> 2;
+  float s0 = 0.f, s1 = 0.f;
+  for (int rr = h; rr < rows; rr += 2) {
+    uint32_t w;
+    asm volatile("ld.shared.u32 %0, [%1];" : "=r"(w) : "r"(buf + rr * 64 + ((uint32_t)(jch ^ ((rr >> 1) & 3)) << 4) + in_chunk));
+    const float2 v = unpack_bf16x2(w);
+    s0 += v.x; s1 += v.y;
+  }
+  s0 += __shfl_xor_sync(0xffffffffu, s0, 16); s1 += __shfl_xor_sync(0xffffffffu, s1, 16);
+  if (h == 0 && rows > 0) asm volatile("red.global.add.v2.f32 [%0], {%1, %2};" ::"l"(dst + 2 * pr), "f"(s0), "f"(s1) : "memory");
+}
+
 struct PairStage {
   uint32_t slots;
   int bar;
@@ -373,14 +395,22 @@
   for (int j = 0; j < 2; ++j) st_shared_v4(base16 + sw64((lane >> 2) + 8 * j, lane & 3), v[j].x, v[j].y, v[j].z, v[j].w);
 }
 
+SVDX_DEVINL void gbw_load_chunk0(const TapGemmKParams& p, const EpiTile& t, int sub, int lane, uint4 (&pa)[2], uint4 (&pb)[2]) {
+  const long long mw = t.m0 + 16 * sub;
+  const int vr = t.valid_rows - 16 * sub;
+  load_rows16(p.gpre + mw * p.ldgpre + t.n0, p.ldgpre, vr, lane, pa);
+  load_rows16(p.gpre + mw * p.ldgpre + p.N + t.n0, p.ldgpre, vr, lane, pb);
+}
+
 template <int EPI, int BN>
 SVDX_DEVINL void epilogue_regs(const TapGemmKParams& p, const float (&acc)[BN / 2], PairStage& ps, const EpiTile& t, int lane, float s_acc,
-                               float s_r1, float s_r2) {
+                               float s_r1, float s_r2, uint4 (&pa)[2], uint4 (&pb)[2]) {
   constexpr bool GEGLU = EPI == EPI_GEGLU;
   constexpr bool RES = EPI == EPI_RES || EPI == EPI_RES_GN;
   constexpr bool GN = EPI == EPI_FAST_GN || EPI == EPI_RES_GN || EPI == EPI_FAST_IL_GN;
   constexpr bool IL = EPI == EPI_FAST_IL || EPI == EPI_FAST_IL_GN;
   constexpr bool GNB = EPI == EPI_FAST_GNB;
+  constexpr bool GBW = EPI == EPI_GEGLU_BWD;
   constexpr int BN_OUT = GEGLU ? BN / 2 : BN;
   const int cq = 2 * (lane & 3);
   const bool issuer = ps.sub == 0 && lane == 0;
@@ -399,7 +429,7 @@
   for (int ch = 0; ch < BN_OUT / 32; ++ch) {
     const int col0 = t.n0 + 32 * ch;
     if (col0 >= t.n_out_total) break;
-    const uint32_t slot = ps.slots + 2048u * (GNB ? 2 * (ps.round & 1) : save_pre ? 2 : (ps.round & 3));
+    const uint32_t slot = ps.slots + 2048u * ((GNB || GBW) ? 2 * (ps.round & 1) : save_pre ? 2 : (ps.round & 3));
     const uint32_t mine = slot + 1024u * ps.sub;
     uint4 xa[2];
     if constexpr (RES) {
@@ -442,11 +472,35 @@
       }
     }
     if constexpr (EPI == EPI_FAST_ACT) act_n(f, p.act);
+    if constexpr (RES || GBW) {
+      if (p.scales) {
+#pragma unroll
+        for (int i = 0; i < 16; ++i) f[i] = __fmul_rn(f[i], s_acc);
+      }
+    }
+    if constexpr (GBW) {
+      uint32_t pv[8], pg[8];
+      stage_rows16(mine, lane, pa);
+      stage_rows16(mine + 2048u, lane, pb);
+      if (ch + 1 < BN_OUT / 32 && col0 + 32 < t.n_out_total) {
+        load_rows16(p.gpre + mw * p.ldgpre + col0 + 32, p.ldgpre, vr, lane, pa);
+        load_rows16(p.gpre + mw * p.ldgpre + p.N + col0 + 32, p.ldgpre, vr, lane, pb);
+      }
+      __syncwarp();
+      ldmatrix_x4(frag_row_addr(mine, lane, 0), pv[0], pv[1], pv[2], pv[3]);
+      ldmatrix_x4(frag_row_addr(mine, lane, 1), pv[4], pv[5], pv[6], pv[7]);
+      ldmatrix_x4(frag_row_addr(mine + 2048u, lane, 0), pg[0], pg[1], pg[2], pg[3]);
+      ldmatrix_x4(frag_row_addr(mine + 2048u, lane, 1), pg[4], pg[5], pg[6], pg[7]);
+      __syncwarp();
+#pragma unroll
+      for (int k = 0; k < 8; ++k) {
+        const float2 v = unpack_bf16x2(pv[k]), gt = unpack_bf16x2(pg[k]), d = unpack_bf16x2(pack_bf16x2(f[2 * k], f[2 * k + 1]));
+        const float2 e0 = geglu_bwd_elem(v.x, gt.x, d.x), e1 = geglu_bwd_elem(v.y, gt.y, d.y);
+        f[2 * k] = e0.x; f[2 * k + 1] = e1.x;
+        g[2 * k] = e0.y; g[2 * k + 1] = e1.y;
+      }
+    }
     if constexpr (RES) {
-      if (p.scales) {
-#pragma unroll
-        for (int i = 0; i < 16; ++i) f[i] = __fmul_rn(f[i], s_acc);
-      }
       if (p.res1) {
         uint32_t a1[8];
         stage_rows16(mine, lane, xa);
@@ -490,13 +544,21 @@
     }
     stage_frag16(mine, lane, f);
     if constexpr (GNB) stage_rows16(mine + 2048u, lane, xa);
+    if constexpr (GBW) stage_frag16(mine + 2048u, lane, g);
     fence_proxy_async_smem();
     if (issuer) {
-      if (GNB || save_pre) bulk_wait_read<0>();
+      if (GNB || GBW || save_pre) bulk_wait_read<0>();
       else bulk_wait_read<2>();
     }
     named_bar_sync(ps.bar, 64);
-    if (issuer) { store_chunk<IL>(p, slot, col0, t.row0, t.grp); bulk_commit(); }
+    if (issuer) {
+      store_chunk<IL>(p, slot, col0, t.row0, t.grp);
+      if constexpr (GBW) store_chunk<false>(p, slot + 2048u, t.n_out_total + col0, t.row0, t.grp);
+      bulk_commit();
+    }
+    if constexpr (GBW) {
+      if (p.gbias) chunk_colsum(slot + 2048u * ps.sub, lane, max(0, min(32, t.valid_rows)), p.gbias + ps.sub * t.n_out_total + col0);
+    }
     if constexpr (IL) {
       if ((ps.round & 1) == (uint32_t)ps.sub) il_store_next_row(p, slot, col0, t.row0, lane);
     }
diff --git a/svd_xtend_b200/engine.py b/svd_xtend_b200/engine.py
--- a/svd_xtend_b200/engine.py
+++ b/svd_xtend_b200/engine.py
@@ -12,7 +12,7 @@
 
 class Var:
 
-    __slots__ = ("data", "grad", "needs_grad", "owned", "csum", "gnb", "gnb_sums")
+    __slots__ = ("data", "grad", "needs_grad", "owned", "csum", "gnb", "gnb_sums", "geglu", "dpre")
 
     def __init__(self, data: torch.Tensor, needs_grad: bool = False):
         self.data = data
@@ -22,6 +22,8 @@
         self.csum = None
         self.gnb = None
         self.gnb_sums = None
+        self.geglu = None
+        self.dpre = None
 
     def take_grad(self) -> Optional[torch.Tensor]:
         g, self.grad, self.owned = self.grad, None, False
@@ -153,6 +155,25 @@
             return None
         sums = self.stat_zeros((M // ctx["rows"]) * 2 * N, device).view(M // ctx["rows"], 2, N)
         return dict(x=ctx["x"], x2=ctx["x2"], ab=ctx["ab"], rows=ctx["rows"], silu=ctx["silu"], sum=sums)
+
+    def _geglu_for(self, x: Var, M: int, N: int, K: int):
+        ctx = x.geglu
+        if ctx is None or x.grad is not None or x.dpre is not None or N % 32:
+            return None
+        if raw.split_plan(True, M, N, K) is not None:
+            return None
+        if K > 640:
+            m_tiles, sms = (M + 127) // 128, raw.num_sms()
+            waves = lambda bn: (m_tiles * ((N + bn - 1) // bn) + sms - 1) // sms
+            if waves(raw.choose_block_n(M, N, max_bn=128)) > waves(raw.choose_block_n(M, N)):
+                return None
+        return ctx
+
+    def _geglu_bias_grad(self, bias, scales, n: int) -> Optional[torch.Tensor]:
+        if bias is None or not bias.requires_grad or scales is not None:
+            return None
+        g = self.pgrad(bias)
+        return g if g.numel() == n else None
 
     def detach_tape(self) -> List[Callable[[], None]]:
         tape, self.tape = self.tape, []
@@ -358,12 +379,15 @@
         y = Var(out, need)
         if sink is not None:
             y.csum = (gn_rows, [(sink, N)])
+        if geglu and pre is not None and res1 is None and res2 is None and rowbias is None and blend is None and not lora:
+            y.geglu = dict(pre=pre, bias=bias, scales=scales)
         if need and self.recording:
             def bwd():
                 dy = y.take_grad()
-                if dy is None:
-                    return
-                if dy.dtype != bf16:
+                dpre, y.dpre = y.dpre, None
+                if dy is None and dpre is None:
+                    return
+                if dy is not None and dy.dtype != bf16:
                     dy = raw.cast_f32_bf16(dy.contiguous(), torch.empty(dy.shape, device=dy.device, dtype=bf16))
                 s_acc = None if scales is None else scales[0:1]
                 self._mix_grad(blend, dy, res1, out)
@@ -371,21 +395,30 @@
                 self._res_grad(res2, dy, None if scales is None else scales[2:3])
                 bias_done = False
                 if geglu:
-                    fuse_b = bias is not None and bias.requires_grad and scales is None and self.pgrad(bias).numel() == pre.shape[1]
-                    dyl = raw.geglu_bwd(pre, dy, torch.empty_like(pre), bias_grad=self.pgrad(bias) if fuse_b else None)
-                    bias_done = fuse_b
+                    bg = self._geglu_bias_grad(bias, scales, N)
+                    if dy is not None:
+                        d2 = raw.geglu_bwd(pre, dy, torch.empty_like(pre), bias_grad=bg)
+                        dpre = d2 if dpre is None else raw.axpby(dpre, d2, dpre)
+                    dyl = dpre
+                    bias_done = bg is not None
                 else:
                     dyl = dy
                 self._rowbias_grad(rowbias, dyl, rowbias_div, s_acc)
                 sc3 = self._acc_only(s_acc)
                 if x.needs_grad:
                     wt = self.w_lin_cat(ws, True) if fused is not None else self.w_lin(weight, True)
-                    dx = self.empty(M, K, x.data)
-                    gnb = None if lora else self._gnb_for(x, M, K, N, 1, sc3, dyl.device)
-                    raw.tapgemm_auto(dyl, wt, dx, M=M, N=K, K=N, scales=sc3, **({} if gnb is None else {"gnb": gnb}))
-                    self.add_grad(x, dx)
-                    if gnb is not None:
-                        x.gnb_sums = (gnb["sum"], dx)
+                    gg = None if lora else self._geglu_for(x, M, K, N)
+                    if gg is not None:
+                        x.dpre = self.empty(M, 2 * K, x.data)
+                        raw.tapgemm(dyl, wt, x.dpre, M=M, N=K, K=N, scales=sc3, geglu_pre=gg["pre"],
+                                    geglu_bias_grad=self._geglu_bias_grad(gg["bias"], gg["scales"], 2 * K))
+                    else:
+                        dx = self.empty(M, K, x.data)
+                        gnb = None if lora else self._gnb_for(x, M, K, N, 1, sc3, dyl.device)
+                        raw.tapgemm_auto(dyl, wt, dx, M=M, N=K, K=N, scales=sc3, **({} if gnb is None else {"gnb": gnb}))
+                        self.add_grad(x, dx)
+                        if gnb is not None:
+                            x.gnb_sums = (gnb["sum"], dx)
                 if any(p.requires_grad for p in ws):
                     self._wgrad(dyl, x.data, ws, N, K, M, sc3)
                 if bias is not None and bias.requires_grad and not bias_done:
diff --git a/svd_xtend_b200/raw.py b/svd_xtend_b200/raw.py
--- a/svd_xtend_b200/raw.py
+++ b/svd_xtend_b200/raw.py
@@ -99,7 +99,7 @@
     return waves * max(mma, l2)
 
 
-def choose_block_n(M: int, n_out: int, geglu: bool = False, mn_major: bool = False) -> int:
+def choose_block_n(M: int, n_out: int, geglu: bool = False, mn_major: bool = False, max_bn: int = 160) -> int:
     sms = num_sms()
     if mn_major:
         best, best_cost = None, None
@@ -109,7 +109,7 @@
             if best_cost is None or cost < best_cost - 1e-9:
                 best, best_cost = bn, cost
         return best
-    cands = [64, 32] if geglu else [160, 128, 96, 64, 32]
+    cands = [64, 32] if geglu else [bn for bn in (160, 128, 96, 64, 32) if bn <= max_bn]
     best, best_cost = None, None
     for bn in cands:
         if n_out % bn and n_out > bn:
@@ -209,9 +209,11 @@
     gnb: Optional[dict] = None,
     phase: Optional[Sequence[int]] = None,
     act: int = ACT_NONE,
+    geglu_pre: Optional[torch.Tensor] = None,
+    geglu_bias_grad: Optional[torch.Tensor] = None,
 ) -> torch.Tensor:
     family = "conv" if (mode == A_CONV2D or len(taps) > 1 or b_mode != 0) else "linear"
-    if _fam(family, 2.0 * M * N * K * len(taps)):
+    if _fam(family, 2.0 * M * N * K * len(taps), 0.0 if geglu_pre is None else 8.0 * M * N):
         return out
     if SHAPE_LOG is not None:
         SHAPE_LOG.append(dict(M=M, N=N, K=K, taps=len(taps), conv2d=int(mode == A_CONV2D), geglu=int(geglu), a_mn=int(a_mn), b_mode=b_mode,
@@ -228,7 +230,8 @@
                                               ("a", a), ("b", b), ("out", out), ("bias", bias), ("rowbias", rowbias), ("res1", res1),
                                               ("res2", res2), ("scales", scales), ("pre", pre), ("gn_sum", gn_sum),
                                               ("gnb_x", None if gnb is None else gnb["x"]), ("gnb_x2", None if gnb is None else gnb.get("x2")),
-                                              ("gnb_ab", None if gnb is None else gnb.get("ab")), ("gnb_sum", None if gnb is None else gnb["sum"]))
+                                              ("gnb_ab", None if gnb is None else gnb.get("ab")), ("gnb_sum", None if gnb is None else gnb["sum"]),
+                                              ("geglu_pre", geglu_pre), ("geglu_bias_grad", geglu_bias_grad))
                                               if t is not None})))
     d = SvdxTapGemm()
     assert a.dtype == bf16 and b.dtype == bf16
@@ -250,8 +253,8 @@
     d.M, d.N, d.K = M, N, K
     n_out = N // 2 if geglu else N
     if block_n is None:
-        block_n = choose_block_n(M, n_out, geglu, b_mn)
-        if _wide_tile_ok(M, N, K * len(taps), out, ldo, geglu, a_mn, b_mn, b_mode, split_k, out_dtype, bias, rowbias):
+        block_n = choose_block_n(M, n_out, geglu, b_mn, max_bn=160 if geglu_pre is None else 128)
+        if geglu_pre is None and _wide_tile_ok(M, N, K * len(taps), out, ldo, geglu, a_mn, b_mn, b_mode, split_k, out_dtype, bias, rowbias):
             block_n = 320
     d.block_n = block_n
     d.split_k = split_k
@@ -306,6 +309,11 @@
         d.interleave = 1
         d.phase_h, d.phase_w = int(phase[0]), int(phase[1])
     d.act = int(act)
+    if geglu_pre is not None:
+        assert geglu_pre.dtype == bf16 and (geglu_bias_grad is None or geglu_bias_grad.dtype == torch.float32)
+        d.geglu_pre = geglu_pre.data_ptr()
+        d.geglu_ldpre = _rowmajor(geglu_pre, "geglu_pre")
+        d.geglu_bias_grad = _ptr(geglu_bias_grad)
     check(load().svdx_tapgemm(C.byref(d), _stream()), "svdx_tapgemm")
     return out
 
```

Result: no change. 160.2 (median of 6 runs) (+0.5%).
